# quocdat32461997/ggpm

Hardware: AMD Instinct MI355X
Metric: HierMPNEncoder fwd+bwd target row (SURVEY 8(d): encoder + KL heads + optimizer, tree fixed-point hint on; full depth loops in full_depth_loops, the full VAE fwd+bwd row in vae_step) of BASELINE's molecules/sec VAE fwd+bwd (hidden=300, depth=20, batch=32) (higher is better)
Workload: dtype f32

## Files before the change

### ggpm_amd/_lib.py

```python
from __future__ import annotations

import ctypes
import os
from ctypes import c_char_p, c_double, c_float, c_int, c_size_t, c_void_p, POINTER

from . import build as _build

_LIB = None

P = c_void_p
I = c_int
SIGNATURES = {
    "ggpm_version": (I, []),
    "ggpm_error_string": (c_char_p, [I]),
    "ggpm_padded_hidden": (I, [I]),
    "ggpm_padded_to_csr": (I, [P, I, I, P, P, P]),
    "ggpm_csr_transpose": (I, [P, P, I, I, P, P, P, P]),
    "ggpm_extract_column": (I, [P, I, I, I, P, P]),
    "ggpm_gemm_workspace_bytes": (c_size_t, [I, I, I]),
    "ggpm_gemm": (I, [I, I, I, I, I, P, I, P, I, P, I, I, P, I, I, I, P, c_size_t, P]),
    "ggpm_gemm_grouped": (I, [I, I, I, I, I, I, P, P]),
    "ggpm_gemm_grouped_splitk_workspace_bytes": (c_size_t, [I, I, I, I]),
    "ggpm_gemm_grouped_splitk": (I, [I, I, I, I, I, I, P, P, c_size_t, P]),
    "ggpm_gemm_ksegments": (I, [I, I, I, I, P, P, P, P, P, P, I, I, P, I, I, I, P]),
    "ggpm_gemm_tn_bf16": (I, [I, I, I, P, I, P, I, P, I, P, c_size_t, P]),
    "ggpm_gemm_tn_bf16_applies": (I, [I, I, I]),
    "ggpm_colsum": (I, [P, I, I, I, P, P, P]),
    "ggpm_act_backward": (I, [P, P, I, I, I, I, I, P, P]),
    "ggpm_segment_sum": (I, [P, I, P, P, I, I, P, I, I, I, P]),
    "ggpm_gather_rows": (I, [P, I, P, I, I, P, I, I, I, P]),
    "ggpm_scatter_rows": (I, [P, I, P, I, I, P, I, I, P]),
    "ggpm_adam_step": (I, [P, P, P, P, c_size_t, c_float, c_float, c_float, c_float, c_float, I, P]),
    "ggpm_flat_sqnorm_workspace_bytes": (c_size_t, [c_size_t]),
    "ggpm_flat_sqnorm_partials": (I, [P, c_size_t, P, c_size_t, P]),
    "ggpm_flat_norm_finish": (I, [P, I, c_float, P, P]),
    "ggpm_adam_step_groups": (I, [P, P, P, P, c_size_t, P, I, P, I, P, I, c_float, P, I, P]),
    "ggpm_onehot": (I, [P, I, I, P, I, I, I, P]),
    "ggpm_embed_graph": (I, [P, I, P, I, I, I, I, P, I, P, I, P]),
    "ggpm_level_bf16_storage": (I, [I, I]),
    "ggpm_gru_backward_stashes": (I, [P, I, I, I, POINTER(c_void_p), POINTER(c_void_p)]),
    "ggpm_lstm_backward_stashes": (I, [P, I, I, I, POINTER(c_void_p), POINTER(c_void_p), POINTER(c_void_p)]),
    "ggpm_sum_slots": (I, [P, I, c_size_t, P, P]),
    "ggpm_gru_pack_floats": (c_size_t, [I]),
    "ggpm_gru_forward": (I, [I, I, I, P, P, P, P, I, P, I, P, P, I, P, P, P, P, P, P, P, P, P, P, I, P, P]),
    "ggpm_gru_backward_workspace_bytes": (c_size_t, [I, I, I]),
    "ggpm_gru_backward": (I, [I, I, I, P, P, I, P, I, P, I, P, P, P, P, P, P, P, P, P, P, P, P, P, P, P,
                              P, I, P, I, P, P, I, P, c_size_t, I, P, P]),
    "ggpm_gru_weight_grads": (I, [I, I, I, P, P, P, P, c_size_t, P, I, P, I, P, P, I, P, P]),
    "ggpm_gru_sparse_forward": (I, [I, I, I, P, P, P, P, P, P, I, P, I, P, P, I, P, P, P, P, P, P, P, P, P, P, I, P, P]),
    "ggpm_gru_sparse_backward": (I, [I, I, I, P, P, P, I, P, I, P, I, P, P, P, P, P, P, P, P, P, P, P, P, P, P, P, P,
                                     P, I, P, I, P, P, I, P, c_size_t, P, P]),
    "ggpm_weight_grads_stacked_workspace_bytes": (c_size_t, [I, I]),
    "ggpm_gru_weight_grads_stacked": (I, [I, I, I, P, P, P, P, P, P, P, I, P, I, P, P, I, P, c_size_t, P]),
    "ggpm_lstm_weight_grads_stacked": (I, [I, I, I, P, P, P, P, P, P, P, I, P, I, P, I, P, I, P, c_size_t, P]),
    "ggpm_decode_steps_forward": (I, [P, P, P, P, P, P, P, P, P, c_size_t, P, P, P]),
    "ggpm_decode_steps_backward": (I, [P, P, P, P, P, P, P, P, c_size_t, P, P, P, P, c_size_t, P, P, P, c_size_t, P, P]),
    "ggpm_decode_steps_forward_async": (I, [P, P, P, P, P, P, P, P, P, c_size_t, P, P, P]),
    "ggpm_decode_steps_backward_async": (I, [P, P, P, P, P, P, P, P, c_size_t, P, P, P, P, c_size_t, P, P, P, c_size_t, P, P]),
    "ggpm_decode_join": (I, []),
    "ggpm_decode_steps_infer": (I, [P, P, P, P, P, P, P, P, P, P, P, P]),
    "ggpm_decode_steps_infer_async": (I, [P, P, P, P, P, P, P, P, P, P, P, P]),
    "ggpm_lstm_pack_floats": (c_size_t, [I]),
    "ggpm_lstm_forward": (I, [I, I, I, P, P, P, P, P, I, P, I, P, I, P, I, P, P, P, P, P, P, P, P, P, P, P, I, P, P]),
    "ggpm_lstm_backward_workspace_bytes": (c_size_t, [I, I, I]),
    "ggpm_lstm_backward": (I, [I, I, I, P, P, I, P, I, P, I, P, I, P, P, P, P, P, P, P, P, P, P, P, P, P,
                               P, P, P, P, P, I, P, I, P, I, P, I, P, c_size_t, I, P, P]),
    "ggpm_lstm_weight_grads": (I, [I, I, I, P, P, P, c_size_t, P, I, P, I, P, I, P, I, P, P]),
    "ggpm_lstm_sparse_forward": (I, [I, I, I, P, P, P, P, P, P, P, P, I, P, I, P, I, P, I, P, P, P, P, P, P, P, P, P, P,
                                     P, I, P, P]),
    "ggpm_lstm_sparse_backward": (I, [I, I, I, P, P, P, I, P, I, P, I, P, I, P, P, P, P, P, P, P, P, P, P, P, P, P, P,
                                      P, P, P, P, P, P, P, I, P, I, P, I, P, I, P, c_size_t, P, P]),
    "ggpm_rsample_forward": (I, [P, P, P, I, I, P, P, P]),
    "ggpm_rsample_backward": (I, [P, P, P, P, P, I, I, P, P, P]),
    "ggpm_softmax_ce": (I, [P, I, I, I, P, I, P, P, P, P, I, P, P, P]),
    "ggpm_bce_logits": (I, [P, P, I, P, P, P, P]),
    "ggpm_scale_rows": (I, [P, I, I, I, P, P]),
    "ggpm_head_accuracies": (I, [P, P, P, P, I, P, I, P, I, P, I, I, I, I, P, P]),
    "ggpm_motif_assm_forward": (I, [P, I, P, I, I, I, I, P, I, P, P, P, P, I, P, P, P, P, P, P]),
    "ggpm_motif_assm_backward": (I, [P, P, I, P, I, I, I, I, I, P, I, P, P, P, I, P, P, P, P, P, P, P, P, P, P]),
    "ggpm_motif_decode_tree_step": (I, [I, I, I, I, POINTER(c_void_p), P, P, P, P, I, I, P, P, P, I, I, P, I, P, I, P, I,
                                        P, I, P]),
    "ggpm_motif_decode_mlp": (I, [P, I, P, P, I, I, I, I, P, P, P, P, I, I, P, I, P, I, P]),
    "ggpm_hier_topk": (I, [P, I, I, P, I, I, P, I, I, I, P, P]),
    "ggpm_motif_decode_assm_score": (I, [P, I, I, I, P, P, I, P, I, P, P, P, P, I, P, P]),
    "ggpm_hier_decode_atom_step": (I, [P, P, P, P, P, P, I, P]),
    "ggpm_hier_decode_tree_step": (I, [P, P, P, P, I, P, I, P, I, I, P, I, P, I, P]),
    "ggpm_hier_decode_assm_score": (I, [P, P, P, P, P, P, I, I, I, I, P, I, P, P, P, I, P, I, I, P, P]),
    "ggpm_sample_topo": (I, [P, P, P, I, I, ctypes.c_uint, ctypes.c_uint, P, P]),
    "ggpm_sample_beam_order": (I, [P, P, P, I, I, I, ctypes.c_uint, ctypes.c_uint, P, P]),
    "ggpm_sample_normal": (I, [P, I, I, I, P, ctypes.c_uint, ctypes.c_uint, P]),
    "ggpm_sample_latent_normal": (I, [P, I, I, I, P, ctypes.c_uint, ctypes.c_uint, P]),
    "ggpm_mol_loss_parts": (I, [P, I, P, P]),
    "ggpm_latent_terms": (I, [P, P, P, I, I, I, P, P, P, P]),
    "ggpm_iwae_finish": (I, [P, P, P, I, I, P, P, P]),
    "ggpm_dropout": (I, [P, I, I, I, ctypes.c_float, ctypes.c_uint, ctypes.c_uint, I, P]),
    "ggpm_property_heads_workspace_bytes": (c_size_t, [I, I, P, P]),
# ... 66 lines not shown
```

### ggpm_amd/csrc/common.h

```cpp
#pragma once
#include <hip/hip_runtime.h>
#include <stdint.h>
#include <stdlib.h>
#include <atomic>
#include <mutex>
#include "../../include/ggpm_hip.h"

typedef float f32x4 __attribute__((ext_vector_type(4)));
typedef float f32x16 __attribute__((ext_vector_type(16)));

#define GGPM_WAVE 64

#define GGPM_CHECK_LAUNCH()                                   \
    do {                                                      \
        if (hipGetLastError() != hipSuccess) return GGPM_ERR_LAUNCH; \
    } while (0)

#define GGPM_CLEAR_STALE_ERROR() (void)hipGetLastError()

#ifdef GGPM_DEV_SWITCHES
inline const char* ggpm_dev_env(const char* name) { return getenv(name); }
#else
inline const char* ggpm_dev_env(const char*) { return nullptr; }
#endif
// ... 48 lines not shown
__device__ __forceinline__ float4 operator*(float4 a, float4 b) {
    return make_float4(a.x * b.x, a.y * b.y, a.z * b.z, a.w * b.w);
}
__device__ __forceinline__ float4 ggpm_sigmoid4(float4 a) {
    return make_float4(ggpm_sigmoid(a.x), ggpm_sigmoid(a.y), ggpm_sigmoid(a.z), ggpm_sigmoid(a.w));
}
__device__ __forceinline__ float4 ggpm_zero4() { return make_float4(0.f, 0.f, 0.f, 0.f); }
__device__ __forceinline__ float ggpm_fsigmoid_fast(float x) { return __frcp_rn(1.0f + __expf(-x)); }
__device__ __forceinline__ float ggpm_fsigmoid_acc(float x) {
    const float L_hi = 1.44269502162933349609375f, L_lo = 1.925963033500011e-08f, LN2 = 0.693147182464599609375f;
    const float nx = -__builtin_amdgcn_fmed3f(x, -88.f, 88.f);
    const float t = nx * L_hi;
    float lo = __builtin_fmaf(nx, L_hi, -t);
    lo = __builtin_fmaf(nx, L_lo, lo);
    float e = __builtin_amdgcn_exp2f(t);
    e = __builtin_fmaf(e, lo * LN2, e);
    const float d = 1.0f + e;
    const float r = __builtin_amdgcn_rcpf(d);
    return __builtin_fmaf(__builtin_fmaf(-d, r, 1.0f), r, r);
}
#ifdef GGPM_ABL_EXACT_GATHER_SIGMOID
template <bool BF16> __device__ __forceinline__ float ggpm_fsigmoid(float x) { return ggpm_sigmoid(x); }
#elif defined(GGPM_ABL_FAST_GATHER_SIGMOID)
template <bool BF16> __device__ __forceinline__ float ggpm_fsigmoid(float x) { return ggpm_fsigmoid_fast(x); }
#elif defined(GGPM_ABL_FAST_SIGMOID_BF16)
template <bool BF16> __device__ __forceinline__ float ggpm_fsigmoid(float x) { return BF16 ? ggpm_fsigmoid_fast(x) : ggpm_fsigmoid_acc(x); }
#else
template <bool BF16> __device__ __forceinline__ float ggpm_fsigmoid(float x) { return ggpm_fsigmoid_acc(x); }
#endif
template <bool BF16> __device__ __forceinline__ float4 ggpm_fsigmoid4(float4 a) {
    return make_float4(ggpm_fsigmoid<BF16>(a.x), ggpm_fsigmoid<BF16>(a.y), ggpm_fsigmoid<BF16>(a.z), ggpm_fsigmoid<BF16>(a.w));
}

__device__ __forceinline__ void ggpm_lds_barrier() {
    asm volatile("s_waitcnt lgkmcnt(0)\n\ts_barrier" ::: "memory");
}

bool ggpm_gemm_prefers_grouped(int M, int N, int K, int count);
int ggpm_gemm_tall_grouped(int M, int N, int count, const ggpm_gemm_problem* p, const int* K, float* ws, size_t ws_bytes,
                           ggpm_stream_t stream, int bf16 = 0);
#define GGPM_GEMM_MAX_GROUP 4
typedef ggpm_gemm_problem GgpmGemmProblem;

inline const ggpm_level_opts& ggpm_opts_or_default(const ggpm_level_opts* opts) {
    static const ggpm_level_opts none = {};
    return opts ? *opts : none;
}
int ggpm_gru_bias_u_grad(int E1, int H, int depth, int lo, float* work, float* dbu, float* csws, const ggpm_level_opts* opts,
                         ggpm_stream_t stream);
int ggpm_gru_sparse_weight_grads(int E1, int H, int depth, const float* Hs, const float* Ss, const float* Gs, float* work,
                                 size_t work_bytes, float* dWz_h, int ld_dwz, float* dUr, int ld_dur, float* dbu, float* dWh_h,
                                 int ld_dwh, const ggpm_level_opts* opts, ggpm_stream_t stream);
int ggpm_lstm_sparse_weight_grads(int E1, int H, int depth, const float* Hs, const float* Ss, float* work, size_t work_bytes,
                                  float* dWi_h, int ld_dwi, float* dWo_h, int ld_dwo, float* dWu_h, int ld_dwu, float* dWf_h,
                                  int ld_dwf, const ggpm_level_opts* opts, ggpm_stream_t stream);
hipEvent_t ggpm_wgrad_event(int i);

bool ggpm_bf16_storage_applies(int E1, int H);
int ggpm_sum_slots_any(const float* src, int slots, size_t slot_floats, float* out, bool src_bf16, ggpm_stream_t stream);
int ggpm_sum_slots_pair_grouped(int count, const float* const* src, const int* slots, size_t slot_floats, float* const* hi,
                                float* const* lo, ggpm_stream_t stream);
struct ggpm_pair_problem { const float *hi, *lo, *B; float* C; int ldc; };
int ggpm_gemm_tn_pair_grouped(int M, int N, int rows, int ld, int count, const ggpm_pair_problem* p, ggpm_stream_t stream);
int ggpm_colsum_any(const float* A, int lda, int rows, int cols, float* out, float* scratch, bool a_bf16, ggpm_stream_t stream);

void ggpm_timing_tag(int tag);
// ... 3 lines not shown
```

### ggpm_amd/csrc/encoder.hip

```cpp
#include "common.h"
#include <condition_variable>
#include <cstring>
#include <cstdlib>
#include <deque>
#include <functional>
#include <mutex>
#include <thread>

hipEvent_t ggpm_wgrad_event(int i);

namespace {

struct Arena {
    char* base;
    size_t off;
    bool overflow;
    size_t cap;
    template <typename T>
    T* take(size_t n) {
        const size_t bytes = (n * sizeof(T) + 255) & ~(size_t)255;
        T* p = base ? reinterpret_cast<T*>(base + off) : nullptr;
        off += bytes;
        if (base && off > cap) overflow = true;
        return p;
// ... 279 lines not shown
inline int backward_lo(const Dims& d, int level, int depth, int E1) {
    static const bool off = ggpm_dev_env("GGPM_TREE_FIXED_POINT") && atoi(ggpm_dev_env("GGPM_TREE_FIXED_POINT")) == 0;
    if (off || level == 2 || bf16_stored(d, E1) || d.tree_chain <= 0) return 1;
    const int lo = depth - d.tree_chain + 1;
    return lo < 1 ? 1 : lo;
}

inline int fixed_slot(const Dims& d, int level, int depth, int E1) {
    const int run = run_steps(d, level, depth, E1);
    if (run >= depth || d.gate_dtype == 1) return 0;
    const int blo = backward_lo(d, level, depth, E1);
    return (blo >= run && blo >= 3) ? run : 0;
}

int replicate_tail(const Dims& d, int E1, int depth, int run, int level, const LevelSaved& L, ggpm_stream_t s) {
    if (run >= depth || fixed_slot(d, level, depth, E1)) return GGPM_OK;
    const size_t slot = (size_t)E1 * d.Hp, ds = (size_t)depth * slot;
    const int blo = backward_lo(d, level, depth, E1);
    ReplicateArgs r = {};
    int n = 0;
    auto add = [&](float* base, int src, int lo, int hi) {
        r.base[n] = base; r.src[n] = src; r.lo[n] = lo > src ? lo : src + 1; r.hi[n] = hi; ++n;
    };
    add(L.Hs, run, blo, depth);
    if (L.Cs) add(L.Cs, run, blo, depth);
    add(L.Qs, run, blo, depth - 1);
    for (int k = 0; k < 5; ++k) add(L.St + k * ds, run - 1, blo - 1, depth - 1);
    r.slot4 = slot / 4;
    dim3 grid((unsigned)ggpm_ceil_div((int)r.slot4, 256 * 4), n);
    replicate_slots_k<<<grid, 256, 0, (hipStream_t)s>>>(r);
    return GGPM_OK;
}

int level_forward(const Dims& d, int E1, int N1, int I, int depth, const float* x, int ldx, float* const* P, int level,
                  const Csr& pred, const Csr& agr, LevelSaved& L, ggpm_stream_t s) {
    const int H = d.H, Hp = d.Hp;
    const size_t slot = (size_t)E1 * Hp;
    const int run = run_steps(d, level, depth, E1);
    struct Tag { Tag(int level) { ggpm_timing_tag(3 - level); } ~Tag() { ggpm_timing_tag(0); } } tag(level);
    ggpm_level_opts o = level_opts(d);
    o.run_depth = run;
    const bool infer = L.hout != nullptr;
    o.h_out = L.hout;
    const int fs = infer ? 0 : fixed_slot(d, level, depth, E1);
    o.fixed_slot = fs;
    const float* result = infer ? L.hout : L.Hs + (size_t)(fs ? fs : depth) * slot;
    if (d.lstm) {
        const float* W[4] = {P[lq(level, Q_WI)], P[lq(level, Q_WOG)], P[lq(level, Q_WU)], P[lq(level, Q_WF)]};
        const float* b[4] = {P[lq(level, Q_BI)], P[lq(level, Q_BOG)], P[lq(level, Q_BU)], P[lq(level, Q_BF)]};
        GgpmGemmProblem gp[4];
        for (int k = 0; k < 4; ++k) gp[k] = {x, ldx, W[k], I + H, L.X + k * slot, Hp, Hp, b[k], 0, GGPM_ACT_NONE, 0};
        CK(ggpm_gemm_grouped(0, 1, E1, H, I, 4, gp, s));
        const size_t dsl = (size_t)depth * slot;
        CK(ggpm_lstm_forward(E1, H, depth, L.X, L.X + slot, L.X + 2 * slot, L.X + 3 * slot, W[0] + I, I + H, W[1] + I, I + H,
                             W[2] + I, I + H, W[3] + I, I + H, pred.rowptr, pred.col, L.Hs, L.Cs, L.Qs,
                             infer ? nullptr : L.St, infer ? nullptr : L.St + dsl, infer ? nullptr : L.St + 2 * dsl,
                             infer ? nullptr : L.St + 3 * dsl, infer ? nullptr : L.St + 4 * dsl, L.wpack, infer ? 0 : 1, &o, s));
        if (!infer) CK(replicate_tail(d, E1, depth, run, level, L, s));
        CK(ggpm_segment_sum(result, Hp, agr.rowptr, agr.col, N1, H, L.nei, Hp, 0, Hp, s));
        return GGPM_OK;
    }
    const float *Wz = P[lp(level, L_WZ)], *Wr = P[lp(level, L_WR)], *Wh = P[lp(level, L_WH)];
    const GgpmGemmProblem gp[3] = {{x, ldx, Wz, I + H, L.X, Hp, Hp, P[lp(level, L_BZ)], 0, GGPM_ACT_NONE, 0},
                                   {x, ldx, Wr, I, L.X + slot, Hp, Hp, nullptr, 0, GGPM_ACT_NONE, 0},
                                   {x, ldx, Wh, I + H, L.X + 2 * slot, Hp, Hp, P[lp(level, L_BH)], 0, GGPM_ACT_NONE, 0}};
    CK(ggpm_gemm_grouped(0, 1, E1, H, I, 3, gp, s));
    const size_t ds = (size_t)depth * slot;
    CK(ggpm_gru_forward(E1, H, depth, L.X, L.X + slot, L.X + 2 * slot, Wz + I, I + H, P[lp(level, L_UR)], H,
                            P[lp(level, L_BU)], Wh + I, I + H, pred.rowptr, pred.col,
                            L.Hs, L.Qs, infer ? nullptr : L.St, infer ? nullptr : L.St + ds, infer ? nullptr : L.St + 2 * ds,
                            infer ? nullptr : L.St + 3 * ds, infer ? nullptr : L.St + 4 * ds, L.wpack, infer ? 0 : 1, &o, s));
    if (!infer) CK(replicate_tail(d, E1, depth, run, level, L, s));
    CK(ggpm_segment_sum(result, Hp, agr.rowptr, agr.col, N1, H, L.nei, Hp, 0, Hp, s));
    return GGPM_OK;
}

int transpose(const Csr& c, const int32_t* col, ggpm_stream_t s) {
    return ggpm_csr_transpose(c.rowptr, col ? col : c.col, c.rows, c.ncols, c.rowptrT, c.colT, c.cursor, s);
}

}

extern "C" size_t ggpm_encoder_saved_bytes(const ggpm_enc_dims* dims) {
    if (!dims) return 0;
    const Dims d = make_dims(dims);
    Arena A = {nullptr, 0, false, 0};
    Saved s;
    layout_saved(A, d, s);
    return A.off;
}

extern "C" size_t ggpm_encoder_infer_bytes(const ggpm_enc_dims* dims) {
    if (!dims) return 0;
    const Dims d = make_dims(dims);
    Arena A = {nullptr, 0, false, 0};
    Saved s;
    layout_infer(A, d, s);
    return A.off;
}

static int encoder_forward_impl(const ggpm_enc_dims* dims, float* const* params, const int64_t* tfnode,
                                const int64_t* tfmess, const int64_t* tagraph, const int64_t* tbgraph,
                                const int64_t* tcgraph, const int64_t* gfnode, const int64_t* gfmess,
                                const int64_t* gagraph, const int64_t* gbgraph, const int32_t* roots, void* saved,
                                size_t saved_bytes, float* hroot, float* hnode, float* hinter, float* hatom,
                                ggpm_stream_t stream, ggpm_stream_t side_stream, bool infer) {
    GGPM_CLEAR_STALE_ERROR();
    if (!dims || !params || !tfnode || !tfmess || !tagraph || !tbgraph || !tcgraph || !gfnode || !gfmess || !gagraph ||
        !gbgraph || !roots || !saved || !hroot || !hnode || !hinter || !hatom)
        return GGPM_ERR_ARG;
    const Dims d = make_dims(dims);
    Arena A = {reinterpret_cast<char*>(saved), 0, false, saved_bytes};
    Saved S;
    if (infer) layout_infer(A, d, S);
    else layout_saved(A, d, S);
    if (A.overflow) return GGPM_ERR_WORKSPACE;
    hipStream_t s = (hipStream_t)stream;
    float* const* P = params;
    const int H = d.H, Hp = d.Hp, He = d.He;

    ggpm_stream_t ts = side_stream ? side_stream : stream;
    SideWorker* wk = side_stream ? SideWorker::get() : nullptr;
    DrainGuard guard = {wk};
    hipEvent_t ev_in = nullptr;
    if (side_stream) {
        ev_in = ggpm_wgrad_event(60);
        if (!ev_in) return GGPM_ERR_LAUNCH;
        (void)hipEventRecord(ev_in, s);
    }
    CK(ggpm_padded_to_csr(gbgraph, d.E1g, d.Kgb, S.gpred.rowptr, S.gpred.col, stream));
    CK(ggpm_padded_to_csr(gagraph, d.N1g, d.Kga, S.gagr.rowptr, S.gagr.col, stream));
    hipEvent_t ev_atom = nullptr, ev_tree = nullptr;
    if (side_stream) {
        ev_atom = ggpm_wgrad_event(54);
        ev_tree = ggpm_wgrad_event(53);
        if (!ev_atom || !ev_tree) return GGPM_ERR_LAUNCH;
        (void)hipEventRecord(ev_atom, s);
    }
    auto tree_layout = [=]() -> int {
        if (side_stream) (void)hipStreamWaitEvent((hipStream_t)side_stream, ev_in, 0);
        CK(ggpm_padded_to_csr(tbgraph, d.E1t, d.Ktb, S.tpred.rowptr, S.tpred.col, ts));
        CK(ggpm_padded_to_csr(tagraph, d.N1t, d.Kta, S.tagr.rowptr, S.tagr.col, ts));
        CK(ggpm_padded_to_csr(tcgraph, d.N1t, d.Ktc, S.tcgr.rowptr, S.tcgr.col, ts));
        CK(ggpm_extract_column(tfmess, d.E1t, 4, 0, S.src, ts));
        CK(ggpm_extract_column(tfmess, d.E1t, 4, 2, S.attr0, ts));
        CK(ggpm_extract_column(tfnode, d.N1t, 2, 0, S.motif_id, ts));
        CK(ggpm_extract_column(tfnode, d.N1t, 2, 1, S.attach_id, ts));
        if (!infer) {
            const int nio = (d.E1t > d.N1t ? d.E1t : d.N1t) + 1;
            const int n = nio > d.B + 1 ? nio : d.B + 1;
            iota_k<<<ggpm_ceil_div(n, 256), 256, 0, (hipStream_t)ts>>>(S.iota, n);
        }
        CK(ggpm_gather_rows(P[P_EI], He, S.attach_id, d.N1t, He, S.finput_i, d.Hep, 0, d.Hep, ts));
        CK(drop(d, S.finput_i, d.N1t, He, d.Hep, DS_EI, ts));
        CK(ggpm_gather_rows(P[P_EC], He, S.motif_id, d.N1t, He, S.finput_t, d.Hep, 0, d.Hep, ts));
        CK(drop(d, S.finput_t, d.N1t, He, d.Hep, DS_EC, ts));
        CK(ggpm_onehot(S.attr0, d.E1t, 20, S.hmess_i, d.ld_t, H, d.ld_t, ts));
        CK(ggpm_onehot(S.attr0, d.E1t, 20, S.hmess_t, d.ld_t, H, d.ld_t, ts));
        if (side_stream) (void)hipEventRecord(ev_tree, (hipStream_t)side_stream);
        if (infer) return GGPM_OK;
        if (side_stream) (void)hipStreamWaitEvent((hipStream_t)side_stream, ev_atom, 0);
        CK(transpose(S.gpred, nullptr, ts));
        CK(transpose(S.gagr, nullptr, ts));
        CK(transpose(S.tpred, nullptr, ts));
        CK(transpose(S.tagr, nullptr, ts));
        CK(transpose(S.tcgr, nullptr, ts));
        CK(transpose(S.tsrc, S.src, ts));
        CK(transpose(S.root, roots, ts));
        CK(transpose(S.motif, S.motif_id, ts));
        CK(transpose(S.attach, S.attach_id, ts));
        return GGPM_OK;
    };
    if (wk) {
        int dev = 0;
        (void)hipGetDevice(&dev);
        wk->use_device(dev);
        wk->post(tree_layout);
    } else {
        CK(tree_layout());
    }

    CK(ggpm_embed_graph(gfnode, d.N1g, gfmess, d.E1g, d.atom, 4, 20, S.hnode_a, d.ld_n, S.hmess_a, d.ld_m, stream));
    CK(level_forward(d, d.E1g, d.N1g, d.Ig, d.depthG, S.hmess_a, d.ld_m, P, 2, S.gpred, S.gagr, S.lv[2], stream));
    CK(linear2(d.N1g, H, S.hnode_a, d.ld_n, d.atom, S.lv[2].nei, Hp, H, P[lwo(d.lstm, 2)], P[lbo(d.lstm, 2)], GGPM_ACT_RELU, 1,
               hatom, Hp, stream));
    CK(drop(d, hatom, d.N1g, H, Hp, DS_WO_ATOM, stream));

    if (wk) CK(wk->drain());
    if (side_stream) (void)hipStreamWaitEvent(s, ev_tree, 0);
    CK(ggpm_segment_sum(hatom, Hp, S.tcgr.rowptr, S.tcgr.col, d.N1t, H, S.pooled, Hp, 0, Hp, stream));
    CK(linear2(d.N1t, H, S.finput_i, d.Hep, He, S.pooled, Hp, H, P[P_WI], P[P_BI], GGPM_ACT_RELU, 0, S.hnode_i, Hp,
               stream));
    CK(drop(d, S.hnode_i, d.N1t, H, Hp, DS_WI, stream));
    CK(ggpm_gather_rows(S.hnode_i, Hp, S.src, d.E1t, H, S.hmess_i, d.ld_t, 0, 0, stream));
    CK(level_forward(d, d.E1t, d.N1t, d.It, d.depthT, S.hmess_i, d.ld_t, P, 1, S.tpred, S.tagr, S.lv[1], stream));
    CK(linear2(d.N1t, H, S.hnode_i, Hp, H, S.lv[1].nei, Hp, H, P[lwo(d.lstm, 1)], P[lbo(d.lstm, 1)], GGPM_ACT_RELU, 1, hinter, Hp,
               stream));
    CK(drop(d, hinter, d.N1t, H, Hp, DS_WO_INTER, stream));

    CK(linear2(d.N1t, H, S.finput_t, d.Hep, He, hinter, Hp, H, P[P_WC], P[P_BC], GGPM_ACT_RELU, 0, S.hnode_t, Hp, stream));
    CK(drop(d, S.hnode_t, d.N1t, H, Hp, DS_WC, stream));
    CK(ggpm_gather_rows(S.hnode_t, Hp, S.src, d.E1t, H, S.hmess_t, d.ld_t, 0, 0, stream));
    CK(level_forward(d, d.E1t, d.N1t, d.It, d.depthT, S.hmess_t, d.ld_t, P, 0, S.tpred, S.tagr, S.lv[0], stream));
    CK(linear2(d.N1t, H, S.hnode_t, Hp, H, S.lv[0].nei, Hp, H, P[lwo(d.lstm, 0)], P[lbo(d.lstm, 0)], GGPM_ACT_RELU, 1, hnode, Hp,
               stream));
    CK(drop(d, hnode, d.N1t, H, Hp, DS_WO_TREE, stream));

    CK(ggpm_gather_rows(S.hnode_t, Hp, roots, d.B, H, S.f, Hp, 0, Hp, stream));
    CK(ggpm_gather_rows(S.lv[0].nei, Hp, roots, d.B, H, S.n, Hp, 0, Hp, stream));
    CK(linear2(d.B, H, S.f, Hp, H, S.n, Hp, H, P[P_WROOT], P[P_BROOT], GGPM_ACT_TANH, 0, hroot, Hp, stream));
    GGPM_CHECK_LAUNCH();
    return GGPM_OK;
}

extern "C" int ggpm_encoder_forward(const ggpm_enc_dims* dims, float* const* params, const int64_t* tfnode,
                                    const int64_t* tfmess, const int64_t* tagraph, const int64_t* tbgraph,
                                    const int64_t* tcgraph, const int64_t* gfnode, const int64_t* gfmess,
                                    const int64_t* gagraph, const int64_t* gbgraph, const int32_t* roots, void* saved,
                                    size_t saved_bytes, float* hroot, float* hnode, float* hinter, float* hatom,
                                    ggpm_stream_t stream, ggpm_stream_t side_stream) {
    return encoder_forward_impl(dims, params, tfnode, tfmess, tagraph, tbgraph, tcgraph, gfnode, gfmess, gagraph, gbgraph,
                                roots, saved, saved_bytes, hroot, hnode, hinter, hatom, stream, side_stream, false);
}

extern "C" int ggpm_encoder_infer(const ggpm_enc_dims* dims, float* const* params, const int64_t* tfnode,
                                  const int64_t* tfmess, const int64_t* tagraph, const int64_t* tbgraph,
                                  const int64_t* tcgraph, const int64_t* gfnode, const int64_t* gfmess,
                                  const int64_t* gagraph, const int64_t* gbgraph, const int32_t* roots, void* arena,
                                  size_t arena_bytes, float* hroot, float* hnode, float* hinter, float* hatom,
                                  ggpm_stream_t stream, ggpm_stream_t side_stream) {
    return encoder_forward_impl(dims, params, tfnode, tfmess, tagraph, tbgraph, tcgraph, gfnode, gfmess, gagraph, gbgraph,
                                roots, arena, arena_bytes, hroot, hnode, hinter, hatom, stream, side_stream, true);
}

namespace {

struct BwdWork {
    float *dpre_root, *df, *dn, *d_hnode_t, *d_nei_t, *dpre, *d_h, *dX, *dx_mess, *d_finput, *d_hinter, *d_hnode_i,
        *d_nei_i, *d_pooled, *d_hatom, *d_nei_g, *level_work, *skws, *csws;
    size_t level_work_bytes, skws_bytes;
    float *xws[3], *xcs[3];
    size_t xws_bytes;
};

void layout_work(Arena& A, const Dims& d, BwdWork& w) {
    const int Hp = d.Hp;
    const int Nmax = d.N1g > d.N1t ? d.N1g : d.N1t, Emax = d.E1g > d.E1t ? d.E1g : d.E1t;
    w.dpre_root = A.take<float>((size_t)d.B * Hp); w.df = A.take<float>((size_t)d.B * Hp);
    w.dn = A.take<float>((size_t)d.B * Hp);
    w.d_hnode_t = A.take<float>((size_t)d.N1t * Hp); w.d_nei_t = A.take<float>((size_t)d.N1t * Hp);
    w.dpre = A.take<float>((size_t)5 * Nmax * Hp);
    w.d_h = A.take<float>((size_t)Emax * Hp);
    w.dX = A.take<float>((size_t)3 * 4 * Emax * Hp);
    w.dx_mess = A.take<float>((size_t)d.E1t * d.ld_t);
    w.d_finput = A.take<float>((size_t)2 * d.N1t * d.Hep);
    w.d_hinter = A.take<float>((size_t)d.N1t * Hp);
    w.d_hnode_i = A.take<float>((size_t)d.N1t * Hp); w.d_nei_i = A.take<float>((size_t)d.N1t * Hp);
    w.d_pooled = A.take<float>((size_t)d.N1t * Hp);
    w.d_hatom = A.take<float>((size_t)d.N1g * Hp); w.d_nei_g = A.take<float>((size_t)d.N1g * Hp);
    size_t lw = d.lstm ? ggpm_lstm_backward_workspace_bytes(d.E1g, d.H, d.depthG)
                       : ggpm_gru_backward_workspace_bytes(d.E1g, d.H, d.depthG);
    const size_t lwt = d.lstm ? ggpm_lstm_backward_workspace_bytes(d.E1t, d.H, d.depthT)
                              : ggpm_gru_backward_workspace_bytes(d.E1t, d.H, d.depthT);
    w.level_work_bytes = lw > lwt ? lw : lwt;
    w.level_work = A.take<float>(3 * (w.level_work_bytes / 4 + 64));
    size_t sk = 0;
    const int Imax = d.It > d.Ig ? d.It : d.Ig;
    const size_t cand[] = {ggpm_gemm_workspace_bytes(d.H, Imax, Emax), ggpm_gemm_workspace_bytes(d.H, d.Hp, Nmax),
                           ggpm_gemm_workspace_bytes(d.H, d.Hp, d.B)};
    for (size_t c : cand) sk = c > sk ? c : sk;
    w.skws_bytes = sk + 1024;
    w.skws = A.take<float>(w.skws_bytes / 4);
    w.csws = A.take<float>((size_t)256 * (Hp > d.ld_t ? Hp : d.ld_t));
    const int gates = d.lstm ? 4 : 3;
    const size_t xa = ggpm_gemm_grouped_splitk_workspace_bytes(d.H, d.It, d.E1t, gates);
    const size_t xb = ggpm_gemm_grouped_splitk_workspace_bytes(d.H, d.Ig, d.E1g, gates);
    w.xws_bytes = (xa > xb ? xa : xb) + 256;
    for (int l = 0; l < 3; ++l) {
        w.xws[l] = A.take<float>(w.xws_bytes / 4);
        w.xcs[l] = A.take<float>((size_t)256 * Hp);
    }
}

struct Streams {
    ggpm_stream_t main, side;
    int n_ev;
    SideWorker* wk;
    int side_after_main() {
        if (!side) return GGPM_OK;
        hipEvent_t ev = ggpm_wgrad_event(n_ev++ & 31);
        if (!ev) return GGPM_ERR_LAUNCH;
        (void)hipEventRecord(ev, (hipStream_t)main);
// ... 14 lines not shown
};

int linear2_dx(int M, int H, int K1, const float* dpre, int ldp, const float* W, float* d1, int ld1, int acc1, float* d2,
               int ld2, int acc2, ggpm_stream_t s) {
    const int ldw = K1 + H;
    if (K1 == H) {
        const GgpmGemmProblem gp[2] = {{dpre, ldp, W, ldw, d1, ld1, ld1, nullptr, acc1, GGPM_ACT_NONE, 0},
                                       {dpre, ldp, W + K1, ldw, d2, ld2, ld2, nullptr, acc2, GGPM_ACT_NONE, 0}};
        return ggpm_gemm_grouped(0, 0, M, H, H, 2, gp, s);
    }
    CK(ggpm_gemm(0, 0, M, K1, H, dpre, ldp, W, ldw, d1, ld1, ld1, nullptr, acc1, GGPM_ACT_NONE, 0, nullptr, 0, s));
    CK(ggpm_gemm(0, 0, M, H, H, dpre, ldp, W + K1, ldw, d2, ld2, ld2, nullptr, acc2, GGPM_ACT_NONE, 0, nullptr, 0, s));
    return GGPM_OK;
}

int linear2_wgrad(int M, int N, const float* dpre, int ldp, const float* x1, int ld1, int K1, const float* x2, int ld2,
                  int K2, float* dW, float* db, BwdWork& w, Streams& st) {
    CK(st.side_after_main());
    const int ldw = K1 + K2;
    const ggpm_stream_t sw = st.w();
    float* const skws = w.skws;
    float* const csws = w.csws;
    const size_t skb = w.skws_bytes;
    return st.on_side([=]() -> int {
        CK(ggpm_gemm(1, 0, N, K1, M, dpre, ldp, x1, ld1, dW, ldw, K1, nullptr, 0, GGPM_ACT_NONE, 0, skws, skb, sw));
        CK(ggpm_gemm(1, 0, N, K2, M, dpre, ldp, x2, ld2, dW + K1, ldw, K2, nullptr, 0, GGPM_ACT_NONE, 0, skws, skb, sw));
        if (db) CK(ggpm_colsum(dpre, ldp, M, N, db, csws, sw));
        return GGPM_OK;
    });
}

int level_backward(const Dims& d, int E1, int I, int depth, const float* x, int ldx, float* const* P, float* const* G,
                   int level, const Csr& pred, const LevelSaved& L, const float* dHD, float* dX, float* level_work,
                   float* dx, int lddx, BwdWork& w, Streams& st) {
    const int H = d.H, Hp = d.Hp;
    const size_t slot = (size_t)E1 * Hp, ds = (size_t)depth * slot;
    const int blo = backward_lo(d, level, depth, E1);
    struct Tag { Tag(int level) { ggpm_timing_tag(3 - level); } ~Tag() { ggpm_timing_tag(0); } } tag(level);
    static const bool xsum_env = !(ggpm_dev_env("GGPM_SKIP_XSUM") && atoi(ggpm_dev_env("GGPM_SKIP_XSUM")) == 0);
    const bool skip_xsum = xsum_env && dx == nullptr && depth > 1;
    ggpm_level_opts o = level_opts(d);
    o.lo = blo;
    o.fixed_slot = fixed_slot(d, level, depth, E1);
    o.skip_x_sums = skip_xsum;
    if (d.lstm) {
        const float* W[4] = {P[lq(level, Q_WI)], P[lq(level, Q_WOG)], P[lq(level, Q_WU)], P[lq(level, Q_WF)]};
        float* dW[4] = {G[lq(level, Q_WI)], G[lq(level, Q_WOG)], G[lq(level, Q_WU)], G[lq(level, Q_WF)]};
        float* db[4] = {G[lq(level, Q_BI)], G[lq(level, Q_BOG)], G[lq(level, Q_BU)], G[lq(level, Q_BF)]};
        CK(ggpm_lstm_backward(E1, H, depth, L.X + 3 * slot, W[0] + I, I + H, W[1] + I, I + H, W[2] + I, I + H, W[3] + I, I + H,
                              pred.rowptr, pred.col, pred.rowptrT, pred.colT, L.Hs, L.Cs, L.Qs, L.St, L.St + ds,
                              L.St + 2 * ds, L.St + 3 * ds, L.St + 4 * ds, dHD, dX, dX + slot, dX + 2 * slot, dX + 3 * slot,
                              dW[0] + I, I + H, dW[1] + I, I + H, dW[2] + I, I + H, dW[3] + I, I + H, level_work,
                              w.level_work_bytes, 0, &o, st.main));
        if (dx) {
            const float* A[4] = {dX, dX + slot, dX + 2 * slot, dX + 3 * slot};
            const int lda[4] = {Hp, Hp, Hp, Hp}, ldb[4] = {I + H, I + H, I + H, I + H}, K[4] = {H, H, H, H};
            CK(ggpm_gemm_ksegments(0, E1, I, 4, A, lda, W, ldb, K, dx, lddx, lddx, nullptr, 0, GGPM_ACT_NONE, 0, st.main));
        }
        CK(st.side_after_main());
        const ggpm_stream_t sw = st.w();
        const BwdWork wc = w;
        float* const dW0 = dW[0]; float* const dW1 = dW[1]; float* const dW2 = dW[2]; float* const dW3 = dW[3];
        float* const db0 = db[0]; float* const db1 = db[1]; float* const db2 = db[2]; float* const db3 = db[3];
        const float* Hs = L.Hs; const float* St = L.St;
        auto x_part = [=](ggpm_stream_t sx) -> int {
            float* const dWk[4] = {dW0, dW1, dW2, dW3};
            float* const dbk[4] = {db0, db1, db2, db3};
            if (skip_xsum) {
                float *DI = nullptr, *DO = nullptr, *DU = nullptr;
                CK(ggpm_lstm_backward_stashes(level_work, E1, H, depth, &DI, &DO, &DU));
                const int lo_ = blo < 1 ? 1 : blo;
                float* const src[3] = {DI, DO, DU};
                const bool b16 = bf16_stored(d, E1);
                for (int k = 0; k < 3; ++k)
                    CK(ggpm_sum_slots_any(src[k] + (b16 ? 0 : (size_t)(lo_ - 1) * slot), depth - lo_ + 1, slot, dX + (size_t)k * slot,
                                          b16, sx));
            }
// ... 94 lines not shown
                                     const float* hnode, const float* hinter, const float* hatom, const float* d_hroot,
                                     const float* d_hnode, const float* d_hinter, const float* d_hatom, void* work,
                                     size_t work_bytes, int phase, ggpm_stream_t stream, ggpm_stream_t side_stream) {
    GGPM_CLEAR_STALE_ERROR();
    if (!dims || !params || !grads || !roots || !saved || !work || !hroot || !hnode || !hinter || !hatom || phase < 0 ||
        phase > 2)
        return GGPM_ERR_ARG;
    const Dims d = make_dims(dims);
    Arena A = {reinterpret_cast<char*>(saved), 0, false, saved_bytes};
    Saved S;
    layout_saved(A, d, S);
    Arena B = {reinterpret_cast<char*>(work), 0, false, work_bytes};
    BwdWork w;
    layout_work(B, d, w);
    if (A.overflow || B.overflow) return GGPM_ERR_WORKSPACE;
    hipStream_t s = (hipStream_t)stream;
    float* const* P = params;
    float* const* G = grads;
    const int H = d.H, Hp = d.Hp, He = d.He;
    Streams st = {stream, side_stream, 0, side_stream ? SideWorker::get() : nullptr};
    DrainGuard guard = {st.wk};
    if (st.wk) {
        int dev = 0;
        (void)hipGetDevice(&dev);
        st.wk->use_device(dev);
    }
    const int Nmax = d.N1g > d.N1t ? d.N1g : d.N1t, Emax = d.E1g > d.E1t ? d.E1g : d.E1t;
    float* dpre[5];
    for (int i = 0; i < 5; ++i) dpre[i] = w.dpre + (size_t)i * Nmax * Hp;
    float* dXl[3];
    for (int i = 0; i < 3; ++i) dXl[i] = w.dX + (size_t)i * 4 * Emax * Hp;
    float* lwork[3];
    for (int i = 0; i < 3; ++i) lwork[i] = w.level_work + (size_t)i * (w.level_work_bytes / 4 + 64);
    const size_t nt = (size_t)d.N1t * Hp * sizeof(float), ng = (size_t)d.N1g * Hp * sizeof(float);

    if (side_stream && phase != 2) {
        hipEvent_t ev = ggpm_wgrad_event(61);
        if (!ev) return GGPM_ERR_LAUNCH;
        (void)hipEventRecord(ev, (hipStream_t)side_stream);
        (void)hipStreamWaitEvent(s, ev, 0);
    }
    if (phase != 2) {
    if (d_hroot) {
        CK(ggpm_act_backward(d_hroot, hroot, d.B, H, Hp, GGPM_ACT_TANH, 0, w.dpre_root, stream));
        CK(linear2_dx(d.B, H, H, w.dpre_root, Hp, P[P_WROOT], w.df, Hp, 0, w.dn, Hp, 0, stream));
        CK(ggpm_segment_sum(w.df, Hp, S.root.rowptrT, S.root.colT, d.N1t, H, w.d_hnode_t, Hp, 0, Hp, stream));
        CK(ggpm_segment_sum(w.dn, Hp, S.root.rowptrT, S.root.colT, d.N1t, H, w.d_nei_t, Hp, 0, Hp, stream));
        CK(linear2_wgrad(d.B, H, w.dpre_root, Hp, S.f, Hp, H, S.n, Hp, H, G[P_WROOT], G[P_BROOT], w, st));
    } else {
        (void)hipMemsetAsync(w.d_hnode_t, 0, nt, s);
        (void)hipMemsetAsync(w.d_nei_t, 0, nt, s);
        float* const gw = G[P_WROOT]; float* const gb = G[P_BROOT];
        const ggpm_stream_t sw = st.w();
        CK(st.on_side([=]() -> int {
            (void)hipMemsetAsync(gw, 0, (size_t)H * 2 * H * sizeof(float), (hipStream_t)sw);
            (void)hipMemsetAsync(gb, 0, (size_t)H * sizeof(float), (hipStream_t)sw);
            return GGPM_OK;
        }));
    }

    if (d_hnode) {
        CK(ggpm_act_backward(d_hnode, hnode, d.N1t, H, Hp, GGPM_ACT_RELU, 1, dpre[0], stream));
        CK(drop(d, dpre[0], d.N1t, H, Hp, DS_WO_TREE, stream));
        CK(linear2_dx(d.N1t, H, H, dpre[0], Hp, P[lwo(d.lstm, 0)], w.d_hnode_t, Hp, 1, w.d_nei_t, Hp, 1, stream));
        CK(linear2_wgrad(d.N1t, H, dpre[0], Hp, S.hnode_t, Hp, H, S.lv[0].nei, Hp, H, G[lwo(d.lstm, 0)], G[lbo(d.lstm, 0)], w, st));
    } else {
        float* const gw = G[lwo(d.lstm, 0)]; float* const gb = G[lbo(d.lstm, 0)];
        const ggpm_stream_t sw = st.w();
        CK(st.on_side([=]() -> int {
            (void)hipMemsetAsync(gw, 0, (size_t)H * 2 * H * sizeof(float), (hipStream_t)sw);
            (void)hipMemsetAsync(gb, 0, (size_t)H * sizeof(float), (hipStream_t)sw);
            return GGPM_OK;
        }));
    }
    CK(ggpm_segment_sum(w.d_nei_t, Hp, S.tagr.rowptrT, S.tagr.colT, d.E1t, H, w.d_h, Hp, 0, Hp, stream));
    CK(level_backward(d, d.E1t, d.It, d.depthT, S.hmess_t, d.ld_t, P, G, 0, S.tpred, S.lv[0], w.d_h, dXl[0], lwork[0],
                      w.dx_mess, d.ld_t, w, st));
    CK(ggpm_segment_sum(w.dx_mess, d.ld_t, S.tsrc.rowptrT, S.tsrc.colT, d.N1t, H, w.d_hnode_t, Hp, 1, 0, stream));
    CK(ggpm_act_backward(w.d_hnode_t, S.hnode_t, d.N1t, H, Hp, GGPM_ACT_RELU, 0, dpre[1], stream));
    CK(drop(d, dpre[1], d.N1t, H, Hp, DS_WC, stream));
    if (d_hinter) (void)hipMemcpyAsync(w.d_hinter, d_hinter, nt, hipMemcpyDeviceToDevice, s);
    CK(linear2_dx(d.N1t, H, He, dpre[1], Hp, P[P_WC], w.d_finput, d.Hep, 0, w.d_hinter, Hp, d_hinter ? 1 : 0, stream));
    CK(drop(d, w.d_finput, d.N1t, He, d.Hep, DS_EC, stream));
    CK(linear2_wgrad(d.N1t, H, dpre[1], Hp, S.finput_t, d.Hep, He, hinter, Hp, H, G[P_WC], G[P_BC], w, st));
    {
        const float* src = w.d_finput; const int32_t* rp = S.motif.rowptrT; const int32_t* cl = S.motif.colT;
        float* const g = G[P_EC]; const ggpm_stream_t sw = st.w(); const int Hep = d.Hep, rows = d.n_motif;
        CK(st.on_side([=]() -> int { return ggpm_segment_sum(src, Hep, rp, cl, rows, He, g, He, 0, He, sw); }));
    }

    CK(ggpm_act_backward(w.d_hinter, hinter, d.N1t, H, Hp, GGPM_ACT_RELU, 1, dpre[2], stream));
    CK(drop(d, dpre[2], d.N1t, H, Hp, DS_WO_INTER, stream));
    CK(linear2_dx(d.N1t, H, H, dpre[2], Hp, P[lwo(d.lstm, 1)], w.d_hnode_i, Hp, 0, w.d_nei_i, Hp, 0, stream));
    CK(linear2_wgrad(d.N1t, H, dpre[2], Hp, S.hnode_i, Hp, H, S.lv[1].nei, Hp, H, G[lwo(d.lstm, 1)], G[lbo(d.lstm, 1)], w, st));
    CK(ggpm_segment_sum(w.d_nei_i, Hp, S.tagr.rowptrT, S.tagr.colT, d.E1t, H, w.d_h, Hp, 0, Hp, stream));
    CK(level_backward(d, d.E1t, d.It, d.depthT, S.hmess_i, d.ld_t, P, G, 1, S.tpred, S.lv[1], w.d_h, dXl[1], lwork[1],
                      w.dx_mess, d.ld_t, w, st));
    CK(ggpm_segment_sum(w.dx_mess, d.ld_t, S.tsrc.rowptrT, S.tsrc.colT, d.N1t, H, w.d_hnode_i, Hp, 1, 0, stream));
    CK(ggpm_act_backward(w.d_hnode_i, S.hnode_i, d.N1t, H, Hp, GGPM_ACT_RELU, 0, dpre[3], stream));
    CK(drop(d, dpre[3], d.N1t, H, Hp, DS_WI, stream));
    float* d_finput_i = w.d_finput + (size_t)d.N1t * d.Hep;
    CK(linear2_dx(d.N1t, H, He, dpre[3], Hp, P[P_WI], d_finput_i, d.Hep, 0, w.d_pooled, Hp, 0, stream));
    CK(drop(d, d_finput_i, d.N1t, He, d.Hep, DS_EI, stream));
    CK(linear2_wgrad(d.N1t, H, dpre[3], Hp, S.finput_i, d.Hep, He, S.pooled, Hp, H, G[P_WI], G[P_BI], w, st));
    {
        const int32_t* rp = S.attach.rowptrT; const int32_t* cl = S.attach.colT;
        float* const g = G[P_EI]; const ggpm_stream_t sw = st.w(); const int Hep = d.Hep, rows = d.n_attach;
        CK(st.on_side([=]() -> int { return ggpm_segment_sum(d_finput_i, Hep, rp, cl, rows, He, g, He, 0, He, sw); }));
    }
    if (d_hatom) (void)hipMemcpyAsync(w.d_hatom, d_hatom, ng, hipMemcpyDeviceToDevice, s);
    CK(ggpm_segment_sum(w.d_pooled, Hp, S.tcgr.rowptrT, S.tcgr.colT, d.N1g, H, w.d_hatom, Hp, d_hatom ? 1 : 0,
                        d_hatom ? 0 : Hp, stream));

    }
    if (phase == 1) {
        CK(st.drain());
        GGPM_CHECK_LAUNCH();
        return GGPM_OK;
    }

    CK(ggpm_act_backward(w.d_hatom, hatom, d.N1g, H, Hp, GGPM_ACT_RELU, 1, dpre[4], stream));
    CK(drop(d, dpre[4], d.N1g, H, Hp, DS_WO_ATOM, stream));
    CK(ggpm_gemm(0, 0, d.N1g, H, H, dpre[4], Hp, P[lwo(d.lstm, 2)] + d.atom, d.atom + H, w.d_nei_g, Hp, Hp, nullptr, 0,
                 GGPM_ACT_NONE, 0, nullptr, 0, stream));
    CK(linear2_wgrad(d.N1g, H, dpre[4], Hp, S.hnode_a, d.ld_n, d.atom, S.lv[2].nei, Hp, H, G[lwo(d.lstm, 2)], G[lbo(d.lstm, 2)], w,
                     st));
    CK(ggpm_segment_sum(w.d_nei_g, Hp, S.gagr.rowptrT, S.gagr.colT, d.E1g, H, w.d_h, Hp, 0, Hp, stream));
    CK(level_backward(d, d.E1g, d.Ig, d.depthG, S.hmess_a, d.ld_m, P, G, 2, S.gpred, S.lv[2], w.d_h, dXl[2], lwork[2],
                      nullptr, 0, w, st));

    CK(st.drain());
    if (side_stream) {
        hipEvent_t ev = ggpm_wgrad_event(62);
        if (!ev) return GGPM_ERR_LAUNCH;
        (void)hipEventRecord(ev, (hipStream_t)side_stream);
        (void)hipStreamWaitEvent(s, ev, 0);
    }
    GGPM_CHECK_LAUNCH();
    return GGPM_OK;
}
```

### ggpm_amd/csrc/gather.hip

```cpp
#include "common.h"
#include <cmath>

namespace {

template <bool VEC>
__global__ void __launch_bounds__(256) segment_sum_k(const float* __restrict__ src, int ld_src,
                                                     const int32_t* __restrict__ rowptr,
                                                     const int32_t* __restrict__ col, int rows, int width,
                                                     float* __restrict__ out, int ld_out, int accumulate, int zero_to) {
    const int lane = threadIdx.x & 63;
    const int r = blockIdx.x * 4 + (threadIdx.x >> 6);
    if (r >= rows) return;
    const int lo = rowptr[r], hi = rowptr[r + 1];
    float* dst = out + (size_t)r * ld_out;
    for (int c = width + lane; c < zero_to; c += 64) dst[c] = 0.f;
    if (VEC) {
        for (int c = lane * 4; c < width; c += 256) {
            float4 acc = accumulate ? ggpm_ld4(dst + c) : ggpm_zero4();
            for (int j = lo; j < hi; ++j) acc = acc + ggpm_ld4(src + (size_t)col[j] * ld_src + c);
            ggpm_st4(dst + c, acc);
        }
    } else {
        for (int c = lane; c < width; c += 64) {
            float acc = accumulate ? dst[c] : 0.f;
            for (int j = lo; j < hi; ++j) acc += src[(size_t)col[j] * ld_src + c];
            dst[c] = acc;
        }
    }
}

__global__ void __launch_bounds__(256) gather_rows_k(const float* __restrict__ table, int ld_table,
                                                     const int32_t* __restrict__ idx, int rows, int width,
                                                     float* __restrict__ out, int ld_out, int col_off, int zero_to) {
    const int lane = threadIdx.x & 63;
    const int r = blockIdx.x * 4 + (threadIdx.x >> 6);
    if (r >= rows) return;
    const int id = idx[r];
    float* dst = out + (size_t)r * ld_out + col_off;
    for (int c = width + lane; c < zero_to - col_off; c += 64) dst[c] = 0.f;
    if (id < 0) {
        for (int c = lane; c < width; c += 64) dst[c] = 0.f;
    } else {
        const float* s = table + (size_t)id * ld_table;
        for (int c = lane; c < width; c += 64) dst[c] = s[c];
    }
}

__global__ void __launch_bounds__(256) scatter_rows_k(const float* __restrict__ src, int ld_src,
                                                      const int32_t* __restrict__ idx, int rows, int width,
                                                      float* __restrict__ dst, int ld_dst, int accumulate) {
    const int lane = threadIdx.x & 63;
    const int r = blockIdx.x * 4 + (threadIdx.x >> 6);
    if (r >= rows) return;
    const int id = idx[r];
    if (id < 0) return;
    const float* s = src + (size_t)r * ld_src;
    float* d = dst + (size_t)id * ld_dst;
    if (accumulate) for (int c = lane; c < width; c += 64) d[c] += s[c];
    else for (int c = lane; c < width; c += 64) d[c] = s[c];
}

__global__ void onehot_k(const int32_t* __restrict__ idx, int rows, int classes, float* __restrict__ out,
                         int ld_out, int col_off, int zero_to) {
    const int c = blockIdx.x * blockDim.x + threadIdx.x;
    const int r = blockIdx.y;
    if (col_off + c >= (zero_to > col_off + classes ? zero_to : col_off + classes)) return;
    out[(size_t)r * ld_out + col_off + c] = (c < classes && idx[r] == c) ? 1.f : 0.f;
}

__global__ void embed_graph_k(const int64_t* __restrict__ fnode, int N1, const int64_t* __restrict__ fmess,
                              int E1, int atom_size, int bond_types, int max_pos, float* __restrict__ hnode,
                              int ld_n, float* __restrict__ hmess, int ld_m) {
    const int r = blockIdx.x;
    const int c = threadIdx.x;
    if (r < N1) {
        if (c < ld_n) hnode[(size_t)r * ld_n + c] = (c < atom_size && fnode[r] == c) ? 1.f : 0.f;
    } else {
        const int e = r - N1;
        if (e < E1 && c < ld_m) {
            const int64_t* f = fmess + (size_t)e * 4;
            const int64_t a = fnode[f[0]];
            float v = 0.f;
            if (c < atom_size) v = (a == c) ? 1.f : 0.f;
            else if (c < atom_size + bond_types) v = (f[2] == c - atom_size) ? 1.f : 0.f;
            else if (c < atom_size + bond_types + max_pos) v = (f[3] == c - atom_size - bond_types) ? 1.f : 0.f;
            hmess[(size_t)e * ld_m + c] = v;
        }
    }
}

}

extern "C" int ggpm_segment_sum(const float* src, int ld_src, const int32_t* rowptr, const int32_t* col,
                                int rows, int width, float* out, int ld_out, int accumulate, int zero_to,
                                ggpm_stream_t stream) {
    GGPM_CLEAR_STALE_ERROR();
    if (!src || !rowptr || !col || !out || rows <= 0 || width <= 0) return GGPM_ERR_ARG;
    hipStream_t s = (hipStream_t)stream;
    const bool vec = (width % 4 == 0) && (ld_src % 4 == 0) && (ld_out % 4 == 0) &&
                     (((uintptr_t)src & 15) == 0) && (((uintptr_t)out & 15) == 0);
    const int grid = ggpm_ceil_div(rows, 4);
    if (vec) segment_sum_k<true><<<grid, 256, 0, s>>>(src, ld_src, rowptr, col, rows, width, out, ld_out, accumulate,
                                                           zero_to);
    else segment_sum_k<false><<<grid, 256, 0, s>>>(src, ld_src, rowptr, col, rows, width, out, ld_out, accumulate, zero_to);
    GGPM_CHECK_LAUNCH();
    return GGPM_OK;
}

extern "C" int ggpm_gather_rows(const float* table, int ld_table, const int32_t* idx, int rows, int width,
                                float* out, int ld_out, int col_off, int zero_to, ggpm_stream_t stream) {
    GGPM_CLEAR_STALE_ERROR();
    if (!table || !idx || !out || rows <= 0 || width <= 0) return GGPM_ERR_ARG;
    gather_rows_k<<<ggpm_ceil_div(rows, 4), 256, 0, (hipStream_t)stream>>>(table, ld_table, idx, rows, width, out,
                                                                          ld_out, col_off, zero_to);
    GGPM_CHECK_LAUNCH();
    return GGPM_OK;
}

extern "C" int ggpm_scatter_rows(const float* src, int ld_src, const int32_t* idx, int rows, int width, float* dst,
                                 int ld_dst, int accumulate, ggpm_stream_t stream) {
    GGPM_CLEAR_STALE_ERROR();
    if (!src || !idx || !dst || rows <= 0 || width <= 0) return GGPM_ERR_ARG;
    scatter_rows_k<<<ggpm_ceil_div(rows, 4), 256, 0, (hipStream_t)stream>>>(src, ld_src, idx, rows, width, dst, ld_dst,
                                                                           accumulate);
    GGPM_CHECK_LAUNCH();
    return GGPM_OK;
}

extern "C" int ggpm_onehot(const int32_t* idx, int rows, int classes, float* out, int ld_out, int col_off, int zero_to,
                           ggpm_stream_t stream) {
    GGPM_CLEAR_STALE_ERROR();
    if (!idx || !out || rows <= 0 || classes <= 0) return GGPM_ERR_ARG;
    const int span = (zero_to > col_off + classes ? zero_to - col_off : classes);
    dim3 grid(ggpm_ceil_div(span, 64), rows);
    onehot_k<<<grid, 64, 0, (hipStream_t)stream>>>(idx, rows, classes, out, ld_out, col_off, zero_to);
    GGPM_CHECK_LAUNCH();
    return GGPM_OK;
}

extern "C" int ggpm_embed_graph(const int64_t* fnode, int N1, const int64_t* fmess, int E1, int atom_size,
                                int bond_types, int max_pos, float* hnode, int ld_n, float* hmess, int ld_m,
                                ggpm_stream_t stream) {
    GGPM_CLEAR_STALE_ERROR();
    if (!fnode || !fmess || !hnode || !hmess || N1 <= 0 || E1 <= 0) return GGPM_ERR_ARG;
    if (ld_n > 256 || ld_m > 256 || ld_n < atom_size || ld_m < atom_size + bond_types + max_pos)
        return GGPM_ERR_UNSUPPORTED;
    embed_graph_k<<<N1 + E1, 256, 0, (hipStream_t)stream>>>(fnode, N1, fmess, E1, atom_size, bond_types, max_pos,
                                                           hnode, ld_n, hmess, ld_m);
    GGPM_CHECK_LAUNCH();
    return GGPM_OK;
}


namespace {
__device__ __forceinline__ unsigned int fmix32(unsigned int h) {
    h ^= h >> 16; h *= 0x85EBCA6Bu; h ^= h >> 13; h *= 0xC2B2AE35u; h ^= h >> 16;
    return h;
}

__global__ void dropout_k(float* __restrict__ x, int rows, int cols, int ld, unsigned int thresh, float scale,
                          unsigned int seed_lo, unsigned int seed_hi, unsigned int site) {
    const int c = blockIdx.x * blockDim.x + threadIdx.x;
    const int r = blockIdx.y;
    if (c >= cols) return;
    const unsigned int idx = (unsigned int)r * (unsigned int)cols + (unsigned int)c;
    unsigned int h = fmix32(idx * 0x9E3779B1u + seed_lo);
    h = fmix32(h ^ (seed_hi + site * 0x7F4A7C15u));
    float* p = x + (size_t)r * ld + c;
    *p = ((h >> 8) >= thresh) ? *p * scale : 0.f;
}
}

namespace {
__global__ void __launch_bounds__(256) adam_flat_k(float* __restrict__ p, const float* __restrict__ g,
                                                   float* __restrict__ m, float* __restrict__ v, size_t n, float b1,
                                                   float b2, float eps, float wd, float step_size, float inv_bc2_sqrt) {
    const size_t n4 = n >> 2;
    for (size_t i = (size_t)blockIdx.x * blockDim.x + threadIdx.x; i < n4; i += (size_t)gridDim.x * blockDim.x) {
        float4 pp = ggpm_ld4(p + 4 * i), gg = ggpm_ld4(g + 4 * i), mm = ggpm_ld4(m + 4 * i), vv = ggpm_ld4(v + 4 * i);
        float* P = &pp.x; float* G = &gg.x; float* M = &mm.x; float* V = &vv.x;
#pragma unroll
// ... 207 lines not shown
```

### ggpm_amd/csrc/gemm.hip

```cpp
#include <stdio.h>
#include <stdlib.h>
#include "common.h"

namespace {

constexpr int BM = 64, BN = 64, BK = 32, LDT = 68;

struct GemmArgs {
    int M, N, K;
    const float* A; int lda;
    const float* B; int ldb;
    float* C; int ldc; int n_pad;
    const float* bias;
    int accumulate, act, zero_row0;
    int vecA, vecB;
    int k_chunk;
    float* ws;
    unsigned long long* dbg;
    int nseg;
    const float* segA[GGPM_GEMM_MAX_GROUP];
    const float* segB[GGPM_GEMM_MAX_GROUP];
    int seg_lda[GGPM_GEMM_MAX_GROUP], seg_ldb[GGPM_GEMM_MAX_GROUP], segK[GGPM_GEMM_MAX_GROUP];
};

struct GemmGroupArgs {
    GemmArgs p[GGPM_GEMM_MAX_GROUP];
};

__device__ __forceinline__ float apply_act(float v, int act) {
    switch (act) {
        case GGPM_ACT_RELU: return v > 0.f ? v : 0.f;
        case GGPM_ACT_TANH: return tanhf(v);
        case GGPM_ACT_SIGMOID: return ggpm_sigmoid(v);
        default: return v;
    }
}

template <bool CONTIG_K>
__device__ __forceinline__ void fetch_tile(const float* __restrict__ P, int ld, int r0, int R, int k0, int kend,
                                           bool vec, float4 (&v)[2]) {
#pragma unroll
    for (int i = 0; i < 2; ++i) {
        const int f = threadIdx.x + 256 * i;
        float4 x = ggpm_zero4();
        if (CONTIG_K) {
            const int gr = r0 + (f >> 3), gk = k0 + (f & 7) * 4;
            if (gr < R && gk < kend) {
                const float* src = P + (size_t)gr * ld + gk;
                if (vec && gk + 3 < kend) x = ggpm_ld4(src);
                else {
                    x.x = src[0];
                    if (gk + 1 < kend) x.y = src[1];
                    if (gk + 2 < kend) x.z = src[2];
                    if (gk + 3 < kend) x.w = src[3];
                }
            }
        } else {
            const int gk = k0 + (f >> 4), gr = r0 + (f & 15) * 4;
            if (gk < kend && gr < R) {
                const float* src = P + (size_t)gk * ld + gr;
                if (vec && gr + 3 < R) x = ggpm_ld4(src);
                else {
                    x.x = src[0];
                    if (gr + 1 < R) x.y = src[1];
                    if (gr + 2 < R) x.z = src[2];
                    if (gr + 3 < R) x.w = src[3];
                }
            }
// ... 36 lines not shown
        fetch_tile<!TA>(g.A, g.lda, m0, g.M, kbeg, kend, g.vecA != 0, ra);
        fetch_tile<TB>(g.B, g.ldb, n0, g.N, kbeg, kend, g.vecB != 0, rb);
        for (int k0 = kbeg; k0 < kend; k0 += BK) {
            stash_tile<!TA>(ra, As);
            stash_tile<TB>(rb, Bs);
            __syncthreads();
            if (k0 + BK < kend) {
                fetch_tile<!TA>(g.A, g.lda, m0, g.M, k0 + BK, kend, g.vecA != 0, ra);
                fetch_tile<TB>(g.B, g.ldb, n0, g.N, k0 + BK, kend, g.vecB != 0, rb);
            }
#pragma unroll
            for (int kk = 0; kk < BK; kk += 2) {
                float a = As[kk + (lane >> 5)][wm * 32 + (lane & 31)];
                float b = Bs[kk + (lane >> 5)][wn * 32 + (lane & 31)];
                acc = __builtin_amdgcn_mfma_f32_32x32x2f32(a, b, acc, 0, 0, 0);
            }
            __syncthreads();
        }
    }

    const int n = n0 + wn * 32 + (lane & 31);
#pragma unroll
    for (int r = 0; r < 16; ++r) {
        const int m = m0 + wm * 32 + (r & 3) + 8 * (r >> 2) + 4 * (lane >> 5);
        if (m >= g.M) continue;
        if (g.ws) {
            if (n < g.N) g.ws[((size_t)blockIdx.z * g.M + m) * g.N + n] = acc[r];
            continue;
        }
        if (n < g.N) {
            float v = acc[r];
            if (g.bias) v += g.bias[n];
            float* dst = g.C + (size_t)m * g.ldc + n;
            if (g.accumulate) v += *dst;
            v = apply_act(v, g.act);
            if (g.zero_row0 && m == 0) v = 0.f;
            *dst = v;
        } else if (n < g.n_pad) {
            g.C[(size_t)m * g.ldc + n] = 0.f;
        }
    }
}

constexpr int BK2 = 64;

template <bool CONTIG_K>
struct OperandStage {
    __amdgpu_buffer_rsrc_t rs;
    unsigned voff[4], vstep;
    int loff[4];
    int kq[4];

    __device__ __forceinline__ void init(const float* P, int ld, int r0, int R, int kbeg, int kend, int total_rows) {
        const size_t last = CONTIG_K ? (size_t)(total_rows - 1) * ld + kend : (size_t)(max(kend, 1) - 1) * ld + R;
        const size_t bytes = kend > 0 ? last * 4 : 0;
        rs = __builtin_amdgcn_make_buffer_rsrc(const_cast<float*>(P), 0, (unsigned)bytes, 0x00020000);
#pragma unroll
        for (int i = 0; i < 4; ++i) {
            const int f = threadIdx.x + 256 * i;
            if (CONTIG_K) {
                const int r = f >> 4, k4 = (f & 15) * 4;
                kq[i] = k4;
                loff[i] = k4 * LDT + r;
                voff[i] = r0 + r < R ? (unsigned)(((size_t)(r0 + r) * ld + kbeg + k4) * 4) : 0xffffff00u;
            } else {
                const int k = f >> 4, c = (f & 15) * 4;
                kq[i] = 0;
// ... 73 lines not shown
            if (sg) ggpm_lds_barrier();
#pragma unroll
            for (int i = 0; i < 4; ++i) { sa.load(ra0[i], i); sb.load(rb0[i], i); }
#pragma unroll
            for (int i = 0; i < 4; ++i) {
                sa.store(Ls[0][0], ra0[i], i, kend - kbeg);
                sb.store(Ls[0][1], rb0[i], i, kend - kbeg);
            }
#pragma unroll
            for (int i = 0; i < 4; ++i) { sa.load(ra1[i], i); sb.load(rb1[i], i); }
            ggpm_lds_barrier();
            frag(0, 0, 0);
            for (int k0 = kbeg; k0 < kend; k0 += 2 * BK2) {
                step(ra1, rb1, ra0, rb0, 0, kend - k0 - BK2);
                step(ra0, rb0, ra1, rb1, 1, kend - k0 - 2 * BK2);
            }
        }
        asm volatile("s_nop 15\n\ts_nop 15" ::: "memory");
    }

    const int n = n0 + wn * 32 + (lane & 31);
#pragma unroll
    for (int r = 0; r < 16; ++r) {
        const int m = m0 + wm * 32 + (r & 3) + 8 * (r >> 2) + 4 * (lane >> 5);
        if (m >= g.M) continue;
        if (g.ws) {
            if (n < g.N) g.ws[((size_t)bz * g.M + m) * g.N + n] = acc[r];
            continue;
        }
        if (n < g.N) {
            float v = acc[r];
            if (g.bias) v += g.bias[n];
            float* dst = g.C + (size_t)m * g.ldc + n;
            if (g.accumulate) v += *dst;
            v = apply_act(v, g.act);
            if (g.zero_row0 && m == 0) v = 0.f;
            *dst = v;
        } else if (n < g.n_pad) {
            g.C[(size_t)m * g.ldc + n] = 0.f;
        }
    }
}

__device__ __forceinline__ void xcd_tile(int& bx, int& by, int& bz) {
    const unsigned T = gridDim.x * gridDim.y * gridDim.z;
    const unsigned L = blockIdx.x + gridDim.x * (blockIdx.y + gridDim.y * blockIdx.z);
    const unsigned xq = T >> 3, xr = T & 7, xcd = L & 7;
    const unsigned logical = xcd * xq + min(xcd, xr) + (L >> 3);
    bx = logical % gridDim.x;
    by = (logical / gridDim.x) % gridDim.y;
    bz = logical / (gridDim.x * gridDim.y);
}

template <bool TA, bool TB>
__global__ void __launch_bounds__(256) gemm_kernel_v2(GemmArgs g) {
    __shared__ __attribute__((aligned(16))) float Ls[2][2][BK2 * LDT];
    int bx, by, bz;
    xcd_tile(bx, by, bz);
    gemm_v2_tile<TA, TB>(g, bx, by, bz, Ls);
}

template <bool TA, bool TB>
__global__ void __launch_bounds__(256) gemm_group_v2(GemmGroupArgs gg) {
    __shared__ __attribute__((aligned(16))) float Ls[2][2][BK2 * LDT];
    int bx, by, bz;
    xcd_tile(bx, by, bz);
    gemm_v2_tile<TA, TB>(gg.p[bz], bx, by, 0, Ls);
// ... 141 lines not shown
#pragma unroll
        for (int i = 0; i < 2; ++i) { sa.load(ra1[i], i); sb.load(rb1[i], i); }
        next_load();
        ggpm_lds_barrier();
        frag(0, 0, 0);
        for (int s2 = 0; s2 < total_steps; s2 += 2) {
            step(ra1, rb1, ra0, rb0, 0);
            step(ra0, rb0, ra1, rb1, 1);
        }
        asm volatile("s_nop 15\n\ts_nop 15" ::: "memory");
    }

    float* part = &Ls[0][0][0];
    __syncthreads();
#pragma unroll
    for (int r = 0; r < 16; ++r) part[(wave * 16 + r) * 64 + lane] = acc[r];
    __syncthreads();
#pragma unroll
    for (int j = 0; j < 4; ++j) {
        const int idx = threadIdx.x + 256 * j, r = idx >> 6, l = idx & 63;
        const int m = m0 + (r & 3) + 8 * (r >> 2) + 4 * (l >> 5), n = n0 + (l & 31);
        if (m >= g.M) continue;
        if (g.ws) {
            if (n < g.N)
                g.ws[((size_t)chunk * g.M + m) * g.N + n] = (part[(0 * 16 + r) * 64 + l] + part[(1 * 16 + r) * 64 + l]) +
                                                             (part[(2 * 16 + r) * 64 + l] + part[(3 * 16 + r) * 64 + l]);
            continue;
        }
        if (n < g.N) {
            float v = (part[(0 * 16 + r) * 64 + l] + part[(1 * 16 + r) * 64 + l]) +
                      (part[(2 * 16 + r) * 64 + l] + part[(3 * 16 + r) * 64 + l]);
            if (g.bias) v += g.bias[n];
            float* dst = g.C + (size_t)m * g.ldc + n;
            if (g.accumulate) v += *dst;
            v = apply_act(v, g.act);
            if (g.zero_row0 && m == 0) v = 0.f;
            *dst = v;
        } else if (n < g.n_pad) {
            g.C[(size_t)m * g.ldc + n] = 0.f;
        }
    }
}

template <bool TA, bool TB>
__global__ void __launch_bounds__(256) gemm_small_v3(GemmGroupArgs gg, int splits) {
    __shared__ __attribute__((aligned(16))) float Ls[2][2][SK * SLD];
    int bx, by, bz;
    xcd_tile(bx, by, bz);
    gemm_v3_tile<TA, TB>(gg.p[bz / splits], bx, by, bz % splits, Ls);
}

__global__ void splitk_reduce_group(GemmGroupArgs gg, int splits) {
    const GemmArgs& g = gg.p[blockIdx.z];
    const int n = blockIdx.x * blockDim.x + threadIdx.x;
    const int m = blockIdx.y;
    if (n >= g.n_pad) return;
    float* dst = g.C + (size_t)m * g.ldc + n;
    if (n >= g.N) { *dst = 0.f; return; }
    float v = 0.f;
    for (int z = 0; z < splits; ++z) v += g.ws[((size_t)z * g.M + m) * g.N + n];
    if (g.bias) v += g.bias[n];
    if (g.accumulate) v += *dst;
    v = apply_act(v, g.act);
    if (g.zero_row0 && m == 0) v = 0.f;
    *dst = v;
}

// ... 475 lines not shown

__global__ void __launch_bounds__(256) colsum_stage2(const float* __restrict__ ws, int N, int chunks,
                                                     float* __restrict__ out) {
    __shared__ float red[4][64];
    const int n = blockIdx.x * 64 + (threadIdx.x & 63);
    const int rl = threadIdx.x >> 6;
    float v = 0.f;
    if (n < N)
        for (int c = rl; c < chunks; c += 4) v += ws[(size_t)c * N + n];
    red[rl][threadIdx.x & 63] = v;
    __syncthreads();
    if (rl == 0 && n < N) out[n] = (red[0][threadIdx.x] + red[1][threadIdx.x]) + (red[2][threadIdx.x] + red[3][threadIdx.x]);
}

constexpr int CS_ONE_MAX = 2048;
__global__ void __launch_bounds__(1024) colsum_one(const float* __restrict__ A, int lda, int M, int N,
                                                   float* __restrict__ out) {
    __shared__ float red[16][64];
    const int c = threadIdx.x & 63, n = blockIdx.x * 64 + c;
    const int rl = threadIdx.x >> 6;
    float v = 0.f;
    if (n < N)
        for (int m = rl; m < M; m += 16) v += A[(size_t)m * lda + n];
    red[rl][c] = v;
    __syncthreads();
    if (rl == 0 && n < N) {
        float t = 0.f;
#pragma unroll
        for (int i = 0; i < 16; ++i) t += red[i][c];
        out[n] = t;
    }
}

__global__ void act_backward_k(const float* __restrict__ dy, const float* __restrict__ y, int rows, int cols,
                               int ld, int act, int zero_row0, float* __restrict__ dpre) {
    const int c = blockIdx.x * blockDim.x + threadIdx.x;
    const int r = blockIdx.y;
    if (c >= cols) return;
    const size_t i = (size_t)r * ld + c;
    float g = dy[i], o = y[i];
    switch (act) {
        case GGPM_ACT_RELU: g = o > 0.f ? g : 0.f; break;
        case GGPM_ACT_TANH: g = g * (1.f - o * o); break;
        case GGPM_ACT_SIGMOID: g = g * o * (1.f - o); break;
        default: break;
    }
    if (zero_row0 && r == 0) g = 0.f;
    dpre[i] = g;
}

}

namespace {
inline bool small_launch(int M, int N, int count) {
    static const int use_v3 = [] { const char* e = ggpm_dev_env("GGPM_GEMM_V3"); return e ? atoi(e) : 1; }();
    static const int max_tiles = [] { const char* e = ggpm_dev_env("GGPM_GEMM_V3_TILES"); return e ? atoi(e) : 300; }();
    return use_v3 && (size_t)ggpm_ceil_div(M, BM) * ggpm_ceil_div(N, BN) * count <= (size_t)max_tiles;
}
inline void launch_small(int trans_a, int trans_b, const GemmGroupArgs& gg, int count, int M, int n_pad_max, hipStream_t s,
                         int splits = 1) {
    dim3 grid(ggpm_ceil_div(n_pad_max, SN), ggpm_ceil_div(M, SM), count * splits);
    if (!trans_a && !trans_b) gemm_small_v3<false, false><<<grid, 256, 0, s>>>(gg, splits);
    else if (!trans_a && trans_b) gemm_small_v3<false, true><<<grid, 256, 0, s>>>(gg, splits);
    else if (trans_a && !trans_b) gemm_small_v3<true, false><<<grid, 256, 0, s>>>(gg, splits);
    else gemm_small_v3<true, true><<<grid, 256, 0, s>>>(gg, splits);
}
inline int small_splits(int M, int N, int K, int count, int* k_chunk) {
    const int tiles = ggpm_ceil_div(M, SM) * ggpm_ceil_div(N, SN) * count;
    int want = 1024 / tiles, maxs = K / (4 * SK);
    int sp = want < maxs ? want : maxs;
    if (sp < 2) { *k_chunk = ggpm_round_up(K, BK); return 1; }
    *k_chunk = ggpm_round_up(ggpm_ceil_div(K, sp), SK);
    return ggpm_ceil_div(K, *k_chunk);
}
}

extern "C" size_t ggpm_gemm_workspace_bytes(int M, int N, int K) {
    const int s = choose_splits(M, N, K);
    size_t bytes = s > 1 ? (size_t)s * M * N * sizeof(float) : 0;
    if (tall_shape(M, N, K)) {
        const int ts = max(tall_splits(M, N, K), tall_splits(M, N, K, GGPM_TALL_BF16_WGS));
        if (ts > 1) bytes = max(bytes, ts * tall_slab_bytes(M, N));
    }
    return bytes;
}

extern "C" int ggpm_gemm(int trans_a, int trans_b, int M, int N, int K, const float* A, int lda,
                         const float* B, int ldb, float* C, int ldc, int n_pad, const float* bias,
                         int accumulate, int act, int zero_row0, float* splitk_ws, size_t splitk_ws_bytes,
                         ggpm_stream_t stream) {
    GGPM_CLEAR_STALE_ERROR();
    if (!A || !B || !C || M <= 0 || N <= 0 || K <= 0 || n_pad < N || n_pad > ldc) return GGPM_ERR_ARG;
    hipStream_t s = (hipStream_t)stream;
    GemmArgs g{};
    g.M = M; g.N = N; g.K = K; g.A = A; g.lda = lda; g.B = B; g.ldb = ldb; g.C = C; g.ldc = ldc;
    g.n_pad = n_pad; g.bias = bias; g.accumulate = accumulate; g.act = act; g.zero_row0 = zero_row0;
    g.vecA = ((lda & 3) == 0) && (((uintptr_t)A & 15) == 0);
    g.vecB = ((ldb & 3) == 0) && (((uintptr_t)B & 15) == 0);
    static const int use_tall = [] { const char* e = ggpm_dev_env("GGPM_GEMM_TALL"); return e ? atoi(e) : 1; }();
    if (use_tall && trans_a && !trans_b && g.vecA && g.vecB && lda >= ggpm_round_up(M, 4) && ldb >= ggpm_round_up(N, 4) &&
        tall_shape(M, N, K) && n_pad <= ggpm_round_up(N, TN) && (size_t)K * lda * 4 < 0xffffff00ull && (size_t)K * ldb * 4 < 0xffffff00ull) {
        const size_t slab = tall_slab_bytes(M, N);
        if (tall_split_mode() && splitk_ws && splitk_ws_bytes >= slab) {
            int sp = tall_splits(M, N, K, tall_split_wgs());
            if ((size_t)sp * slab > splitk_ws_bytes) sp = (int)(splitk_ws_bytes / slab);
            if (sp < 1) sp = 1;
            g.k_chunk = ggpm_round_up(ggpm_ceil_div(K, sp), BTK);
            sp = ggpm_ceil_div(K, g.k_chunk);
            g.ws = splitk_ws;
            const int tiles_n = ggpm_ceil_div(N, TN), tiles_m = ggpm_ceil_div(M, TM);
            GemmGroupArgs gg;
            for (int i = 0; i < GGPM_GEMM_MAX_GROUP; ++i) gg.p[i] = g;
            launch_tall_split(gg, dim3(tiles_n, tiles_m, sp), sp, s);
            tall_reduce<<<tiles_n * tiles_m * 100, 256, 0, s>>>(gg, sp, tiles_n, tiles_n * tiles_m);
            GGPM_CHECK_LAUNCH();
            return GGPM_OK;
        }
        int splits = splitk_ws ? tall_splits(M, N, K) : 1;
        if (splits > 1 && (size_t)splits * slab > splitk_ws_bytes) splits = (int)(splitk_ws_bytes / slab);
        if (splits < 1) splits = 1;
        g.k_chunk = ggpm_round_up(ggpm_ceil_div(K, splits), TK);
        splits = ggpm_ceil_div(K, g.k_chunk);
        g.ws = splits > 1 ? splitk_ws : nullptr;
        const int tiles_n = ggpm_ceil_div(N, TN), tiles_m = ggpm_ceil_div(M, TM);
        dim3 grid(tiles_n, tiles_m, splits);
        static unsigned long long* dbg = [] {
            unsigned long long* p = nullptr;
            if (ggpm_dev_env("GGPM_GEMM_DEBUG")) (void)hipMalloc(&p, 64);
            return p;
// ... 24 lines not shown
        g.k_chunk = ggpm_round_up(ggpm_ceil_div(K, splits), BK);
        splits = ggpm_ceil_div(K, g.k_chunk);
    }
    if (splits <= 1) { splits = 1; g.k_chunk = ggpm_round_up(K, BK); g.ws = nullptr; } else { g.ws = splitk_ws; }
    dim3 grid(ggpm_ceil_div(splits > 1 ? N : n_pad, BN), ggpm_ceil_div(M, BM), splits);
    static const int use_v2 = [] { const char* e = ggpm_dev_env("GGPM_GEMM_V2"); return e ? atoi(e) : 1; }();
    const size_t rows_a = trans_a ? K : M, rows_b = trans_b ? N : K;
    if (use_v2 && splits == 1 && small_launch(M, N, 1) && g.vecA && g.vecB && rows_a * lda * 4 < 0xffffff00ull &&
        rows_b * ldb * 4 < 0xffffff00ull) {
        GemmGroupArgs gg;
        for (int i = 0; i < GGPM_GEMM_MAX_GROUP; ++i) gg.p[i] = g;
        launch_small(trans_a, trans_b, gg, 1, M, n_pad, s);
        GGPM_CHECK_LAUNCH();
        return GGPM_OK;
    }
    const bool resident = (size_t)grid.x * grid.y * grid.z <= 512 || use_v2 == 2;
    if (use_v2 && resident && g.vecA && g.vecB && rows_a * lda * 4 < 0xffffff00ull && rows_b * ldb * 4 < 0xffffff00ull) {
        if (!trans_a && !trans_b) gemm_kernel_v2<false, false><<<grid, 256, 0, s>>>(g);
        else if (!trans_a && trans_b) gemm_kernel_v2<false, true><<<grid, 256, 0, s>>>(g);
        else if (trans_a && !trans_b) gemm_kernel_v2<true, false><<<grid, 256, 0, s>>>(g);
        else gemm_kernel_v2<true, true><<<grid, 256, 0, s>>>(g);
    } else if (!trans_a && !trans_b) gemm_kernel<false, false><<<grid, 256, 0, s>>>(g);
    else if (!trans_a && trans_b) gemm_kernel<false, true><<<grid, 256, 0, s>>>(g);
    else if (trans_a && !trans_b) gemm_kernel<true, false><<<grid, 256, 0, s>>>(g);
    else gemm_kernel<true, true><<<grid, 256, 0, s>>>(g);
    if (splits > 1) {
        dim3 rg(ggpm_ceil_div(n_pad, 256), M);
        splitk_reduce<<<rg, 256, 0, s>>>(g, splits);
    }
    GGPM_CHECK_LAUNCH();
    return GGPM_OK;
}

namespace {
inline bool v2_operands_ok(const float* A, int lda, size_t rows_a, const float* B, int ldb, size_t rows_b) {
    static const int use_v2 = [] { const char* e = ggpm_dev_env("GGPM_GEMM_V2"); return e ? atoi(e) : 1; }();
    return use_v2 && (lda & 3) == 0 && (ldb & 3) == 0 && ((uintptr_t)A & 15) == 0 && ((uintptr_t)B & 15) == 0 &&
           rows_a * lda * 4 < 0xffffff00ull && rows_b * ldb * 4 < 0xffffff00ull;
}
inline void fill_args(GemmArgs& g, int M, int N, int K, const GgpmGemmProblem& p) {
    g = GemmArgs{};
    g.M = M; g.N = N; g.K = K; g.A = p.A; g.lda = p.lda; g.B = p.B; g.ldb = p.ldb; g.C = p.C; g.ldc = p.ldc;
    g.n_pad = p.n_pad; g.bias = p.bias; g.accumulate = p.accumulate; g.act = p.act; g.zero_row0 = p.zero_row0;
    g.vecA = g.vecB = 1;
    g.k_chunk = ggpm_round_up(K, BK);
}
}

int ggpm_gemm_tall_grouped(int M, int N, int count, const GgpmGemmProblem* p, const int* K, float* ws, size_t ws_bytes,
                           ggpm_stream_t stream, int bf16) {
    GGPM_CLEAR_STALE_ERROR();
    if (count <= 0 || count > GGPM_GEMM_MAX_GROUP || !p || !K || M <= 0 || N <= 0) return GGPM_ERR_ARG;
    static const int use_tall = [] { const char* e = ggpm_dev_env("GGPM_GEMM_TALL"); return e ? atoi(e) : 1; }();
    const size_t slab = tall_slab_bytes(M, N);
    const bool in16 = bf16 == 2;
    const size_t es = in16 ? 2 : 4;
    bool ok = use_tall && (count > 1 || bf16) && ws != nullptr;
    const bool split = !bf16 && tall_split_mode() != 0;
    int splits = 1 << 30;
    for (int i = 0; i < count && ok; ++i) {
        ok = (p[i].lda & 3) == 0 && (p[i].ldb & 3) == 0 && ((uintptr_t)p[i].A & 15) == 0 && ((uintptr_t)p[i].B & 15) == 0 &&
             p[i].lda >= ggpm_round_up(M, 4) && p[i].ldb >= ggpm_round_up(N, 4) && tall_shape(M, N, K[i]) &&
             p[i].n_pad <= ggpm_round_up(N, TN) && p[i].n_pad >= N && p[i].n_pad <= p[i].ldc &&
             (size_t)K[i] * p[i].lda * es < 0xffffff00ull && (size_t)K[i] * p[i].ldb * es < 0xffffff00ull;
        splits = min(splits, tall_splits(M, N, K[i], bf16 ? GGPM_TALL_BF16_WGS / count : (split ? tall_split_wgs() / count : 0)));
    }
// ... 89 lines not shown
    bool ok = count > 1;
    int n_pad_max = 0;
    for (int i = 0; i < count; ++i) {
        if (!p[i].A || !p[i].B || !p[i].C || p[i].n_pad < N || p[i].n_pad > p[i].ldc) return GGPM_ERR_ARG;
        ok = ok && v2_operands_ok(p[i].A, p[i].lda, trans_a ? K : M, p[i].B, p[i].ldb, trans_b ? N : K);
        n_pad_max = max(n_pad_max, p[i].n_pad);
    }
    if (!ok) {
        for (int i = 0; i < count; ++i) {
            const int rc = ggpm_gemm(trans_a, trans_b, M, N, K, p[i].A, p[i].lda, p[i].B, p[i].ldb, p[i].C, p[i].ldc,
                                     p[i].n_pad, p[i].bias, p[i].accumulate, p[i].act, p[i].zero_row0, nullptr, 0, stream);
            if (rc) return rc;
        }
        return GGPM_OK;
    }
    GemmGroupArgs gg;
    for (int i = 0; i < count; ++i) fill_args(gg.p[i], M, N, K, p[i]);
    for (int i = count; i < GGPM_GEMM_MAX_GROUP; ++i) gg.p[i] = gg.p[0];
    hipStream_t s = (hipStream_t)stream;
    if (small_launch(M, N, count)) {
        launch_small(trans_a, trans_b, gg, count, M, n_pad_max, s);
        GGPM_CHECK_LAUNCH();
        return GGPM_OK;
    }
    dim3 grid(ggpm_ceil_div(n_pad_max, BN), ggpm_ceil_div(M, BM), count);
    if (!trans_a && !trans_b) gemm_group_v2<false, false><<<grid, 256, 0, s>>>(gg);
    else if (!trans_a && trans_b) gemm_group_v2<false, true><<<grid, 256, 0, s>>>(gg);
    else if (trans_a && !trans_b) gemm_group_v2<true, false><<<grid, 256, 0, s>>>(gg);
    else gemm_group_v2<true, true><<<grid, 256, 0, s>>>(gg);
    GGPM_CHECK_LAUNCH();
    return GGPM_OK;
}

extern "C" size_t ggpm_gemm_grouped_splitk_workspace_bytes(int M, int N, int K, int count) {
    if (M <= 0 || N <= 0 || K <= 0 || count <= 0 || count > GGPM_GEMM_MAX_GROUP || !small_launch(M, N, count)) return 0;
    int kc;
    const int sp = small_splits(M, N, K, count, &kc);
    return sp > 1 ? (size_t)sp * count * M * N * sizeof(float) : 0;
}

extern "C" int ggpm_gemm_grouped_splitk(int trans_a, int trans_b, int M, int N, int K, int count, const ggpm_gemm_problem* p,
                                        float* ws, size_t ws_bytes, ggpm_stream_t stream) {
    GGPM_CLEAR_STALE_ERROR();
    if (count <= 0 || count > GGPM_GEMM_MAX_GROUP || !p || M <= 0 || N <= 0 || K <= 0) return GGPM_ERR_ARG;
    const size_t need = ggpm_gemm_grouped_splitk_workspace_bytes(M, N, K, count);
    bool ok = need > 0 && ws && ws_bytes >= need;
    int n_pad_max = 0;
    for (int i = 0; i < count && ok; ++i) {
        if (!p[i].A || !p[i].B || !p[i].C || p[i].n_pad < N || p[i].n_pad > p[i].ldc) return GGPM_ERR_ARG;
        ok = v2_operands_ok(p[i].A, p[i].lda, trans_a ? K : M, p[i].B, p[i].ldb, trans_b ? N : K);
        n_pad_max = max(n_pad_max, p[i].n_pad);
    }
    if (!ok) return ggpm_gemm_grouped(trans_a, trans_b, M, N, K, count, p, stream);
    int kc;
    const int sp = small_splits(M, N, K, count, &kc);
    GemmGroupArgs gg;
    for (int i = 0; i < count; ++i) {
        fill_args(gg.p[i], M, N, K, p[i]);
        gg.p[i].k_chunk = kc;
        gg.p[i].ws = ws + (size_t)i * sp * M * N;
    }
    for (int i = count; i < GGPM_GEMM_MAX_GROUP; ++i) gg.p[i] = gg.p[0];
    hipStream_t s = (hipStream_t)stream;
    launch_small(trans_a, trans_b, gg, count, M, N, s, sp);
    splitk_reduce_group<<<dim3(ggpm_ceil_div(n_pad_max, 256), M, count), 256, 0, s>>>(gg, sp);
    GGPM_CHECK_LAUNCH();
// ... 43 lines not shown
    return GGPM_OK;
}

extern "C" int ggpm_colsum(const float* A, int lda, int M, int N, float* out, float* ws, ggpm_stream_t stream) {
    return ggpm_colsum_any(A, lda, M, N, out, ws, false, stream);
}

int ggpm_colsum_any(const float* A, int lda, int M, int N, float* out, float* ws, bool a_bf16, ggpm_stream_t stream) {
    GGPM_CLEAR_STALE_ERROR();
    if (!A || !out || !ws || M <= 0 || N <= 0) return GGPM_ERR_ARG;
    hipStream_t s = (hipStream_t)stream;
    if (a_bf16) {
        int chunks = ggpm_ceil_div(M, 128);
        if (chunks > CS_ROWS) chunks = CS_ROWS;
        colsum_stage1<true><<<dim3(ggpm_ceil_div(N, 64), chunks), 256, 0, s>>>(A, lda, M, N, ws);
        colsum_stage2<<<ggpm_ceil_div(N, 64), 256, 0, s>>>(ws, N, chunks, out);
        GGPM_CHECK_LAUNCH();
        return GGPM_OK;
    }
    if (M <= CS_ONE_MAX) {
        colsum_one<<<ggpm_ceil_div(N, 64), 1024, 0, s>>>(A, lda, M, N, out);
        GGPM_CHECK_LAUNCH();
        return GGPM_OK;
    }
    int chunks = ggpm_ceil_div(M, 128);
    if (chunks > CS_ROWS) chunks = CS_ROWS;
    dim3 g1(ggpm_ceil_div(N, 64), chunks);
    colsum_stage1<false><<<g1, 256, 0, s>>>(A, lda, M, N, ws);
    colsum_stage2<<<ggpm_ceil_div(N, 64), 256, 0, s>>>(ws, N, chunks, out);
    GGPM_CHECK_LAUNCH();
    return GGPM_OK;
}

extern "C" int ggpm_act_backward(const float* dy, const float* y, int rows, int cols, int ld, int act,
                                 int zero_row0, float* dpre, ggpm_stream_t stream) {
    GGPM_CLEAR_STALE_ERROR();
    if (!dy || !y || !dpre || rows <= 0 || cols <= 0) return GGPM_ERR_ARG;
    dim3 grid(ggpm_ceil_div(cols, 256), rows);
    act_backward_k<<<grid, 256, 0, (hipStream_t)stream>>>(dy, y, rows, cols, ld, act, zero_row0, dpre);
    GGPM_CHECK_LAUNCH();
    return GGPM_OK;
}

extern "C" int ggpm_linear_wgrads_batch(int count, const ggpm_wgrad_item* items, float* ws, size_t ws_bytes, float* csws,
                                        ggpm_stream_t stream) {
    if (count < 0 || (count > 0 && !items)) return GGPM_ERR_ARG;
    for (int i = 0; i < count; ++i) {
        const ggpm_wgrad_item& it = items[i];
        if (!it.dpre || !it.x || !it.dW || it.M <= 0 || it.N <= 0 || it.K <= 0) return GGPM_ERR_ARG;
        const size_t need = ggpm_gemm_workspace_bytes(it.N, it.K, it.M);
        const bool split = ws && need && need <= ws_bytes;
        int rc = ggpm_gemm(1, 0, it.N, it.K, it.M, it.dpre, it.ld_dpre, it.x, it.ld_x, it.dW, it.ld_dw, it.K, nullptr, 0, GGPM_ACT_NONE, 0,
                           split ? ws : nullptr, split ? ws_bytes : 0, stream);
        if (rc) return rc;
        if (it.db) {
            if (!csws) return GGPM_ERR_ARG;
            rc = ggpm_colsum(it.dpre, it.ld_dpre, it.M, it.N, it.db, csws, stream);
            if (rc) return rc;
        }
    }
    return GGPM_OK;
}
```

### ggpm_amd/csrc/graph.hip

```cpp
#include "common.h"

namespace {

constexpr int SCAN_THREADS = 1024;

__global__ void count_nonzero_rows(const int64_t* __restrict__ padded, int rows, int width,
                                   int32_t* __restrict__ counts) {
    int r = blockIdx.x * blockDim.x + threadIdx.x;
    if (r >= rows) return;
    const int64_t* p = padded + (size_t)r * width;
    int c = 0;
    for (int k = 0; k < width; ++k) c += (p[k] != 0);
    counts[r] = c;
}

__global__ void __launch_bounds__(SCAN_THREADS) exclusive_scan_1block(const int32_t* counts, int n,
                                                                      int32_t* out) {
    __shared__ int32_t partial[SCAN_THREADS];
    const int t = threadIdx.x;
    const int ipt = (n + SCAN_THREADS - 1) / SCAN_THREADS;
    const int lo = min(t * ipt, n), hi = min(lo + ipt, n);
    int32_t sum = 0;
    for (int i = lo; i < hi; ++i) sum += counts[i];
    partial[t] = sum;
// ... 68 lines not shown

__global__ void extract_column_k(const int64_t* __restrict__ mat, int rows, int width, int column,
                                 int32_t* __restrict__ out) {
    int r = blockIdx.x * blockDim.x + threadIdx.x;
    if (r < rows) out[r] = (int32_t)mat[(size_t)r * width + column];
}

constexpr int SMALL_ROWS = 16384;

__device__ __forceinline__ void block_exclusive_scan_inplace(int32_t* data, int n, int32_t* partial) {
    const int t = threadIdx.x;
    const int ipt = (n + SCAN_THREADS - 1) / SCAN_THREADS;
    const int lo = min(t * ipt, n), hi = min(lo + ipt, n);
    int32_t sum = 0;
    for (int i = lo; i < hi; ++i) sum += data[i];
    partial[t] = sum;
    __syncthreads();
    for (int off = 1; off < SCAN_THREADS; off <<= 1) {
        int32_t v = (t >= off) ? partial[t - off] : 0;
        __syncthreads();
        partial[t] += v;
        __syncthreads();
    }
    int32_t run = partial[t] - sum;
    for (int i = lo; i < hi; ++i) {
        int32_t c = data[i];
        data[i] = run;
        run += c;
    }
    if (t == SCAN_THREADS - 1) data[n] = partial[t];
    __syncthreads();
}

__global__ void __launch_bounds__(SCAN_THREADS) padded_to_csr_small(const int64_t* __restrict__ padded, int rows,
                                                                     int width, int32_t* __restrict__ rowptr,
                                                                     int32_t* __restrict__ col) {
    __shared__ int32_t partial[SCAN_THREADS];
    for (int r = threadIdx.x; r < rows; r += SCAN_THREADS) {
        const int64_t* p = padded + (size_t)r * width;
        int c = 0;
        for (int k = 0; k < width; ++k) c += (p[k] != 0);
        rowptr[r] = c;
    }
    __syncthreads();
    block_exclusive_scan_inplace(rowptr, rows, partial);
    for (int r = threadIdx.x; r < rows; r += SCAN_THREADS) {
        const int64_t* p = padded + (size_t)r * width;
        int o = rowptr[r];
        for (int k = 0; k < width; ++k) {
            const int64_t v = p[k];
            if (v != 0) col[o++] = (int32_t)v;
        }
    }
}

constexpr int SORT_SERIAL = 24, SORT_WAVE_CAP = 512, SORT_WAVES = SCAN_THREADS / 64, SORT_LIST = 512;
constexpr int SORT_BLOCK_CAP = SORT_WAVES * SORT_WAVE_CAP;
constexpr int SORT_PER_THREAD = 16;

__device__ __forceinline__ void insertion_sort_global(int32_t* colT, int lo, int hi) {
    for (int i = lo + 1; i < hi; ++i) {
        const int32_t v = colT[i];
        int j = i - 1;
        while (j >= lo && colT[j] > v) { colT[j + 1] = colT[j]; --j; }
        colT[j + 1] = v;
    }
}

__global__ void __launch_bounds__(SCAN_THREADS) csr_transpose_small(const int32_t* __restrict__ rowptr,
                                                                     const int32_t* __restrict__ col, int rows,
// ... 55 lines not shown
        for (int q = 0; q < SORT_PER_THREAD; ++q) {
            const int i = threadIdx.x + q * SCAN_THREADS;
            v[q] = i < n ? colT[lo + i] : 0;
            rank[q] = 0;
        }
        for (int c0 = 0; c0 < n; c0 += SORT_BLOCK_CAP) {
            const int cn = min(SORT_BLOCK_CAP, n - c0);
            for (int j = threadIdx.x; j < cn; j += SCAN_THREADS) stage[j] = colT[lo + c0 + j];
            __syncthreads();
            for (int j = 0; j < cn; ++j) {
                const int32_t x = stage[j];
                const int gj = c0 + j;
#pragma unroll
                for (int q = 0; q < SORT_PER_THREAD; ++q)
                    rank[q] += (x < v[q]) || (x == v[q] && gj < threadIdx.x + q * SCAN_THREADS);
            }
            __syncthreads();
        }
#pragma unroll
        for (int q = 0; q < SORT_PER_THREAD; ++q)
            if (threadIdx.x + q * SCAN_THREADS < n) colT[lo + rank[q]] = v[q];
        __syncthreads();
    }
}

}

extern "C" int ggpm_padded_to_csr(const int64_t* padded, int rows, int width, int32_t* rowptr, int32_t* col,
                                  ggpm_stream_t stream) {
    GGPM_CLEAR_STALE_ERROR();
    if (!padded || !rowptr || !col || rows <= 0 || width <= 0) return GGPM_ERR_ARG;
    hipStream_t s = (hipStream_t)stream;
    if (rows <= SMALL_ROWS) {
        padded_to_csr_small<<<1, SCAN_THREADS, 0, s>>>(padded, rows, width, rowptr, col);
        GGPM_CHECK_LAUNCH();
        return GGPM_OK;
    }
    const int T = 256, B = ggpm_ceil_div(rows, T);
    count_nonzero_rows<<<B, T, 0, s>>>(padded, rows, width, rowptr);
    exclusive_scan_1block<<<1, SCAN_THREADS, 0, s>>>(rowptr, rows, rowptr);
    fill_csr_from_padded<<<B, T, 0, s>>>(padded, rows, width, rowptr, col);
    GGPM_CHECK_LAUNCH();
    return GGPM_OK;
}

extern "C" int ggpm_csr_transpose(const int32_t* rowptr, const int32_t* col, int rows, int ncols,
                                  int32_t* rowptrT, int32_t* colT, int32_t* cursor, ggpm_stream_t stream) {
    GGPM_CLEAR_STALE_ERROR();
    if (!rowptr || !col || !rowptrT || !colT || !cursor || rows <= 0 || ncols <= 0) return GGPM_ERR_ARG;
    hipStream_t s = (hipStream_t)stream;
    if (rows <= SMALL_ROWS && ncols <= SMALL_ROWS) {
        csr_transpose_small<<<1, SCAN_THREADS, 0, s>>>(rowptr, col, rows, ncols, rowptrT, colT, cursor);
        GGPM_CHECK_LAUNCH();
        return GGPM_OK;
    }
    const int T = 256;
    zero_i32<<<ggpm_ceil_div(ncols + 1, T), T, 0, s>>>(rowptrT, ncols + 1);
    zero_i32<<<ggpm_ceil_div(ncols, T), T, 0, s>>>(cursor, ncols);
    count_columns<<<ggpm_ceil_div(rows, T), T, 0, s>>>(rowptr, col, rows, ncols, rowptrT);
    exclusive_scan_1block<<<1, SCAN_THREADS, 0, s>>>(rowptrT, ncols, rowptrT);
    fill_transpose<<<ggpm_ceil_div(rows, T), T, 0, s>>>(rowptr, col, rows, ncols, rowptrT, cursor, colT);
    sort_lists<<<ggpm_ceil_div(ncols, T), T, 0, s>>>(rowptrT, colT, ncols);
    GGPM_CHECK_LAUNCH();
    return GGPM_OK;
}

extern "C" int ggpm_extract_column(const int64_t* mat, int rows, int width, int column, int32_t* out,
                                   ggpm_stream_t stream) {
    GGPM_CLEAR_STALE_ERROR();
    if (!mat || !out || rows <= 0 || column < 0 || column >= width) return GGPM_ERR_ARG;
    extract_column_k<<<ggpm_ceil_div(rows, 256), 256, 0, (hipStream_t)stream>>>(mat, rows, width, column, out);
    GGPM_CHECK_LAUNCH();
    return GGPM_OK;
}
```

### ggpm_amd/csrc/mpn_gru.hip

```cpp
#include "tile_mma.h"
#include <cstdlib>
#include <cstdio>

__global__ void ggpm_pack_weight_kernel(GgpmPackArgs a) {
    const int Hp = a.Hp, H = a.H, KC = Hp / 16;
    const int lane = threadIdx.x;
    const int kc = blockIdx.x, t = blockIdx.y, m = blockIdx.z;
    const float* __restrict__ W = a.W[m];
    const int ldw = a.ldw[m];
    const int out = 16 * t + (lane & 15);
    if (a.bf16 == 2) {
        const int KC32 = ggpm_kc32_dev(Hp);
        float x[8];
#pragma unroll
        for (int i = 0; i < 8; ++i) {
            const int k = 32 * kc + 8 * (lane >> 4) + i;
            x[i] = (out < H && k < H) ? (a.transpose ? W[(size_t)k * ldw + out] : W[(size_t)out * ldw + k]) : 0.f;
        }
        uint2 lo[3], hi[3];
        ggpm_split3(make_float4(x[0], x[1], x[2], x[3]), lo[0], lo[1], lo[2]);
        ggpm_split3(make_float4(x[4], x[5], x[6], x[7]), hi[0], hi[1], hi[2]);
        __bf16* dst = reinterpret_cast<__bf16*>(a.dst) + (size_t)m * 2 * ggpm_packed_matrix_floats(Hp, 2);
#pragma unroll
        for (int pl = 0; pl < 3; ++pl)
// ... 789 lines not shown
        (void)hipMemcpy(h, a.dbg, sizeof(h), hipMemcpyDeviceToHost);
        fprintf(stderr, "[adebug bwd E1=%d grid=%dx%d fuse=%d] gather %.2f barrier %.2f gemm %.2f epilogue %.2f us\n", a.E1,
                grid_a.x, grid_a.y, a.fuse_b, (h[1] - h[0]) * 0.01, (h[2] - h[1]) * 0.01, (h[3] - h[2]) * 0.01,
                (h[4] - h[3]) * 0.01);
    }
    if (with_b) {
        ggpm_timing_begin(5, s, 2 * flops1);
        if (a.st16) { if (rt2) go(gru_bwd_b<1, 2, true>, lds); else go(gru_bwd_b<1, 1, true>, lds); }
        else if (rt2) { if (a.bf16 == 1) go(gru_bwd_b<1, 2>, lds); else go(gru_bwd_b<0, 2>, lds); }
        else { if (a.bf16 == 2) go(gru_bwd_b<2, 1>, lds); else if (a.bf16 == 1) go(gru_bwd_b<1, 1>, lds); else go(gru_bwd_b<0, 1>, lds); }
        ggpm_timing_end(5, s);
    }
}

}

extern "C" size_t ggpm_gru_pack_floats(int H) {
    const int Hp = ggpm_padded_hidden(H);
    return 3 * ggpm_packed_matrix_slot(Hp) + (size_t)Hp;
}

static int gru_shape_ok(int Hp) {
    return (size_t)2 * 16 * (Hp + 4) * sizeof(float) <= 160 * 1024;
}

namespace {
__global__ void sparse_init_state(const float* __restrict__ h_in, const unsigned char* __restrict__ frozen,
                                  float* __restrict__ H0, int Hp) {
    const int c = blockIdx.x * blockDim.x + threadIdx.x;
    const int r = blockIdx.y;
    if (c >= Hp) return;
    H0[(size_t)r * Hp + c] = frozen[r] ? h_in[(size_t)r * Hp + c] : 0.f;
}
}

static int gru_forward_impl(int E1, int H, int depth, const float* Xz, const float* Xr, const float* Xh,
                            const float* Wz_h, int ld_wz, const float* Ur, int ld_ur, const float* bu,
                            const float* Wh_h, int ld_wh, const int32_t* pred_rowptr, const int32_t* pred_col,
                            float* Hs, float* Qs, float* Ss, float* Gs, float* Zs, float* Ms, float* Rs,
                            float* wpack, int save_for_backward, const float* h_in, const unsigned char* frozen,
                            const ggpm_level_opts& o, ggpm_stream_t stream) {
    GGPM_CLEAR_STALE_ERROR();
    if (E1 <= 0 || H <= 0 || depth <= 0 || !Xz || !Xr || !Xh || !Wz_h || !Ur || !bu || !Wh_h || !pred_rowptr ||
        !pred_col || !Hs || !Qs || !wpack)
        return GGPM_ERR_ARG;
    if (save_for_backward && (!Ss || !Gs || !Zs || !Ms || !Rs)) return GGPM_ERR_ARG;
    const int Hp = ggpm_padded_hidden(H);
    if (!gru_shape_ok(Hp)) return GGPM_ERR_UNSUPPORTED;
    hipStream_t s = (hipStream_t)stream;
    const size_t HH = (size_t)Hp * Hp, slot = (size_t)E1 * Hp;
    const bool rt2 = use_rt2(o, E1, Hp, frozen != nullptr);
    const int bf16 = gate_mode(o, Hp, rt2, single_group(E1, Hp), frozen != nullptr);
    const size_t mstep = ggpm_packed_matrix_floats(Hp, bf16);
    float* pWz = wpack; float* pWh = wpack + mstep; float* pUr = wpack + 2 * mstep;
    float* pbu = wpack + 3 * ggpm_packed_matrix_slot(Hp);
    {
        GgpmPackArgs pk = {};
        pk.W[0] = Wz_h; pk.ldw[0] = ld_wz; pk.W[1] = Wh_h; pk.ldw[1] = ld_wh; pk.W[2] = Ur; pk.ldw[2] = ld_ur;
        pk.H = H; pk.Hp = Hp; pk.transpose = 0; pk.dst = wpack; pk.bias = bu; pk.bias_out = pbu; pk.bf16 = bf16;
        if (!o.weights_packed) ggpm_launch_pack(pk, 3, s);
    }
    dim3 ig(ggpm_ceil_div(Hp, 256), E1);
    const int tg0 = pick_tg(E1, Hp / 16);
    const bool gathered = o.gather_h && o.gather_idx && frozen;
    if (frozen) {
        if (h_in != Hs && !gathered) sparse_init_state<<<ig, 256, 0, s>>>(h_in, frozen, Hs, Hp);
// ... 457 lines not shown
```

### ggpm_amd/csrc/mpn_lstm.hip

```cpp
#include "tile_mma.h"
#include <cstdlib>

namespace {

constexpr int ROWS = 16;

struct LstmFwdArgs {
    int E1, Hp, tg;
    const float *Xi, *Xo, *Xu, *Xf;
    const float *Hprev, *Cprev, *Qprev;
    float *Hnew, *Cnew, *Qnew;
    float *S, *I, *O, *U, *F;
    const float *Wi, *Wo, *Wu, *Wf;
    const int32_t *rowptr, *col;
    const unsigned char* frozen;
    int fuse_b;
    int h0_zero;
    int bf16;
    int st16;
    float* Hout;
    const float *src_h, *src_c;
    const int32_t* src_idx;
};

// ... 673 lines not shown
    else if (a.bf16 == 1) { set_lds(lstm_bwd_a<1, 1>, la); lstm_bwd_a<1, 1><<<grid_a, GGPM_NWA * 64, la, s>>>(a); }
    else { set_lds(lstm_bwd_a<0, 1>, la); lstm_bwd_a<0, 1><<<grid_a, GGPM_NWA * 64, la, s>>>(a); }
    ggpm_timing_end(3, s);
    if (with_b) {
        ggpm_timing_begin(7, s, 3 * flops1);
        if (a.st16) { set_lds(lstm_bwd_b<1, 1, true>, l3); lstm_bwd_b<1, 1, true><<<grid_a, GGPM_NWA * 64, l3, s>>>(a); }
        else if (rt2) { set_lds(lstm_bwd_b<0, 2>, l3); lstm_bwd_b<0, 2><<<grid_a, GGPM_NWA * 64, l3, s>>>(a); }
        else if (a.bf16 == 2) { set_lds(lstm_bwd_b<2, 1>, l3); lstm_bwd_b<2, 1><<<grid_a, GGPM_NWA * 64, l3, s>>>(a); }
        else if (a.bf16 == 1) { set_lds(lstm_bwd_b<1, 1>, l3); lstm_bwd_b<1, 1><<<grid_a, GGPM_NWA * 64, l3, s>>>(a); }
        else { set_lds(lstm_bwd_b<0, 1>, l3); lstm_bwd_b<0, 1><<<grid_a, GGPM_NWA * 64, l3, s>>>(a); }
        ggpm_timing_end(7, s);
    }
}

}

extern "C" size_t ggpm_lstm_pack_floats(int H) {
    return 4 * ggpm_packed_matrix_slot(ggpm_padded_hidden(H));
}

static int lstm_shape_ok(int Hp) { return lds_tiles(3, Hp) <= 160 * 1024; }

namespace {
__global__ void lstm_sparse_init_state(const float* __restrict__ h_in, const float* __restrict__ c_in,
                                       const unsigned char* __restrict__ frozen, float* __restrict__ H0,
                                       float* __restrict__ C0, int Hp) {
    const int c = blockIdx.x * blockDim.x + threadIdx.x;
    const int r = blockIdx.y;
    if (c >= Hp) return;
    const size_t o = (size_t)r * Hp + c;
    H0[o] = frozen[r] ? h_in[o] : 0.f;
    C0[o] = frozen[r] ? c_in[o] : 0.f;
}
}

static int lstm_forward_impl(int E1, int H, int depth, const float* Xi, const float* Xo, const float* Xu,
                             const float* Xf, const float* Wi_h, int ld_wi, const float* Wo_h, int ld_wo,
                             const float* Wu_h, int ld_wu, const float* Wf_h, int ld_wf,
                             const int32_t* pred_rowptr, const int32_t* pred_col, float* Hs, float* Cs, float* Qs,
                             float* Ss, float* Is, float* Os, float* Us, float* Fs, float* wpack,
                             int save_for_backward, const float* h_in, const float* c_in,
                             const unsigned char* frozen, const ggpm_level_opts& o, ggpm_stream_t stream) {
    GGPM_CLEAR_STALE_ERROR();
    if (E1 <= 0 || H <= 0 || depth <= 0 || !Xi || !Xo || !Xu || !Xf || !Wi_h || !Wo_h || !Wu_h || !Wf_h ||
        !pred_rowptr || !pred_col || !Hs || !Cs || !Qs || !wpack)
        return GGPM_ERR_ARG;
    if (save_for_backward && (!Ss || !Is || !Os || !Us || !Fs)) return GGPM_ERR_ARG;
    const int Hp = ggpm_padded_hidden(H);
    if (!lstm_shape_ok(Hp) || (size_t)E1 * Hp >= ((size_t)1 << 30)) return GGPM_ERR_UNSUPPORTED;
    hipStream_t s = (hipStream_t)stream;
    const size_t HH = (size_t)Hp * Hp, slot = (size_t)E1 * Hp;
    const bool rt2 = use_rt2(o, Hp, frozen != nullptr);
    const int bf16 = gate_mode(o, Hp, rt2, pick_tg(E1, Hp / 16) >= Hp / 16, frozen != nullptr);
    const size_t mstep = ggpm_packed_matrix_floats(Hp, bf16);
    float* pWi = wpack; float* pWo = wpack + mstep; float* pWu = wpack + 2 * mstep; float* pWf = wpack + 3 * mstep;
    {
        GgpmPackArgs pk = {};
        pk.W[0] = Wi_h; pk.ldw[0] = ld_wi; pk.W[1] = Wo_h; pk.ldw[1] = ld_wo; pk.W[2] = Wu_h; pk.ldw[2] = ld_wu;
        pk.W[3] = Wf_h; pk.ldw[3] = ld_wf;
        pk.H = H; pk.Hp = Hp; pk.transpose = 0; pk.dst = wpack; pk.bias = nullptr; pk.bias_out = nullptr; pk.bf16 = bf16;
        if (!o.weights_packed) ggpm_launch_pack(pk, 4, s);
    }
    const int tg = pick_tg(E1, Hp / 16);
    const bool gathered = o.gather_h && o.gather_idx && frozen && o.gather_c;
    if (frozen) {
        dim3 ig(ggpm_ceil_div(Hp, 256), E1);
// ... 361 lines not shown
```

### include/ggpm_hip.h

```cpp
#ifndef GGPM_HIP_H
#define GGPM_HIP_H

#include <stddef.h>
#include <stdint.h>

#ifdef __cplusplus
extern "C" {
#endif

typedef void* ggpm_stream_t;

enum {
    GGPM_OK = 0,
    GGPM_ERR_ARG = 1,
    GGPM_ERR_LAUNCH = 2,
    GGPM_ERR_UNSUPPORTED = 3,
    GGPM_ERR_WORKSPACE = 4
};

enum { GGPM_ACT_NONE = 0, GGPM_ACT_RELU = 1, GGPM_ACT_TANH = 2, GGPM_ACT_SIGMOID = 3 };

int ggpm_version(void);
const char* ggpm_error_string(int code);
int ggpm_padded_hidden(int H);

int ggpm_padded_to_csr(const int64_t* padded, int rows, int width, int32_t* rowptr, int32_t* col,
                       ggpm_stream_t stream);
int ggpm_csr_transpose(const int32_t* rowptr, const int32_t* col, int rows, int ncols,
                       int32_t* rowptrT, int32_t* colT, int32_t* cursor, ggpm_stream_t stream);
int ggpm_extract_column(const int64_t* mat, int rows, int width, int column, int32_t* out,
                        ggpm_stream_t stream);

size_t ggpm_gemm_workspace_bytes(int M, int N, int K);
int ggpm_gemm(int trans_a, int trans_b, int M, int N, int K, const float* A, int lda, const float* B,
              int ldb, float* C, int ldc, int n_pad, const float* bias, int accumulate, int act,
              int zero_row0, float* splitk_ws, size_t splitk_ws_bytes, ggpm_stream_t stream);
typedef struct ggpm_gemm_problem {
    const float* A; int lda;
    const float* B; int ldb;
    float* C; int ldc; int n_pad;
    const float* bias;
    int accumulate, act, zero_row0;
} ggpm_gemm_problem;
int ggpm_gemm_grouped(int trans_a, int trans_b, int M, int N, int K, int count, const ggpm_gemm_problem* problems,
                      ggpm_stream_t stream);
size_t ggpm_gemm_grouped_splitk_workspace_bytes(int M, int N, int K, int count);
int ggpm_gemm_grouped_splitk(int trans_a, int trans_b, int M, int N, int K, int count, const ggpm_gemm_problem* problems,
                             float* ws, size_t ws_bytes, ggpm_stream_t stream);
int ggpm_gemm_ksegments(int trans_b, int M, int N, int nseg, const float* const* A, const int* lda,
                        const float* const* B, const int* ldb, const int* K, float* C, int ldc, int n_pad,
                        const float* bias, int accumulate, int act, int zero_row0, ggpm_stream_t stream);
int ggpm_gemm_tn_bf16(int M, int N, int K, const float* A, int lda, const float* B, int ldb, float* C, int ldc, float* ws,
                      size_t ws_bytes, ggpm_stream_t stream);
int ggpm_gemm_tn_bf16_applies(int M, int N, int K);
typedef struct ggpm_wgrad_item {
    const float* dpre; int ld_dpre;
    const float* x; int ld_x;
    float* dW; int ld_dw;
    float* db;
    int M, N, K;
} ggpm_wgrad_item;
int ggpm_linear_wgrads_batch(int count, const ggpm_wgrad_item* items, float* ws, size_t ws_bytes, float* csws,
                             ggpm_stream_t stream);
int ggpm_colsum(const float* A, int lda, int M, int N, float* out, float* ws, ggpm_stream_t stream);
int ggpm_act_backward(const float* dy, const float* y, int rows, int cols, int ld, int act,
                      int zero_row0, float* dpre, ggpm_stream_t stream);

int ggpm_segment_sum(const float* src, int ld_src, const int32_t* rowptr, const int32_t* col, int rows,
                     int width, float* out, int ld_out, int accumulate, int zero_to, ggpm_stream_t stream);
int ggpm_gather_rows(const float* table, int ld_table, const int32_t* idx, int rows, int width,
                     float* out, int ld_out, int col_off, int zero_to, ggpm_stream_t stream);
int ggpm_scatter_rows(const float* src, int ld_src, const int32_t* idx, int rows, int width, float* dst, int ld_dst,
                      int accumulate, ggpm_stream_t stream);
int ggpm_dropout(float* x, int rows, int cols, int ld, float p, unsigned int seed_lo, unsigned int seed_hi, int site,
                 ggpm_stream_t stream);
#define GGPM_PROP_MAX_LINEAR 5
#define GGPM_SITE_PROP_HOMO 16
#define GGPM_SITE_PROP_LUMO 20
typedef struct ggpm_prop_head {
    int n_linear;
    int width[GGPM_PROP_MAX_LINEAR + 1];
    const float* W[GGPM_PROP_MAX_LINEAR];
    const float* b[GGPM_PROP_MAX_LINEAR];
} ggpm_prop_head;
typedef struct ggpm_prop_head_grads {
    float* dW[GGPM_PROP_MAX_LINEAR];
    float* db[GGPM_PROP_MAX_LINEAR];
    int accumulate;
} ggpm_prop_head_grads;
size_t ggpm_property_heads_workspace_bytes(int B, int half, const ggpm_prop_head* homo, const ggpm_prop_head* lumo);
int ggpm_property_heads_forward(int B, const float* z, int ld, int half, const ggpm_prop_head* homo,
                                const ggpm_prop_head* lumo, const float* t_homo, const float* t_lumo, float p,
                                unsigned int seed_lo, unsigned int seed_hi, float* pred, float* loss, void* ws,
                                size_t ws_bytes, ggpm_stream_t stream);
int ggpm_property_heads_backward(int B, const float* z, int ld, int half, const ggpm_prop_head* homo,
                                 const ggpm_prop_head* lumo, const float* t_homo, const float* t_lumo, float p,
                                 const float* pred, const float* dloss, void* ws, size_t ws_bytes, float* dz, int ld_dz,
                                 int accumulate_dz, const ggpm_prop_head_grads* g_homo, const ggpm_prop_head_grads* g_lumo,
                                 ggpm_stream_t stream);
enum { GGPM_PROP_SEARCH_FIXED = 0, GGPM_PROP_SEARCH_SOFT = 1, GGPM_PROP_SEARCH_PATIENCE = 2 };
enum { GGPM_PROP_DONE = 0, GGPM_PROP_CAPPED = 1 };
int ggpm_property_latent_search(int mode, int B, const float* z, int ld, int half, const ggpm_prop_head* homo,
                                const ggpm_prop_head* lumo, const float* t_homo, const float* t_lumo, float lr, int steps,
                                float delta, float patience, float threshold, int max_steps, float* z_out, float* pred_out,
                                int32_t* steps_taken, int32_t* status, ggpm_stream_t stream);
int ggpm_adam_step(float* p, const float* g, float* m, float* v, size_t n, float lr, float beta1, float beta2, float eps,
                   float weight_decay, int step, ggpm_stream_t stream);
#define GGPM_NORM_MAX_PARTIALS 256
size_t ggpm_flat_sqnorm_workspace_bytes(size_t n);
int ggpm_flat_sqnorm_partials(const float* x, size_t n, double* partials, size_t partials_bytes, ggpm_stream_t stream);
int ggpm_flat_norm_finish(const double* partials, int n_partials, float max_norm, float* out, ggpm_stream_t stream);
#define GGPM_ADAM_MAX_GROUPS 8
typedef struct ggpm_adam_group { float lr, beta1, beta2, eps, weight_decay; } ggpm_adam_group;
int ggpm_adam_step_groups(float* p, float* g, float* m, float* v, size_t n, const uint8_t* tile_group, int n_groups,
                          const ggpm_adam_group* groups, int step, const double* partials, int n_partials, float max_norm,
                          float* clip_out, int write_clipped, ggpm_stream_t stream);
int ggpm_onehot(const int32_t* idx, int rows, int classes, float* out, int ld_out, int col_off, int zero_to,
                ggpm_stream_t stream);
int ggpm_embed_graph(const int64_t* fnode, int N1, const int64_t* fmess, int E1, int atom_size,
                     int bond_types, int max_pos, float* hnode, int ld_n, float* hmess, int ld_m,
                     ggpm_stream_t stream);

int ggpm_gru_backward_stashes(float* work, int E1, int H, int depth, float** DMP, float** DZP);
int ggpm_lstm_backward_stashes(float* work, int E1, int H, int depth, float** DI, float** DO, float** DU);
int ggpm_sum_slots(const float* src, int slots, size_t slot_floats, float* out, ggpm_stream_t stream);
int ggpm_level_bf16_storage(int E1, int H);
typedef struct ggpm_level_opts {
    int gate_dtype;
    int prefer_narrow;
    int weights_packed;
    float* defer_stash[4];
    const float* gather_h;
    const float* gather_c;
    const int32_t* gather_idx;
    float* scatter_h;
    float* scatter_c;
    const int32_t* scatter_idx;
    int skip_x_sums;
    int run_depth;
    int lo;
    int skip_bias_u;
    int skip_sparse_wgrads;
    float* h_out;
    float* c_out;
    int fixed_slot;
} ggpm_level_opts;

size_t ggpm_gru_pack_floats(int H);
int ggpm_gru_forward(int E1, int H, int depth, const float* Xz, const float* Xr, const float* Xh,
                     const float* Wz_h, int ld_wz, const float* Ur, int ld_ur, const float* bu,
                     const float* Wh_h, int ld_wh, const int32_t* pred_rowptr, const int32_t* pred_col,
                     float* Hs, float* Qs, float* Ss, float* Gs, float* Zs, float* Ms, float* Rs,
                     float* wpack, int save_for_backward, const ggpm_level_opts* opts, ggpm_stream_t stream);
size_t ggpm_gru_backward_workspace_bytes(int E1, int H, int depth);
int ggpm_gru_backward(int E1, int H, int depth, const float* Xr, const float* Wz_h, int ld_wz,
                      const float* Ur, int ld_ur, const float* Wh_h, int ld_wh,
                      const int32_t* pred_rowptr, const int32_t* pred_col, const int32_t* succ_rowptr,
                      const int32_t* succ_col, const float* Hs, const float* Qs, const float* Ss,
                      const float* Gs, const float* Zs, const float* Ms, const float* Rs, const float* dHD, float* dXz,
                      float* dXr, float* dXh, float* dWz_h, int ld_dwz, float* dUr, int ld_dur,
                      float* dbu, float* dWh_h, int ld_dwh, float* work, size_t work_bytes,
                      int weight_grads, const ggpm_level_opts* opts, ggpm_stream_t stream);
int ggpm_gru_weight_grads(int E1, int H, int depth, const float* Hs, const float* Ss, const float* Gs, float* work,
                          size_t work_bytes, float* dWz_h, int ld_dwz, float* dUr, int ld_dur, float* dbu,
                          float* dWh_h, int ld_dwh, const ggpm_level_opts* opts, ggpm_stream_t stream);

int ggpm_gru_sparse_forward(int E1, int H, int depth, const float* h_in, const unsigned char* frozen, const float* Xz,
                            const float* Xr, const float* Xh, const float* Wz_h, int ld_wz, const float* Ur, int ld_ur,
                            const float* bu, const float* Wh_h, int ld_wh, const int32_t* pred_rowptr,
                            const int32_t* pred_col, float* Hs, float* Qs, float* Ss, float* Gs, float* Zs, float* Ms,
                            float* Rs, float* wpack, int save_for_backward, const ggpm_level_opts* opts, ggpm_stream_t stream);
int ggpm_gru_sparse_backward(int E1, int H, int depth, const unsigned char* frozen, const float* Xr, const float* Wz_h,
                             int ld_wz, const float* Ur, int ld_ur, const float* Wh_h, int ld_wh,
                             const int32_t* pred_rowptr, const int32_t* pred_col, const int32_t* succ_rowptr,
                             const int32_t* succ_col, const float* Hs, const float* Qs, const float* Ss, const float* Gs,
                             const float* Zs, const float* Ms, const float* Rs, const float* dHD, float* dHin,
                             float* dXz, float* dXr, float* dXh, float* dWz_h, int ld_dwz, float* dUr, int ld_dur,
                             float* dbu, float* dWh_h, int ld_dwh, float* work, size_t work_bytes,
                             const ggpm_level_opts* opts, ggpm_stream_t stream);

size_t ggpm_lstm_pack_floats(int H);
int ggpm_lstm_forward(int E1, int H, int depth, const float* Xi, const float* Xo, const float* Xu,
                      const float* Xf, const float* Wi_h, int ld_wi, const float* Wo_h, int ld_wo,
                      const float* Wu_h, int ld_wu, const float* Wf_h, int ld_wf,
                      const int32_t* pred_rowptr, const int32_t* pred_col, float* Hs, float* Cs,
                      float* Qs, float* Ss, float* Is, float* Os, float* Us, float* Fs, float* wpack,
                      int save_for_backward, const ggpm_level_opts* opts, ggpm_stream_t stream);
size_t ggpm_lstm_backward_workspace_bytes(int E1, int H, int depth);
int ggpm_lstm_backward(int E1, int H, int depth, const float* Xf, const float* Wi_h, int ld_wi,
                       const float* Wo_h, int ld_wo, const float* Wu_h, int ld_wu, const float* Wf_h,
                       int ld_wf, const int32_t* pred_rowptr, const int32_t* pred_col,
                       const int32_t* succ_rowptr, const int32_t* succ_col, const float* Hs,
                       const float* Cs, const float* Qs, const float* Ss, const float* Is,
                       const float* Os, const float* Us, const float* Fs, const float* dHD, float* dXi,
                       float* dXo, float* dXu, float* dXf, float* dWi_h, int ld_dwi, float* dWo_h, int ld_dwo,
                       float* dWu_h, int ld_dwu, float* dWf_h, int ld_dwf, float* work,
                       size_t work_bytes, int weight_grads, const ggpm_level_opts* opts, ggpm_stream_t stream);
int ggpm_lstm_weight_grads(int E1, int H, int depth, const float* Hs, const float* Ss, float* work, size_t work_bytes,
                           float* dWi_h, int ld_dwi, float* dWo_h, int ld_dwo, float* dWu_h, int ld_dwu,
                           float* dWf_h, int ld_dwf, const ggpm_level_opts* opts, ggpm_stream_t stream);

int ggpm_lstm_sparse_forward(int E1, int H, int depth, const float* h_in, const float* c_in, const unsigned char* frozen,
                             const float* Xi, const float* Xo, const float* Xu, const float* Xf, const float* Wi_h,
                             int ld_wi, const float* Wo_h, int ld_wo, const float* Wu_h, int ld_wu, const float* Wf_h,
                             int ld_wf, const int32_t* pred_rowptr, const int32_t* pred_col, float* Hs, float* Cs,
                             float* Qs, float* Ss, float* Is, float* Os, float* Us, float* Fs, float* wpack,
                             int save_for_backward, const ggpm_level_opts* opts, ggpm_stream_t stream);
int ggpm_lstm_sparse_backward(int E1, int H, int depth, const unsigned char* frozen, const float* Xf, const float* Wi_h,
                              int ld_wi, const float* Wo_h, int ld_wo, const float* Wu_h, int ld_wu, const float* Wf_h,
                              int ld_wf, const int32_t* pred_rowptr, const int32_t* pred_col,
                              const int32_t* succ_rowptr, const int32_t* succ_col, const float* Hs, const float* Cs,
                              const float* Qs, const float* Ss, const float* Is, const float* Os, const float* Us,
                              const float* Fs, const float* dHD, const float* dCD, float* dHin, float* dCin, float* dXi,
                              float* dXo, float* dXu, float* dXf, float* dWi_h, int ld_dwi, float* dWo_h, int ld_dwo,
                              float* dWu_h, int ld_dwu, float* dWf_h, int ld_dwf, float* work, size_t work_bytes,
                              const ggpm_level_opts* opts, ggpm_stream_t stream);

size_t ggpm_weight_grads_stacked_workspace_bytes(int H, int rows);
int ggpm_gru_weight_grads_stacked(int rows, int rows_q, int H, const float* DMP, const float* Gs, const float* DZP,
                                  const float* Ss, const float* DQ, const float* Hs, float* dWz_h, int ld_dwz, float* dUr,
// ... 210 lines not shown
```

Baseline: 12180.

## Overlap weight packing on side stream and fuse encoder input, gather and activation kernels

```diff
diff --git a/ggpm_amd/_lib.py b/ggpm_amd/_lib.py
--- a/ggpm_amd/_lib.py
+++ b/ggpm_amd/_lib.py
@@ -15,6 +15,7 @@
     "ggpm_error_string": (c_char_p, [I]),
     "ggpm_padded_hidden": (I, [I]),
     "ggpm_padded_to_csr": (I, [P, I, I, P, P, P]),
+    "ggpm_padded_to_csr_pair": (I, [P, I, I, P, P, P, I, I, P, P, P]),
     "ggpm_csr_transpose": (I, [P, P, I, I, P, P, P, P]),
     "ggpm_extract_column": (I, [P, I, I, I, P, P]),
     "ggpm_gemm_workspace_bytes": (c_size_t, [I, I, I]),
@@ -23,11 +24,15 @@
     "ggpm_gemm_grouped_splitk_workspace_bytes": (c_size_t, [I, I, I, I]),
     "ggpm_gemm_grouped_splitk": (I, [I, I, I, I, I, I, P, P, c_size_t, P]),
     "ggpm_gemm_ksegments": (I, [I, I, I, I, P, P, P, P, P, P, I, I, P, I, I, I, P]),
+    "ggpm_gemm_row_table": (I, [I, I, I, I, P, I, P, I, P, I, I, P, I, I, P, P, I, I, P]),
+    "ggpm_gemm_k_quarters": (I, [I, I, I, I, P]),
     "ggpm_gemm_tn_bf16": (I, [I, I, I, P, I, P, I, P, I, P, c_size_t, P]),
     "ggpm_gemm_tn_bf16_applies": (I, [I, I, I]),
     "ggpm_colsum": (I, [P, I, I, I, P, P, P]),
     "ggpm_act_backward": (I, [P, P, I, I, I, I, I, P, P]),
+    "ggpm_act_backward_add": (I, [P, P, P, I, I, I, I, I, P, P]),
     "ggpm_segment_sum": (I, [P, I, P, P, I, I, P, I, I, I, P]),
+    "ggpm_segment_sum_masked": (I, [P, I, P, P, I, I, P, I, P, I, I, I, P, I, I, P]),
     "ggpm_gather_rows": (I, [P, I, P, I, I, P, I, I, I, P]),
     "ggpm_scatter_rows": (I, [P, I, P, I, I, P, I, I, P]),
     "ggpm_adam_step": (I, [P, P, P, P, c_size_t, c_float, c_float, c_float, c_float, c_float, I, P]),
@@ -37,12 +42,15 @@
     "ggpm_adam_step_groups": (I, [P, P, P, P, c_size_t, P, I, P, I, P, I, c_float, P, I, P]),
     "ggpm_onehot": (I, [P, I, I, P, I, I, I, P]),
     "ggpm_embed_graph": (I, [P, I, P, I, I, I, I, P, I, P, I, P]),
+    "ggpm_gate_inputs_threehot": (I, [P, I, P, I, I, I, I, I, I, P, P]),
     "ggpm_level_bf16_storage": (I, [I, I]),
     "ggpm_gru_backward_stashes": (I, [P, I, I, I, POINTER(c_void_p), POINTER(c_void_p)]),
     "ggpm_lstm_backward_stashes": (I, [P, I, I, I, POINTER(c_void_p), POINTER(c_void_p), POINTER(c_void_p)]),
     "ggpm_sum_slots": (I, [P, I, c_size_t, P, P]),
     "ggpm_gru_pack_floats": (c_size_t, [I]),
     "ggpm_gru_forward": (I, [I, I, I, P, P, P, P, I, P, I, P, P, I, P, P, P, P, P, P, P, P, P, P, I, P, P]),
+    "ggpm_gru_pack_forward": (I, [I, I, P, I, P, I, P, P, I, P, P, P]),
+    "ggpm_gru_pack_backward": (I, [I, I, P, I, P, I, P, I, P, P, P]),
     "ggpm_gru_backward_workspace_bytes": (c_size_t, [I, I, I]),
     "ggpm_gru_backward": (I, [I, I, I, P, P, I, P, I, P, I, P, P, P, P, P, P, P, P, P, P, P, P, P, P, P,
                               P, I, P, I, P, P, I, P, c_size_t, I, P, P]),
@@ -62,6 +70,8 @@
     "ggpm_decode_steps_infer_async": (I, [P, P, P, P, P, P, P, P, P, P, P, P]),
     "ggpm_lstm_pack_floats": (c_size_t, [I]),
     "ggpm_lstm_forward": (I, [I, I, I, P, P, P, P, P, I, P, I, P, I, P, I, P, P, P, P, P, P, P, P, P, P, P, I, P, P]),
+    "ggpm_lstm_pack_forward": (I, [I, I, P, I, P, I, P, I, P, I, P, P, P]),
+    "ggpm_lstm_pack_backward": (I, [I, I, P, I, P, I, P, I, P, I, P, P, P]),
     "ggpm_lstm_backward_workspace_bytes": (c_size_t, [I, I, I]),
     "ggpm_lstm_backward": (I, [I, I, I, P, P, I, P, I, P, I, P, I, P, P, P, P, P, P, P, P, P, P, P, P, P,
                                P, P, P, P, P, I, P, I, P, I, P, I, P, c_size_t, I, P, P]),
diff --git a/ggpm_amd/csrc/common.h b/ggpm_amd/csrc/common.h
--- a/ggpm_amd/csrc/common.h
+++ b/ggpm_amd/csrc/common.h
@@ -104,6 +104,15 @@
     return make_float4(ggpm_fsigmoid<BF16>(a.x), ggpm_fsigmoid<BF16>(a.y), ggpm_fsigmoid<BF16>(a.z), ggpm_fsigmoid<BF16>(a.w));
 }
 
+__device__ __forceinline__ float ggpm_act_grad(float g, float o, int act) {
+    switch (act) {
+        case GGPM_ACT_RELU: return o > 0.f ? g : 0.f;
+        case GGPM_ACT_TANH: return g * (1.f - o * o);
+        case GGPM_ACT_SIGMOID: return g * o * (1.f - o);
+        default: return g;
+    }
+}
+
 __device__ __forceinline__ void ggpm_lds_barrier() {
     asm volatile("s_waitcnt lgkmcnt(0)\n\ts_barrier" ::: "memory");
 }
diff --git a/ggpm_amd/csrc/encoder.hip b/ggpm_amd/csrc/encoder.hip
--- a/ggpm_amd/csrc/encoder.hip
+++ b/ggpm_amd/csrc/encoder.hip
@@ -335,8 +335,24 @@
     return GGPM_OK;
 }
 
+int gate_problems(const Dims& d, int E1, int I, const float* x, int ldx, float* const* P, int level, const LevelSaved& L,
+                  GgpmGemmProblem (&gp)[4]) {
+    const int H = d.H, Hp = d.Hp;
+    const size_t slot = (size_t)E1 * Hp;
+    if (d.lstm) {
+        const float* W[4] = {P[lq(level, Q_WI)], P[lq(level, Q_WOG)], P[lq(level, Q_WU)], P[lq(level, Q_WF)]};
+        const float* b[4] = {P[lq(level, Q_BI)], P[lq(level, Q_BOG)], P[lq(level, Q_BU)], P[lq(level, Q_BF)]};
+        for (int k = 0; k < 4; ++k) gp[k] = {x, ldx, W[k], I + H, L.X + k * slot, Hp, Hp, b[k], 0, GGPM_ACT_NONE, 0};
+        return 4;
+    }
+    gp[0] = {x, ldx, P[lp(level, L_WZ)], I + H, L.X, Hp, Hp, P[lp(level, L_BZ)], 0, GGPM_ACT_NONE, 0};
+    gp[1] = {x, ldx, P[lp(level, L_WR)], I, L.X + slot, Hp, Hp, nullptr, 0, GGPM_ACT_NONE, 0};
+    gp[2] = {x, ldx, P[lp(level, L_WH)], I + H, L.X + 2 * slot, Hp, Hp, P[lp(level, L_BH)], 0, GGPM_ACT_NONE, 0};
+    return 3;
+}
+
 int level_forward(const Dims& d, int E1, int N1, int I, int depth, const float* x, int ldx, float* const* P, int level,
-                  const Csr& pred, const Csr& agr, LevelSaved& L, ggpm_stream_t s) {
+                  const Csr& pred, const Csr& agr, LevelSaved& L, ggpm_stream_t s, bool x_ready = false, bool packed = false) {
     const int H = d.H, Hp = d.Hp;
     const size_t slot = (size_t)E1 * Hp;
     const int run = run_steps(d, level, depth, E1);
@@ -347,13 +363,15 @@
     o.h_out = L.hout;
     const int fs = infer ? 0 : fixed_slot(d, level, depth, E1);
     o.fixed_slot = fs;
+    o.weights_packed = packed ? 1 : 0;
     const float* result = infer ? L.hout : L.Hs + (size_t)(fs ? fs : depth) * slot;
+    if (!x_ready) {
+        GgpmGemmProblem gp[4];
+        const int gates = gate_problems(d, E1, I, x, ldx, P, level, L, gp);
+        CK(ggpm_gemm_grouped(0, 1, E1, H, I, gates, gp, s));
+    }
     if (d.lstm) {
         const float* W[4] = {P[lq(level, Q_WI)], P[lq(level, Q_WOG)], P[lq(level, Q_WU)], P[lq(level, Q_WF)]};
-        const float* b[4] = {P[lq(level, Q_BI)], P[lq(level, Q_BOG)], P[lq(level, Q_BU)], P[lq(level, Q_BF)]};
-        GgpmGemmProblem gp[4];
-        for (int k = 0; k < 4; ++k) gp[k] = {x, ldx, W[k], I + H, L.X + k * slot, Hp, Hp, b[k], 0, GGPM_ACT_NONE, 0};
-        CK(ggpm_gemm_grouped(0, 1, E1, H, I, 4, gp, s));
         const size_t dsl = (size_t)depth * slot;
         CK(ggpm_lstm_forward(E1, H, depth, L.X, L.X + slot, L.X + 2 * slot, L.X + 3 * slot, W[0] + I, I + H, W[1] + I, I + H,
                              W[2] + I, I + H, W[3] + I, I + H, pred.rowptr, pred.col, L.Hs, L.Cs, L.Qs,
@@ -363,11 +381,7 @@
         CK(ggpm_segment_sum(result, Hp, agr.rowptr, agr.col, N1, H, L.nei, Hp, 0, Hp, s));
         return GGPM_OK;
     }
-    const float *Wz = P[lp(level, L_WZ)], *Wr = P[lp(level, L_WR)], *Wh = P[lp(level, L_WH)];
-    const GgpmGemmProblem gp[3] = {{x, ldx, Wz, I + H, L.X, Hp, Hp, P[lp(level, L_BZ)], 0, GGPM_ACT_NONE, 0},
-                                   {x, ldx, Wr, I, L.X + slot, Hp, Hp, nullptr, 0, GGPM_ACT_NONE, 0},
-                                   {x, ldx, Wh, I + H, L.X + 2 * slot, Hp, Hp, P[lp(level, L_BH)], 0, GGPM_ACT_NONE, 0}};
-    CK(ggpm_gemm_grouped(0, 1, E1, H, I, 3, gp, s));
+    const float *Wz = P[lp(level, L_WZ)], *Wh = P[lp(level, L_WH)];
     const size_t ds = (size_t)depth * slot;
     CK(ggpm_gru_forward(E1, H, depth, L.X, L.X + slot, L.X + 2 * slot, Wz + I, I + H, P[lp(level, L_UR)], H,
                             P[lp(level, L_BU)], Wh + I, I + H, pred.rowptr, pred.col,
@@ -381,6 +395,23 @@
 int transpose(const Csr& c, const int32_t* col, ggpm_stream_t s) {
     return ggpm_csr_transpose(c.rowptr, col ? col : c.col, c.rows, c.ncols, c.rowptrT, c.colT, c.cursor, s);
 }
+
+int level_pack(const Dims& d, int E1, int I, float* const* P, int level, float* dst, bool backward, ggpm_stream_t s) {
+    const int H = d.H;
+    const ggpm_level_opts o = level_opts(d);
+    if (d.lstm) {
+        const float* W[4] = {P[lq(level, Q_WI)] + I, P[lq(level, Q_WOG)] + I, P[lq(level, Q_WU)] + I, P[lq(level, Q_WF)] + I};
+        return backward ? ggpm_lstm_pack_backward(E1, H, W[0], I + H, W[1], I + H, W[2], I + H, W[3], I + H, dst, &o, s)
+                        : ggpm_lstm_pack_forward(E1, H, W[0], I + H, W[1], I + H, W[2], I + H, W[3], I + H, dst, &o, s);
+    }
+    const float *Wz = P[lp(level, L_WZ)] + I, *Ur = P[lp(level, L_UR)], *Wh = P[lp(level, L_WH)] + I;
+    return backward ? ggpm_gru_pack_backward(E1, H, Wz, I + H, Ur, H, Wh, I + H, dst, &o, s)
+                    : ggpm_gru_pack_forward(E1, H, Wz, I + H, Ur, H, P[lp(level, L_BU)], Wh, I + H, dst, &o, s);
+}
+
+struct PackJoin {
+    hipEvent_t wait, done[3];
+};
 
 }
 
@@ -431,8 +462,24 @@
         if (!ev_in) return GGPM_ERR_LAUNCH;
         (void)hipEventRecord(ev_in, s);
     }
-    CK(ggpm_padded_to_csr(gbgraph, d.E1g, d.Kgb, S.gpred.rowptr, S.gpred.col, stream));
-    CK(ggpm_padded_to_csr(gagraph, d.N1g, d.Kga, S.gagr.rowptr, S.gagr.col, stream));
+    const bool packs_aside = side_stream != nullptr && !infer;
+    PackJoin pj = {};
+    if (packs_aside) {
+        pj.wait = ev_in;
+        for (int l = 0; l < 3; ++l)
+            if (!(pj.done[l] = ggpm_wgrad_event(55 + l))) return GGPM_ERR_LAUNCH;
+        auto packs = [=]() -> int {
+            (void)hipStreamWaitEvent((hipStream_t)side_stream, pj.wait, 0);
+            for (int l = 2; l >= 0; --l) {
+                CK(level_pack(d, l == 2 ? d.E1g : d.E1t, l == 2 ? d.Ig : d.It, P, l, S.lv[l].wpack, false, side_stream));
+                (void)hipEventRecord(pj.done[l], (hipStream_t)side_stream);
+            }
+            return GGPM_OK;
+        };
+        CK(packs());
+    }
+    CK(ggpm_padded_to_csr_pair(gbgraph, d.E1g, d.Kgb, S.gpred.rowptr, S.gpred.col, gagraph, d.N1g, d.Kga, S.gagr.rowptr,
+                               S.gagr.col, stream));
     hipEvent_t ev_atom = nullptr, ev_tree = nullptr;
     if (side_stream) {
         ev_atom = ggpm_wgrad_event(54);
@@ -440,8 +487,17 @@
         if (!ev_atom || !ev_tree) return GGPM_ERR_LAUNCH;
         (void)hipEventRecord(ev_atom, s);
     }
+    const bool wo_table = (d.atom & 3) != 0;
+    {
+        GgpmGemmProblem gp[4];
+        const int gates = gate_problems(d, d.E1g, d.Ig, S.hmess_a, d.ld_m, P, 2, S.lv[2], gp);
+        CK(ggpm_gate_inputs_threehot(gfnode, d.N1g, gfmess, d.E1g, d.atom, 4, 20, H, gates, gp, stream));
+    }
+    if (packs_aside) (void)hipStreamWaitEvent(s, pj.done[2], 0);
     auto tree_layout = [=]() -> int {
         if (side_stream) (void)hipStreamWaitEvent((hipStream_t)side_stream, ev_in, 0);
+        if (!infer || !wo_table)
+            CK(ggpm_embed_graph(gfnode, d.N1g, gfmess, d.E1g, d.atom, 4, 20, S.hnode_a, d.ld_n, S.hmess_a, d.ld_m, ts));
         CK(ggpm_padded_to_csr(tbgraph, d.E1t, d.Ktb, S.tpred.rowptr, S.tpred.col, ts));
         CK(ggpm_padded_to_csr(tagraph, d.N1t, d.Kta, S.tagr.rowptr, S.tagr.col, ts));
         CK(ggpm_padded_to_csr(tcgraph, d.N1t, d.Ktc, S.tcgr.rowptr, S.tcgr.col, ts));
@@ -483,10 +539,20 @@
         CK(tree_layout());
     }
 
-    CK(ggpm_embed_graph(gfnode, d.N1g, gfmess, d.E1g, d.atom, 4, 20, S.hnode_a, d.ld_n, S.hmess_a, d.ld_m, stream));
-    CK(level_forward(d, d.E1g, d.N1g, d.Ig, d.depthG, S.hmess_a, d.ld_m, P, 2, S.gpred, S.gagr, S.lv[2], stream));
-    CK(linear2(d.N1g, H, S.hnode_a, d.ld_n, d.atom, S.lv[2].nei, Hp, H, P[lwo(d.lstm, 2)], P[lbo(d.lstm, 2)], GGPM_ACT_RELU, 1,
-               hatom, Hp, stream));
+    CK(level_forward(d, d.E1g, d.N1g, d.Ig, d.depthG, S.hmess_a, d.ld_m, P, 2, S.gpred, S.gagr, S.lv[2], stream, true,
+                     packs_aside));
+    if (wo_table) {
+        const float* Wo = P[lwo(d.lstm, 2)];
+        CK(ggpm_gemm_row_table(1, d.N1g, H, H, S.lv[2].nei, Hp, Wo + d.atom, d.atom + H, hatom, Hp, Hp, Wo, d.atom + H, d.atom,
+                               gfnode, P[lbo(d.lstm, 2)], GGPM_ACT_RELU, 1, stream));
+    } else {
+        if (side_stream) {
+            if (wk) CK(wk->drain());
+            (void)hipStreamWaitEvent(s, ev_tree, 0);
+        }
+        CK(linear2(d.N1g, H, S.hnode_a, d.ld_n, d.atom, S.lv[2].nei, Hp, H, P[lwo(d.lstm, 2)], P[lbo(d.lstm, 2)], GGPM_ACT_RELU,
+                   1, hatom, Hp, stream));
+    }
     CK(drop(d, hatom, d.N1g, H, Hp, DS_WO_ATOM, stream));
 
     if (wk) CK(wk->drain());
@@ -496,7 +562,9 @@
                stream));
     CK(drop(d, S.hnode_i, d.N1t, H, Hp, DS_WI, stream));
     CK(ggpm_gather_rows(S.hnode_i, Hp, S.src, d.E1t, H, S.hmess_i, d.ld_t, 0, 0, stream));
-    CK(level_forward(d, d.E1t, d.N1t, d.It, d.depthT, S.hmess_i, d.ld_t, P, 1, S.tpred, S.tagr, S.lv[1], stream));
+    if (packs_aside) (void)hipStreamWaitEvent(s, pj.done[1], 0);
+    CK(level_forward(d, d.E1t, d.N1t, d.It, d.depthT, S.hmess_i, d.ld_t, P, 1, S.tpred, S.tagr, S.lv[1], stream, false,
+                     packs_aside));
     CK(linear2(d.N1t, H, S.hnode_i, Hp, H, S.lv[1].nei, Hp, H, P[lwo(d.lstm, 1)], P[lbo(d.lstm, 1)], GGPM_ACT_RELU, 1, hinter, Hp,
                stream));
     CK(drop(d, hinter, d.N1t, H, Hp, DS_WO_INTER, stream));
@@ -504,7 +572,9 @@
     CK(linear2(d.N1t, H, S.finput_t, d.Hep, He, hinter, Hp, H, P[P_WC], P[P_BC], GGPM_ACT_RELU, 0, S.hnode_t, Hp, stream));
     CK(drop(d, S.hnode_t, d.N1t, H, Hp, DS_WC, stream));
     CK(ggpm_gather_rows(S.hnode_t, Hp, S.src, d.E1t, H, S.hmess_t, d.ld_t, 0, 0, stream));
-    CK(level_forward(d, d.E1t, d.N1t, d.It, d.depthT, S.hmess_t, d.ld_t, P, 0, S.tpred, S.tagr, S.lv[0], stream));
+    if (packs_aside) (void)hipStreamWaitEvent(s, pj.done[0], 0);
+    CK(level_forward(d, d.E1t, d.N1t, d.It, d.depthT, S.hmess_t, d.ld_t, P, 0, S.tpred, S.tagr, S.lv[0], stream, false,
+                     packs_aside));
     CK(linear2(d.N1t, H, S.hnode_t, Hp, H, S.lv[0].nei, Hp, H, P[lwo(d.lstm, 0)], P[lbo(d.lstm, 0)], GGPM_ACT_RELU, 1, hnode, Hp,
                stream));
     CK(drop(d, hnode, d.N1t, H, Hp, DS_WO_TREE, stream));
@@ -540,7 +610,7 @@
 
 struct BwdWork {
     float *dpre_root, *df, *dn, *d_hnode_t, *d_nei_t, *dpre, *d_h, *dX, *dx_mess, *d_finput, *d_hinter, *d_hnode_i,
-        *d_nei_i, *d_pooled, *d_hatom, *d_nei_g, *level_work, *skws, *csws;
+        *d_nei_i, *d_pooled, *d_nei_g, *level_work, *skws, *csws;
     size_t level_work_bytes, skws_bytes;
     float *xws[3], *xcs[3];
     size_t xws_bytes;
@@ -560,7 +630,7 @@
     w.d_hinter = A.take<float>((size_t)d.N1t * Hp);
     w.d_hnode_i = A.take<float>((size_t)d.N1t * Hp); w.d_nei_i = A.take<float>((size_t)d.N1t * Hp);
     w.d_pooled = A.take<float>((size_t)d.N1t * Hp);
-    w.d_hatom = A.take<float>((size_t)d.N1g * Hp); w.d_nei_g = A.take<float>((size_t)d.N1g * Hp);
+    w.d_nei_g = A.take<float>((size_t)d.N1g * Hp);
     size_t lw = d.lstm ? ggpm_lstm_backward_workspace_bytes(d.E1g, d.H, d.depthG)
                        : ggpm_gru_backward_workspace_bytes(d.E1g, d.H, d.depthG);
     const size_t lwt = d.lstm ? ggpm_lstm_backward_workspace_bytes(d.E1t, d.H, d.depthT)
@@ -641,7 +711,7 @@
 
 int level_backward(const Dims& d, int E1, int I, int depth, const float* x, int ldx, float* const* P, float* const* G,
                    int level, const Csr& pred, const LevelSaved& L, const float* dHD, float* dX, float* level_work,
-                   float* dx, int lddx, BwdWork& w, Streams& st) {
+                   float* dx, int lddx, BwdWork& w, Streams& st, bool packed) {
     const int H = d.H, Hp = d.Hp;
     const size_t slot = (size_t)E1 * Hp, ds = (size_t)depth * slot;
     const int blo = backward_lo(d, level, depth, E1);
@@ -652,6 +722,7 @@
     o.lo = blo;
     o.fixed_slot = fixed_slot(d, level, depth, E1);
     o.skip_x_sums = skip_xsum;
+    o.weights_packed = packed ? 1 : 0;
     if (d.lstm) {
         const float* W[4] = {P[lq(level, Q_WI)], P[lq(level, Q_WOG)], P[lq(level, Q_WU)], P[lq(level, Q_WF)]};
         float* dW[4] = {G[lq(level, Q_WI)], G[lq(level, Q_WOG)], G[lq(level, Q_WU)], G[lq(level, Q_WF)]};
@@ -812,7 +883,7 @@
     for (int i = 0; i < 3; ++i) dXl[i] = w.dX + (size_t)i * 4 * Emax * Hp;
     float* lwork[3];
     for (int i = 0; i < 3; ++i) lwork[i] = w.level_work + (size_t)i * (w.level_work_bytes / 4 + 64);
-    const size_t nt = (size_t)d.N1t * Hp * sizeof(float), ng = (size_t)d.N1g * Hp * sizeof(float);
+    const size_t nt = (size_t)d.N1t * Hp * sizeof(float);
 
     if (side_stream && phase != 2) {
         hipEvent_t ev = ggpm_wgrad_event(61);
@@ -820,6 +891,22 @@
         (void)hipEventRecord(ev, (hipStream_t)side_stream);
         (void)hipStreamWaitEvent(s, ev, 0);
     }
+    const bool packs_aside = side_stream != nullptr;
+    PackJoin pj = {};
+    if (packs_aside) {
+        for (int l = 0; l < 3; ++l)
+            if (!(pj.done[l] = ggpm_wgrad_event(45 + l))) return GGPM_ERR_LAUNCH;
+    }
+    if (packs_aside && phase != 2) {
+        if (!(pj.wait = ggpm_wgrad_event(44))) return GGPM_ERR_LAUNCH;
+        (void)hipEventRecord(pj.wait, s);
+        (void)hipStreamWaitEvent((hipStream_t)side_stream, pj.wait, 0);
+        for (int l = 0; l < 3; ++l) {
+            CK(level_pack(d, l == 2 ? d.E1g : d.E1t, l == 2 ? d.Ig : d.It, P, l, lwork[l], true, side_stream));
+            (void)hipEventRecord(pj.done[l], (hipStream_t)side_stream);
+        }
+    }
+
     if (phase != 2) {
     if (d_hroot) {
         CK(ggpm_act_backward(d_hroot, hroot, d.B, H, Hp, GGPM_ACT_TANH, 0, w.dpre_root, stream));
@@ -854,13 +941,13 @@
         }));
     }
     CK(ggpm_segment_sum(w.d_nei_t, Hp, S.tagr.rowptrT, S.tagr.colT, d.E1t, H, w.d_h, Hp, 0, Hp, stream));
+    if (packs_aside) (void)hipStreamWaitEvent(s, pj.done[0], 0);
     CK(level_backward(d, d.E1t, d.It, d.depthT, S.hmess_t, d.ld_t, P, G, 0, S.tpred, S.lv[0], w.d_h, dXl[0], lwork[0],
-                      w.dx_mess, d.ld_t, w, st));
-    CK(ggpm_segment_sum(w.dx_mess, d.ld_t, S.tsrc.rowptrT, S.tsrc.colT, d.N1t, H, w.d_hnode_t, Hp, 1, 0, stream));
-    CK(ggpm_act_backward(w.d_hnode_t, S.hnode_t, d.N1t, H, Hp, GGPM_ACT_RELU, 0, dpre[1], stream));
+                      w.dx_mess, d.ld_t, w, st, packs_aside));
+    CK(ggpm_segment_sum_masked(w.dx_mess, d.ld_t, S.tsrc.rowptrT, S.tsrc.colT, d.N1t, H, w.d_hnode_t, Hp, S.hnode_t, Hp,
+                               GGPM_ACT_RELU, 0, dpre[1], Hp, 0, stream));
     CK(drop(d, dpre[1], d.N1t, H, Hp, DS_WC, stream));
-    if (d_hinter) (void)hipMemcpyAsync(w.d_hinter, d_hinter, nt, hipMemcpyDeviceToDevice, s);
-    CK(linear2_dx(d.N1t, H, He, dpre[1], Hp, P[P_WC], w.d_finput, d.Hep, 0, w.d_hinter, Hp, d_hinter ? 1 : 0, stream));
+    CK(linear2_dx(d.N1t, H, He, dpre[1], Hp, P[P_WC], w.d_finput, d.Hep, 0, w.d_hinter, Hp, 0, stream));
     CK(drop(d, w.d_finput, d.N1t, He, d.Hep, DS_EC, stream));
     CK(linear2_wgrad(d.N1t, H, dpre[1], Hp, S.finput_t, d.Hep, He, hinter, Hp, H, G[P_WC], G[P_BC], w, st));
     {
@@ -869,15 +956,16 @@
         CK(st.on_side([=]() -> int { return ggpm_segment_sum(src, Hep, rp, cl, rows, He, g, He, 0, He, sw); }));
     }
 
-    CK(ggpm_act_backward(w.d_hinter, hinter, d.N1t, H, Hp, GGPM_ACT_RELU, 1, dpre[2], stream));
+    CK(ggpm_act_backward_add(w.d_hinter, d_hinter, hinter, d.N1t, H, Hp, GGPM_ACT_RELU, 1, dpre[2], stream));
     CK(drop(d, dpre[2], d.N1t, H, Hp, DS_WO_INTER, stream));
     CK(linear2_dx(d.N1t, H, H, dpre[2], Hp, P[lwo(d.lstm, 1)], w.d_hnode_i, Hp, 0, w.d_nei_i, Hp, 0, stream));
     CK(linear2_wgrad(d.N1t, H, dpre[2], Hp, S.hnode_i, Hp, H, S.lv[1].nei, Hp, H, G[lwo(d.lstm, 1)], G[lbo(d.lstm, 1)], w, st));
     CK(ggpm_segment_sum(w.d_nei_i, Hp, S.tagr.rowptrT, S.tagr.colT, d.E1t, H, w.d_h, Hp, 0, Hp, stream));
+    if (packs_aside) (void)hipStreamWaitEvent(s, pj.done[1], 0);
     CK(level_backward(d, d.E1t, d.It, d.depthT, S.hmess_i, d.ld_t, P, G, 1, S.tpred, S.lv[1], w.d_h, dXl[1], lwork[1],
-                      w.dx_mess, d.ld_t, w, st));
-    CK(ggpm_segment_sum(w.dx_mess, d.ld_t, S.tsrc.rowptrT, S.tsrc.colT, d.N1t, H, w.d_hnode_i, Hp, 1, 0, stream));
-    CK(ggpm_act_backward(w.d_hnode_i, S.hnode_i, d.N1t, H, Hp, GGPM_ACT_RELU, 0, dpre[3], stream));
+                      w.dx_mess, d.ld_t, w, st, packs_aside));
+    CK(ggpm_segment_sum_masked(w.dx_mess, d.ld_t, S.tsrc.rowptrT, S.tsrc.colT, d.N1t, H, w.d_hnode_i, Hp, S.hnode_i, Hp,
+                               GGPM_ACT_RELU, 0, dpre[3], Hp, 0, stream));
     CK(drop(d, dpre[3], d.N1t, H, Hp, DS_WI, stream));
     float* d_finput_i = w.d_finput + (size_t)d.N1t * d.Hep;
     CK(linear2_dx(d.N1t, H, He, dpre[3], Hp, P[P_WI], d_finput_i, d.Hep, 0, w.d_pooled, Hp, 0, stream));
@@ -888,26 +976,26 @@
         float* const g = G[P_EI]; const ggpm_stream_t sw = st.w(); const int Hep = d.Hep, rows = d.n_attach;
         CK(st.on_side([=]() -> int { return ggpm_segment_sum(d_finput_i, Hep, rp, cl, rows, He, g, He, 0, He, sw); }));
     }
-    if (d_hatom) (void)hipMemcpyAsync(w.d_hatom, d_hatom, ng, hipMemcpyDeviceToDevice, s);
-    CK(ggpm_segment_sum(w.d_pooled, Hp, S.tcgr.rowptrT, S.tcgr.colT, d.N1g, H, w.d_hatom, Hp, d_hatom ? 1 : 0,
-                        d_hatom ? 0 : Hp, stream));
+    CK(ggpm_segment_sum_masked(w.d_pooled, Hp, S.tcgr.rowptrT, S.tcgr.colT, d.N1g, H, d_hatom, Hp, hatom, Hp, GGPM_ACT_RELU, 1,
+                               dpre[4], Hp, 0, stream));
 
     }
     if (phase == 1) {
+        if (packs_aside) (void)hipStreamWaitEvent(s, pj.done[2], 0);
         CK(st.drain());
         GGPM_CHECK_LAUNCH();
         return GGPM_OK;
     }
 
-    CK(ggpm_act_backward(w.d_hatom, hatom, d.N1g, H, Hp, GGPM_ACT_RELU, 1, dpre[4], stream));
     CK(drop(d, dpre[4], d.N1g, H, Hp, DS_WO_ATOM, stream));
     CK(ggpm_gemm(0, 0, d.N1g, H, H, dpre[4], Hp, P[lwo(d.lstm, 2)] + d.atom, d.atom + H, w.d_nei_g, Hp, Hp, nullptr, 0,
                  GGPM_ACT_NONE, 0, nullptr, 0, stream));
     CK(linear2_wgrad(d.N1g, H, dpre[4], Hp, S.hnode_a, d.ld_n, d.atom, S.lv[2].nei, Hp, H, G[lwo(d.lstm, 2)], G[lbo(d.lstm, 2)], w,
                      st));
     CK(ggpm_segment_sum(w.d_nei_g, Hp, S.gagr.rowptrT, S.gagr.colT, d.E1g, H, w.d_h, Hp, 0, Hp, stream));
+    if (packs_aside && phase != 2) (void)hipStreamWaitEvent(s, pj.done[2], 0);
     CK(level_backward(d, d.E1g, d.Ig, d.depthG, S.hmess_a, d.ld_m, P, G, 2, S.gpred, S.lv[2], w.d_h, dXl[2], lwork[2],
-                      nullptr, 0, w, st));
+                      nullptr, 0, w, st, packs_aside));
 
     CK(st.drain());
     if (side_stream) {
diff --git a/ggpm_amd/csrc/gather.hip b/ggpm_amd/csrc/gather.hip
--- a/ggpm_amd/csrc/gather.hip
+++ b/ggpm_amd/csrc/gather.hip
@@ -2,28 +2,45 @@
 #include <cmath>
 
 namespace {
+
+struct SegmentSumExtra {
+    const float* addend; int ld_addend;
+    const float* y; int ld_y, act, zero_row0;
+};
 
 template <bool VEC>
 __global__ void __launch_bounds__(256) segment_sum_k(const float* __restrict__ src, int ld_src,
                                                      const int32_t* __restrict__ rowptr,
                                                      const int32_t* __restrict__ col, int rows, int width,
-                                                     float* __restrict__ out, int ld_out, int accumulate, int zero_to) {
+                                                     float* __restrict__ out, int ld_out, int accumulate, int zero_to,
+                                                     SegmentSumExtra x) {
     const int lane = threadIdx.x & 63;
     const int r = blockIdx.x * 4 + (threadIdx.x >> 6);
     if (r >= rows) return;
     const int lo = rowptr[r], hi = rowptr[r + 1];
     float* dst = out + (size_t)r * ld_out;
+    const float* add = x.addend ? x.addend + (size_t)r * x.ld_addend : (accumulate ? dst : nullptr);
+    const float* y = x.y ? x.y + (size_t)r * x.ld_y : nullptr;
+    const bool zero_row = x.zero_row0 && r == 0;
     for (int c = width + lane; c < zero_to; c += 64) dst[c] = 0.f;
     if (VEC) {
         for (int c = lane * 4; c < width; c += 256) {
-            float4 acc = accumulate ? ggpm_ld4(dst + c) : ggpm_zero4();
+            float4 acc = add ? ggpm_ld4(add + c) : ggpm_zero4();
             for (int j = lo; j < hi; ++j) acc = acc + ggpm_ld4(src + (size_t)col[j] * ld_src + c);
+            if (y) {
+                const float4 o = ggpm_ld4(y + c);
+                acc = make_float4(ggpm_act_grad(acc.x, o.x, x.act), ggpm_act_grad(acc.y, o.y, x.act),
+                                  ggpm_act_grad(acc.z, o.z, x.act), ggpm_act_grad(acc.w, o.w, x.act));
+            }
+            if (zero_row) acc = ggpm_zero4();
             ggpm_st4(dst + c, acc);
         }
     } else {
         for (int c = lane; c < width; c += 64) {
-            float acc = accumulate ? dst[c] : 0.f;
+            float acc = add ? add[c] : 0.f;
             for (int j = lo; j < hi; ++j) acc += src[(size_t)col[j] * ld_src + c];
+            if (y) acc = ggpm_act_grad(acc, y[c], x.act);
+            if (zero_row) acc = 0.f;
             dst[c] = acc;
         }
     }
@@ -89,22 +106,114 @@
     }
 }
 
+constexpr int GI_ROWS = 96, GI_THREADS = 1024, GI_COL_CHUNKS = 4, GI_UNROLL = 5, GI_MAX_GATES = 4;
+struct GateInputArgs {
+    const float* W[GI_MAX_GATES]; int ldw[GI_MAX_GATES];
+    const float* bias[GI_MAX_GATES];
+    float* X[GI_MAX_GATES]; int ldx[GI_MAX_GATES];
+    int quarters;
+    const int64_t *fnode, *fmess;
+    int N1, E1, atom, bond_types, max_pos, H, Hp, Hc;
+};
+
+__global__ void __launch_bounds__(GI_THREADS) gate_inputs_threehot_k(GateInputArgs a) {
+    extern __shared__ float gi_w[];
+    __shared__ int feat[GI_ROWS][3];
+    const int g = blockIdx.z, I = a.atom + a.bond_types + a.max_pos, S = I | 1, H = a.H;
+    const int c0 = blockIdx.y * a.Hc;
+    const int hc = min(a.Hc, H - c0);
+    const int wc = min(a.Hc, a.Hp - c0);
+    const int e0 = blockIdx.x * GI_ROWS;
+    int ka = -1, kt = -1, kp = -1;
+    if (threadIdx.x < GI_ROWS && e0 + (int)threadIdx.x < a.E1) {
+        const int64_t* f = a.fmess + (size_t)(e0 + threadIdx.x) * 4;
+        const int64_t u = f[0], t = f[2], p = f[3];
+        if (u >= 0 && u < a.N1) {
+            const int64_t at = a.fnode[u];
+            if (at >= 0 && at < a.atom) ka = (int)at;
+        }
+        if (t >= 0 && t < a.bond_types) kt = a.atom + (int)t;
+        if (p >= 0 && p < a.max_pos) kp = a.atom + a.bond_types + (int)p;
+    }
+    if (threadIdx.x < GI_ROWS) { feat[threadIdx.x][0] = ka; feat[threadIdx.x][1] = kt; feat[threadIdx.x][2] = kp; }
+    const float* __restrict__ W = a.W[g] + (size_t)c0 * a.ldw[g];
+    const int ldw = a.ldw[g], n = hc * I;
+    for (int base = 0; base < n; base += GI_THREADS * GI_UNROLL) {
+        float v[GI_UNROLL];
+        int at[GI_UNROLL];
+#pragma unroll
+        for (int u = 0; u < GI_UNROLL; ++u) {
+            const int i = base + u * GI_THREADS + threadIdx.x;
+            const int c = i / I, k = i - c * I;
+            at[u] = i < n ? c * S + k : -1;
+            v[u] = i < n ? W[(size_t)c * ldw + k] : 0.f;
+        }
+#pragma unroll
+        for (int u = 0; u < GI_UNROLL; ++u)
+            if (at[u] >= 0) gi_w[at[u]] = v[u];
+    }
+    float* bias = gi_w + a.Hc * S;
+    const float* __restrict__ b = a.bias[g];
+    for (int c = threadIdx.x; c < hc; c += GI_THREADS) bias[c] = b ? b[c0 + c] : 0.f;
+    __syncthreads();
+    const bool quarters = (a.quarters >> g) & 1;
+    float* __restrict__ X = a.X[g] + c0;
+    const int ldx = a.ldx[g];
+    const int rows = min(GI_ROWS, a.E1 - e0);
+    for (int i = threadIdx.x; i < rows * wc; i += GI_THREADS) {
+        const int r = i / wc, c = i - r * wc;
+        float v = 0.f;
+        if (c < hc) {
+            const int fa = feat[r][0], ft = feat[r][1], fp = feat[r][2];
+            const int qa = quarters ? (fa & 63) >> 4 : 0, qt = quarters ? (ft & 63) >> 4 : 0, qp = quarters ? (fp & 63) >> 4 : 0;
+            const float* w = gi_w + c * S;
+            const float va = fa >= 0 ? w[fa] : 0.f, vt = ft >= 0 ? w[ft] : 0.f, vp = fp >= 0 ? w[fp] : 0.f;
+            float part[4];
+#pragma unroll
+            for (int q = 0; q < 4; ++q) {
+                float s = 0.f;
+                s += qa == q ? va : 0.f;
+                s += qt == q ? vt : 0.f;
+                s += qp == q ? vp : 0.f;
+                part[q] = s;
+            }
+            v = ((part[0] + part[1]) + (part[2] + part[3])) + bias[c];
+        }
+        X[(size_t)(e0 + r) * ldx + c] = v;
+    }
+}
+
+}
+
+static int segment_sum_launch(const float* src, int ld_src, const int32_t* rowptr, const int32_t* col, int rows, int width,
+                              float* out, int ld_out, int accumulate, int zero_to, const SegmentSumExtra& x,
+                              ggpm_stream_t stream) {
+    GGPM_CLEAR_STALE_ERROR();
+    if (!src || !rowptr || !col || !out || rows <= 0 || width <= 0) return GGPM_ERR_ARG;
+    hipStream_t s = (hipStream_t)stream;
+    bool vec = (width % 4 == 0) && (ld_src % 4 == 0) && (ld_out % 4 == 0) &&
+               (((uintptr_t)src & 15) == 0) && (((uintptr_t)out & 15) == 0);
+    if (x.addend) vec = vec && (x.ld_addend % 4 == 0) && (((uintptr_t)x.addend & 15) == 0);
+    if (x.y) vec = vec && (x.ld_y % 4 == 0) && (((uintptr_t)x.y & 15) == 0);
+    const int grid = ggpm_ceil_div(rows, 4);
+    if (vec) segment_sum_k<true><<<grid, 256, 0, s>>>(src, ld_src, rowptr, col, rows, width, out, ld_out, accumulate,
+                                                           zero_to, x);
+    else segment_sum_k<false><<<grid, 256, 0, s>>>(src, ld_src, rowptr, col, rows, width, out, ld_out, accumulate, zero_to, x);
+    GGPM_CHECK_LAUNCH();
+    return GGPM_OK;
 }
 
 extern "C" int ggpm_segment_sum(const float* src, int ld_src, const int32_t* rowptr, const int32_t* col,
                                 int rows, int width, float* out, int ld_out, int accumulate, int zero_to,
                                 ggpm_stream_t stream) {
-    GGPM_CLEAR_STALE_ERROR();
-    if (!src || !rowptr || !col || !out || rows <= 0 || width <= 0) return GGPM_ERR_ARG;
-    hipStream_t s = (hipStream_t)stream;
-    const bool vec = (width % 4 == 0) && (ld_src % 4 == 0) && (ld_out % 4 == 0) &&
-                     (((uintptr_t)src & 15) == 0) && (((uintptr_t)out & 15) == 0);
-    const int grid = ggpm_ceil_div(rows, 4);
-    if (vec) segment_sum_k<true><<<grid, 256, 0, s>>>(src, ld_src, rowptr, col, rows, width, out, ld_out, accumulate,
-                                                           zero_to);
-    else segment_sum_k<false><<<grid, 256, 0, s>>>(src, ld_src, rowptr, col, rows, width, out, ld_out, accumulate, zero_to);
-    GGPM_CHECK_LAUNCH();
-    return GGPM_OK;
+    return segment_sum_launch(src, ld_src, rowptr, col, rows, width, out, ld_out, accumulate, zero_to, SegmentSumExtra{}, stream);
+}
+
+extern "C" int ggpm_segment_sum_masked(const float* src, int ld_src, const int32_t* rowptr, const int32_t* col, int rows,
+                                       int width, const float* addend, int ld_addend, const float* y, int ld_y, int act,
+                                       int zero_row0, float* out, int ld_out, int zero_to, ggpm_stream_t stream) {
+    const SegmentSumExtra x = {addend, ld_addend, y, ld_y, act, zero_row0};
+    return segment_sum_launch(src, ld_src, rowptr, col, rows, width, out, ld_out, 0, zero_to, x, stream);
 }
 
 extern "C" int ggpm_gather_rows(const float* table, int ld_table, const int32_t* idx, int rows, int width,
@@ -147,6 +256,31 @@
         return GGPM_ERR_UNSUPPORTED;
     embed_graph_k<<<N1 + E1, 256, 0, (hipStream_t)stream>>>(fnode, N1, fmess, E1, atom_size, bond_types, max_pos,
                                                            hnode, ld_n, hmess, ld_m);
+    GGPM_CHECK_LAUNCH();
+    return GGPM_OK;
+}
+
+extern "C" int ggpm_gate_inputs_threehot(const int64_t* fnode, int N1, const int64_t* fmess, int E1, int atom_size, int bond_types,
+                                         int max_pos, int H, int count, const ggpm_gemm_problem* gates, ggpm_stream_t stream) {
+    GGPM_CLEAR_STALE_ERROR();
+    if (!fnode || !fmess || !gates || N1 <= 0 || E1 <= 0 || atom_size <= 0 || bond_types <= 0 || max_pos <= 0 || H <= 0 ||
+        count <= 0 || count > GI_MAX_GATES)
+        return GGPM_ERR_ARG;
+    const int I = atom_size + bond_types + max_pos, Hp = ggpm_padded_hidden(H);
+    const int Hc = ggpm_ceil_div(Hp, GI_COL_CHUNKS);
+    const size_t lds = ((size_t)Hc * (I | 1) + Hc) * sizeof(float);
+    if (lds > 60 * 1024) return GGPM_ERR_UNSUPPORTED;
+    GateInputArgs a = {};
+    for (int g = 0; g < count; ++g) {
+        const ggpm_gemm_problem& p = gates[g];
+        if (!p.B || !p.C || p.ldb < I || p.ldc < Hp) return GGPM_ERR_ARG;
+        a.W[g] = p.B; a.ldw[g] = p.ldb; a.bias[g] = p.bias; a.X[g] = p.C; a.ldx[g] = p.ldc;
+    }
+    a.quarters = ggpm_gemm_k_quarters(E1, H, I, count, gates);
+    a.fnode = fnode; a.fmess = fmess; a.N1 = N1; a.E1 = E1; a.atom = atom_size; a.bond_types = bond_types; a.max_pos = max_pos;
+    a.H = H; a.Hp = Hp; a.Hc = Hc;
+    const dim3 grid(ggpm_ceil_div(E1, GI_ROWS), ggpm_ceil_div(Hp, Hc), count);
+    gate_inputs_threehot_k<<<grid, GI_THREADS, lds, (hipStream_t)stream>>>(a);
     GGPM_CHECK_LAUNCH();
     return GGPM_OK;
 }
diff --git a/ggpm_amd/csrc/gemm.hip b/ggpm_amd/csrc/gemm.hip
--- a/ggpm_amd/csrc/gemm.hip
+++ b/ggpm_amd/csrc/gemm.hip
@@ -21,6 +21,9 @@
     const float* segA[GGPM_GEMM_MAX_GROUP];
     const float* segB[GGPM_GEMM_MAX_GROUP];
     int seg_lda[GGPM_GEMM_MAX_GROUP], seg_ldb[GGPM_GEMM_MAX_GROUP], segK[GGPM_GEMM_MAX_GROUP];
+    const float* tab; int ld_tab, tab_cols;
+    const int64_t* tab_idx;
+    const float* tab_bias;
 };
 
 struct GemmGroupArgs {
@@ -34,6 +37,14 @@
         case GGPM_ACT_SIGMOID: return ggpm_sigmoid(v);
         default: return v;
     }
+}
+
+__device__ __forceinline__ float table_addend(const GemmArgs& g, int m, int n) {
+    const int64_t a = g.tab_idx[m];
+    float v = 0.f;
+    if (a >= 0 && a < g.tab_cols) v += g.tab[(size_t)n * g.ld_tab + a];
+    if (g.tab_bias) v += g.tab_bias[n];
+    return v;
 }
 
 template <bool CONTIG_K>
@@ -136,7 +147,8 @@
             float v = acc[r];
             if (g.bias) v += g.bias[n];
             float* dst = g.C + (size_t)m * g.ldc + n;
-            if (g.accumulate) v += *dst;
+            if (g.tab) v += table_addend(g, m, n);
+            else if (g.accumulate) v += *dst;
             v = apply_act(v, g.act);
             if (g.zero_row0 && m == 0) v = 0.f;
             *dst = v;
@@ -276,7 +288,8 @@
             float v = acc[r];
             if (g.bias) v += g.bias[n];
             float* dst = g.C + (size_t)m * g.ldc + n;
-            if (g.accumulate) v += *dst;
+            if (g.tab) v += table_addend(g, m, n);
+            else if (g.accumulate) v += *dst;
             v = apply_act(v, g.act);
             if (g.zero_row0 && m == 0) v = 0.f;
             *dst = v;
@@ -484,7 +497,8 @@
                       (part[(2 * 16 + r) * 64 + l] + part[(3 * 16 + r) * 64 + l]);
             if (g.bias) v += g.bias[n];
             float* dst = g.C + (size_t)m * g.ldc + n;
-            if (g.accumulate) v += *dst;
+            if (g.tab) v += table_addend(g, m, n);
+            else if (g.accumulate) v += *dst;
             v = apply_act(v, g.act);
             if (g.zero_row0 && m == 0) v = 0.f;
             *dst = v;
@@ -1026,19 +1040,15 @@
     }
 }
 
-__global__ void act_backward_k(const float* __restrict__ dy, const float* __restrict__ y, int rows, int cols,
-                               int ld, int act, int zero_row0, float* __restrict__ dpre) {
+__global__ void act_backward_k(const float* __restrict__ dy, const float* __restrict__ dy2, const float* __restrict__ y,
+                               int rows, int cols, int ld, int act, int zero_row0, float* __restrict__ dpre) {
     const int c = blockIdx.x * blockDim.x + threadIdx.x;
     const int r = blockIdx.y;
     if (c >= cols) return;
     const size_t i = (size_t)r * ld + c;
     float g = dy[i], o = y[i];
-    switch (act) {
-        case GGPM_ACT_RELU: g = o > 0.f ? g : 0.f; break;
-        case GGPM_ACT_TANH: g = g * (1.f - o * o); break;
-        case GGPM_ACT_SIGMOID: g = g * o * (1.f - o); break;
-        default: break;
-    }
+    if (dy2) g += dy2[i];
+    g = ggpm_act_grad(g, o, act);
     if (zero_row0 && r == 0) g = 0.f;
     dpre[i] = g;
 }
@@ -1079,16 +1089,25 @@
     return bytes;
 }
 
-extern "C" int ggpm_gemm(int trans_a, int trans_b, int M, int N, int K, const float* A, int lda,
-                         const float* B, int ldb, float* C, int ldc, int n_pad, const float* bias,
-                         int accumulate, int act, int zero_row0, float* splitk_ws, size_t splitk_ws_bytes,
-                         ggpm_stream_t stream) {
+namespace {
+struct RowTable {
+    const float* tab; int ld_tab, tab_cols;
+    const int64_t* idx;
+    const float* bias;
+};
+}
+
+static int gemm_impl(int trans_a, int trans_b, int M, int N, int K, const float* A, int lda, const float* B, int ldb, float* C,
+                     int ldc, int n_pad, const float* bias, int accumulate, int act, int zero_row0, float* splitk_ws,
+                     size_t splitk_ws_bytes, const RowTable& rt, ggpm_stream_t stream) {
     GGPM_CLEAR_STALE_ERROR();
     if (!A || !B || !C || M <= 0 || N <= 0 || K <= 0 || n_pad < N || n_pad > ldc) return GGPM_ERR_ARG;
+    if (rt.tab && (trans_a || splitk_ws || accumulate)) return GGPM_ERR_ARG;
     hipStream_t s = (hipStream_t)stream;
     GemmArgs g{};
     g.M = M; g.N = N; g.K = K; g.A = A; g.lda = lda; g.B = B; g.ldb = ldb; g.C = C; g.ldc = ldc;
     g.n_pad = n_pad; g.bias = bias; g.accumulate = accumulate; g.act = act; g.zero_row0 = zero_row0;
+    g.tab = rt.tab; g.ld_tab = rt.ld_tab; g.tab_cols = rt.tab_cols; g.tab_idx = rt.idx; g.tab_bias = rt.bias;
     g.vecA = ((lda & 3) == 0) && (((uintptr_t)A & 15) == 0);
     g.vecB = ((ldb & 3) == 0) && (((uintptr_t)B & 15) == 0);
     static const int use_tall = [] { const char* e = ggpm_dev_env("GGPM_GEMM_TALL"); return e ? atoi(e) : 1; }();
@@ -1179,6 +1198,22 @@
     return GGPM_OK;
 }
 
+extern "C" int ggpm_gemm(int trans_a, int trans_b, int M, int N, int K, const float* A, int lda,
+                         const float* B, int ldb, float* C, int ldc, int n_pad, const float* bias,
+                         int accumulate, int act, int zero_row0, float* splitk_ws, size_t splitk_ws_bytes,
+                         ggpm_stream_t stream) {
+    return gemm_impl(trans_a, trans_b, M, N, K, A, lda, B, ldb, C, ldc, n_pad, bias, accumulate, act, zero_row0, splitk_ws,
+                     splitk_ws_bytes, RowTable{}, stream);
+}
+
+extern "C" int ggpm_gemm_row_table(int trans_b, int M, int N, int K, const float* A, int lda, const float* B, int ldb, float* C,
+                                   int ldc, int n_pad, const float* table, int ld_table, int table_cols, const int64_t* row_idx,
+                                   const float* table_bias, int act, int zero_row0, ggpm_stream_t stream) {
+    if (!table || !row_idx || table_cols <= 0 || ld_table < table_cols) return GGPM_ERR_ARG;
+    const RowTable rt = {table, ld_table, table_cols, row_idx, table_bias};
+    return gemm_impl(0, trans_b, M, N, K, A, lda, B, ldb, C, ldc, n_pad, nullptr, 0, act, zero_row0, nullptr, 0, rt, stream);
+}
+
 namespace {
 inline bool v2_operands_ok(const float* A, int lda, size_t rows_a, const float* B, int ldb, size_t rows_b) {
     static const int use_v2 = [] { const char* e = ggpm_dev_env("GGPM_GEMM_V2"); return e ? atoi(e) : 1; }();
@@ -1334,6 +1369,17 @@
     return GGPM_OK;
 }
 
+extern "C" int ggpm_gemm_k_quarters(int M, int N, int K, int count, const ggpm_gemm_problem* p) {
+    if (count <= 0 || count > GGPM_GEMM_MAX_GROUP || !p || M <= 0 || N <= 0 || K <= 0) return 0;
+    bool all = count > 1;
+    for (int i = 0; i < count; ++i) all = all && v2_operands_ok(p[i].A, p[i].lda, M, p[i].B, p[i].ldb, N);
+    if (all) return small_launch(M, N, count) ? (1 << count) - 1 : 0;
+    int mask = 0;
+    for (int i = 0; i < count; ++i)
+        if (small_launch(M, N, 1) && v2_operands_ok(p[i].A, p[i].lda, M, p[i].B, p[i].ldb, N)) mask |= 1 << i;
+    return mask;
+}
+
 extern "C" size_t ggpm_gemm_grouped_splitk_workspace_bytes(int M, int N, int K, int count) {
     if (M <= 0 || N <= 0 || K <= 0 || count <= 0 || count > GGPM_GEMM_MAX_GROUP || !small_launch(M, N, count)) return 0;
     int kc;
@@ -1443,14 +1489,19 @@
     return GGPM_OK;
 }
 
-extern "C" int ggpm_act_backward(const float* dy, const float* y, int rows, int cols, int ld, int act,
-                                 int zero_row0, float* dpre, ggpm_stream_t stream) {
+extern "C" int ggpm_act_backward_add(const float* dy, const float* dy2, const float* y, int rows, int cols, int ld, int act,
+                                     int zero_row0, float* dpre, ggpm_stream_t stream) {
     GGPM_CLEAR_STALE_ERROR();
     if (!dy || !y || !dpre || rows <= 0 || cols <= 0) return GGPM_ERR_ARG;
     dim3 grid(ggpm_ceil_div(cols, 256), rows);
-    act_backward_k<<<grid, 256, 0, (hipStream_t)stream>>>(dy, y, rows, cols, ld, act, zero_row0, dpre);
+    act_backward_k<<<grid, 256, 0, (hipStream_t)stream>>>(dy, dy2, y, rows, cols, ld, act, zero_row0, dpre);
     GGPM_CHECK_LAUNCH();
     return GGPM_OK;
+}
+
+extern "C" int ggpm_act_backward(const float* dy, const float* y, int rows, int cols, int ld, int act,
+                                 int zero_row0, float* dpre, ggpm_stream_t stream) {
+    return ggpm_act_backward_add(dy, nullptr, y, rows, cols, ld, act, zero_row0, dpre, stream);
 }
 
 extern "C" int ggpm_linear_wgrads_batch(int count, const ggpm_wgrad_item* items, float* ws, size_t ws_bytes, float* csws,
diff --git a/ggpm_amd/csrc/graph.hip b/ggpm_amd/csrc/graph.hip
--- a/ggpm_amd/csrc/graph.hip
+++ b/ggpm_amd/csrc/graph.hip
@@ -124,10 +124,17 @@
     __syncthreads();
 }
 
-__global__ void __launch_bounds__(SCAN_THREADS) padded_to_csr_small(const int64_t* __restrict__ padded, int rows,
-                                                                     int width, int32_t* __restrict__ rowptr,
-                                                                     int32_t* __restrict__ col) {
+struct PaddedToCsrArgs {
+    const int64_t* padded[2];
+    int rows[2], width[2];
+    int32_t *rowptr[2], *col[2];
+};
+__global__ void __launch_bounds__(SCAN_THREADS) padded_to_csr_small(PaddedToCsrArgs a) {
     __shared__ int32_t partial[SCAN_THREADS];
+    const int64_t* __restrict__ padded = a.padded[blockIdx.x];
+    const int rows = a.rows[blockIdx.x], width = a.width[blockIdx.x];
+    int32_t* __restrict__ rowptr = a.rowptr[blockIdx.x];
+    int32_t* __restrict__ col = a.col[blockIdx.x];
     for (int r = threadIdx.x; r < rows; r += SCAN_THREADS) {
         const int64_t* p = padded + (size_t)r * width;
         int c = 0;
@@ -249,7 +256,8 @@
     if (!padded || !rowptr || !col || rows <= 0 || width <= 0) return GGPM_ERR_ARG;
     hipStream_t s = (hipStream_t)stream;
     if (rows <= SMALL_ROWS) {
-        padded_to_csr_small<<<1, SCAN_THREADS, 0, s>>>(padded, rows, width, rowptr, col);
+        const PaddedToCsrArgs a = {{padded, padded}, {rows, rows}, {width, width}, {rowptr, rowptr}, {col, col}};
+        padded_to_csr_small<<<1, SCAN_THREADS, 0, s>>>(a);
         GGPM_CHECK_LAUNCH();
         return GGPM_OK;
     }
@@ -259,6 +267,22 @@
     fill_csr_from_padded<<<B, T, 0, s>>>(padded, rows, width, rowptr, col);
     GGPM_CHECK_LAUNCH();
     return GGPM_OK;
+}
+
+extern "C" int ggpm_padded_to_csr_pair(const int64_t* padded0, int rows0, int width0, int32_t* rowptr0, int32_t* col0,
+                                       const int64_t* padded1, int rows1, int width1, int32_t* rowptr1, int32_t* col1,
+                                       ggpm_stream_t stream) {
+    GGPM_CLEAR_STALE_ERROR();
+    if (!padded0 || !rowptr0 || !col0 || rows0 <= 0 || width0 <= 0 || !padded1 || !rowptr1 || !col1 || rows1 <= 0 || width1 <= 0)
+        return GGPM_ERR_ARG;
+    if (rows0 <= SMALL_ROWS && rows1 <= SMALL_ROWS) {
+        const PaddedToCsrArgs a = {{padded0, padded1}, {rows0, rows1}, {width0, width1}, {rowptr0, rowptr1}, {col0, col1}};
+        padded_to_csr_small<<<2, SCAN_THREADS, 0, (hipStream_t)stream>>>(a);
+        GGPM_CHECK_LAUNCH();
+        return GGPM_OK;
+    }
+    const int rc = ggpm_padded_to_csr(padded0, rows0, width0, rowptr0, col0, stream);
+    return rc ? rc : ggpm_padded_to_csr(padded1, rows1, width1, rowptr1, col1, stream);
 }
 
 extern "C" int ggpm_csr_transpose(const int32_t* rowptr, const int32_t* col, int rows, int ncols,
diff --git a/ggpm_amd/csrc/mpn_gru.hip b/ggpm_amd/csrc/mpn_gru.hip
--- a/ggpm_amd/csrc/mpn_gru.hip
+++ b/ggpm_amd/csrc/mpn_gru.hip
@@ -845,6 +845,37 @@
     if (c >= Hp) return;
     H0[(size_t)r * Hp + c] = frozen[r] ? h_in[(size_t)r * Hp + c] : 0.f;
 }
+}
+
+extern "C" int ggpm_gru_pack_forward(int E1, int H, const float* Wz_h, int ld_wz, const float* Ur, int ld_ur, const float* bu,
+                                     const float* Wh_h, int ld_wh, float* wpack, const ggpm_level_opts* opts,
+                                     ggpm_stream_t stream) {
+    GGPM_CLEAR_STALE_ERROR();
+    if (E1 <= 0 || H <= 0 || !Wz_h || !Ur || !bu || !Wh_h || !wpack) return GGPM_ERR_ARG;
+    const ggpm_level_opts& o = ggpm_opts_or_default(opts);
+    const int Hp = ggpm_padded_hidden(H);
+    GgpmPackArgs pk = {};
+    pk.W[0] = Wz_h; pk.ldw[0] = ld_wz; pk.W[1] = Wh_h; pk.ldw[1] = ld_wh; pk.W[2] = Ur; pk.ldw[2] = ld_ur;
+    pk.H = H; pk.Hp = Hp; pk.transpose = 0; pk.dst = wpack; pk.bias = bu; pk.bias_out = wpack + 3 * ggpm_packed_matrix_slot(Hp);
+    pk.bf16 = gate_mode(o, Hp, use_rt2(o, E1, Hp, false), single_group(E1, Hp), false);
+    ggpm_launch_pack(pk, 3, (hipStream_t)stream);
+    GGPM_CHECK_LAUNCH();
+    return GGPM_OK;
+}
+
+extern "C" int ggpm_gru_pack_backward(int E1, int H, const float* Wz_h, int ld_wz, const float* Ur, int ld_ur, const float* Wh_h,
+                                      int ld_wh, float* work, const ggpm_level_opts* opts, ggpm_stream_t stream) {
+    GGPM_CLEAR_STALE_ERROR();
+    if (E1 <= 0 || H <= 0 || !Wz_h || !Ur || !Wh_h || !work) return GGPM_ERR_ARG;
+    const ggpm_level_opts& o = ggpm_opts_or_default(opts);
+    const int Hp = ggpm_padded_hidden(H);
+    GgpmPackArgs pk = {};
+    pk.W[0] = Wz_h; pk.ldw[0] = ld_wz; pk.W[1] = Wh_h; pk.ldw[1] = ld_wh; pk.W[2] = Ur; pk.ldw[2] = ld_ur;
+    pk.H = H; pk.Hp = Hp; pk.transpose = 1; pk.dst = work; pk.bias = nullptr; pk.bias_out = nullptr;
+    pk.bf16 = gate_mode(o, Hp, use_rt2(o, E1, Hp, false), single_group(E1, Hp), false);
+    ggpm_launch_pack(pk, 3, (hipStream_t)stream);
+    GGPM_CHECK_LAUNCH();
+    return GGPM_OK;
 }
 
 static int gru_forward_impl(int E1, int H, int depth, const float* Xz, const float* Xr, const float* Xh,
diff --git a/ggpm_amd/csrc/mpn_lstm.hip b/ggpm_amd/csrc/mpn_lstm.hip
--- a/ggpm_amd/csrc/mpn_lstm.hip
+++ b/ggpm_amd/csrc/mpn_lstm.hip
@@ -729,6 +729,34 @@
     H0[o] = frozen[r] ? h_in[o] : 0.f;
     C0[o] = frozen[r] ? c_in[o] : 0.f;
 }
+}
+
+static int lstm_pack(int E1, int H, const float* Wi_h, int ld_wi, const float* Wo_h, int ld_wo, const float* Wu_h, int ld_wu,
+                     const float* Wf_h, int ld_wf, float* dst, int transpose, const ggpm_level_opts* opts, ggpm_stream_t stream) {
+    GGPM_CLEAR_STALE_ERROR();
+    if (E1 <= 0 || H <= 0 || !Wi_h || !Wo_h || !Wu_h || !Wf_h || !dst) return GGPM_ERR_ARG;
+    const ggpm_level_opts& o = ggpm_opts_or_default(opts);
+    const int Hp = ggpm_padded_hidden(H);
+    GgpmPackArgs pk = {};
+    pk.W[0] = Wi_h; pk.ldw[0] = ld_wi; pk.W[1] = Wo_h; pk.ldw[1] = ld_wo; pk.W[2] = Wu_h; pk.ldw[2] = ld_wu;
+    pk.W[3] = Wf_h; pk.ldw[3] = ld_wf;
+    pk.H = H; pk.Hp = Hp; pk.transpose = transpose; pk.dst = dst; pk.bias = nullptr; pk.bias_out = nullptr;
+    pk.bf16 = gate_mode(o, Hp, use_rt2(o, Hp, false), pick_tg(E1, Hp / 16) >= Hp / 16, false);
+    ggpm_launch_pack(pk, 4, (hipStream_t)stream);
+    GGPM_CHECK_LAUNCH();
+    return GGPM_OK;
+}
+
+extern "C" int ggpm_lstm_pack_forward(int E1, int H, const float* Wi_h, int ld_wi, const float* Wo_h, int ld_wo,
+                                      const float* Wu_h, int ld_wu, const float* Wf_h, int ld_wf, float* wpack,
+                                      const ggpm_level_opts* opts, ggpm_stream_t stream) {
+    return lstm_pack(E1, H, Wi_h, ld_wi, Wo_h, ld_wo, Wu_h, ld_wu, Wf_h, ld_wf, wpack, 0, opts, stream);
+}
+
+extern "C" int ggpm_lstm_pack_backward(int E1, int H, const float* Wi_h, int ld_wi, const float* Wo_h, int ld_wo,
+                                       const float* Wu_h, int ld_wu, const float* Wf_h, int ld_wf, float* work,
+                                       const ggpm_level_opts* opts, ggpm_stream_t stream) {
+    return lstm_pack(E1, H, Wi_h, ld_wi, Wo_h, ld_wo, Wu_h, ld_wu, Wf_h, ld_wf, work, 1, opts, stream);
 }
 
 static int lstm_forward_impl(int E1, int H, int depth, const float* Xi, const float* Xo, const float* Xu,
diff --git a/include/ggpm_hip.h b/include/ggpm_hip.h
--- a/include/ggpm_hip.h
+++ b/include/ggpm_hip.h
@@ -26,6 +26,9 @@
 
 int ggpm_padded_to_csr(const int64_t* padded, int rows, int width, int32_t* rowptr, int32_t* col,
                        ggpm_stream_t stream);
+int ggpm_padded_to_csr_pair(const int64_t* padded0, int rows0, int width0, int32_t* rowptr0, int32_t* col0,
+                            const int64_t* padded1, int rows1, int width1, int32_t* rowptr1, int32_t* col1,
+                            ggpm_stream_t stream);
 int ggpm_csr_transpose(const int32_t* rowptr, const int32_t* col, int rows, int ncols,
                        int32_t* rowptrT, int32_t* colT, int32_t* cursor, ggpm_stream_t stream);
 int ggpm_extract_column(const int64_t* mat, int rows, int width, int column, int32_t* out,
@@ -50,6 +53,10 @@
 int ggpm_gemm_ksegments(int trans_b, int M, int N, int nseg, const float* const* A, const int* lda,
                         const float* const* B, const int* ldb, const int* K, float* C, int ldc, int n_pad,
                         const float* bias, int accumulate, int act, int zero_row0, ggpm_stream_t stream);
+int ggpm_gemm_row_table(int trans_b, int M, int N, int K, const float* A, int lda, const float* B, int ldb, float* C, int ldc,
+                        int n_pad, const float* table, int ld_table, int table_cols, const int64_t* row_idx,
+                        const float* table_bias, int act, int zero_row0, ggpm_stream_t stream);
+int ggpm_gemm_k_quarters(int M, int N, int K, int count, const ggpm_gemm_problem* problems);
 int ggpm_gemm_tn_bf16(int M, int N, int K, const float* A, int lda, const float* B, int ldb, float* C, int ldc, float* ws,
                       size_t ws_bytes, ggpm_stream_t stream);
 int ggpm_gemm_tn_bf16_applies(int M, int N, int K);
@@ -65,9 +72,14 @@
 int ggpm_colsum(const float* A, int lda, int M, int N, float* out, float* ws, ggpm_stream_t stream);
 int ggpm_act_backward(const float* dy, const float* y, int rows, int cols, int ld, int act,
                       int zero_row0, float* dpre, ggpm_stream_t stream);
+int ggpm_act_backward_add(const float* dy, const float* dy2, const float* y, int rows, int cols, int ld, int act,
+                          int zero_row0, float* dpre, ggpm_stream_t stream);
 
 int ggpm_segment_sum(const float* src, int ld_src, const int32_t* rowptr, const int32_t* col, int rows,
                      int width, float* out, int ld_out, int accumulate, int zero_to, ggpm_stream_t stream);
+int ggpm_segment_sum_masked(const float* src, int ld_src, const int32_t* rowptr, const int32_t* col, int rows, int width,
+                            const float* addend, int ld_addend, const float* y, int ld_y, int act, int zero_row0,
+                            float* out, int ld_out, int zero_to, ggpm_stream_t stream);
 int ggpm_gather_rows(const float* table, int ld_table, const int32_t* idx, int rows, int width,
                      float* out, int ld_out, int col_off, int zero_to, ggpm_stream_t stream);
 int ggpm_scatter_rows(const float* src, int ld_src, const int32_t* idx, int rows, int width, float* dst, int ld_dst,
@@ -120,6 +132,8 @@
 int ggpm_embed_graph(const int64_t* fnode, int N1, const int64_t* fmess, int E1, int atom_size,
                      int bond_types, int max_pos, float* hnode, int ld_n, float* hmess, int ld_m,
                      ggpm_stream_t stream);
+int ggpm_gate_inputs_threehot(const int64_t* fnode, int N1, const int64_t* fmess, int E1, int atom_size, int bond_types,
+                              int max_pos, int H, int count, const ggpm_gemm_problem* gates, ggpm_stream_t stream);
 
 int ggpm_gru_backward_stashes(float* work, int E1, int H, int depth, float** DMP, float** DZP);
 int ggpm_lstm_backward_stashes(float* work, int E1, int H, int depth, float** DI, float** DO, float** DU);
@@ -164,6 +178,10 @@
 int ggpm_gru_weight_grads(int E1, int H, int depth, const float* Hs, const float* Ss, const float* Gs, float* work,
                           size_t work_bytes, float* dWz_h, int ld_dwz, float* dUr, int ld_dur, float* dbu,
                           float* dWh_h, int ld_dwh, const ggpm_level_opts* opts, ggpm_stream_t stream);
+int ggpm_gru_pack_forward(int E1, int H, const float* Wz_h, int ld_wz, const float* Ur, int ld_ur, const float* bu,
+                          const float* Wh_h, int ld_wh, float* wpack, const ggpm_level_opts* opts, ggpm_stream_t stream);
+int ggpm_gru_pack_backward(int E1, int H, const float* Wz_h, int ld_wz, const float* Ur, int ld_ur, const float* Wh_h,
+                           int ld_wh, float* work, const ggpm_level_opts* opts, ggpm_stream_t stream);
 
 int ggpm_gru_sparse_forward(int E1, int H, int depth, const float* h_in, const unsigned char* frozen, const float* Xz,
                             const float* Xr, const float* Xh, const float* Wz_h, int ld_wz, const float* Ur, int ld_ur,
@@ -186,6 +204,12 @@
                       const int32_t* pred_rowptr, const int32_t* pred_col, float* Hs, float* Cs,
                       float* Qs, float* Ss, float* Is, float* Os, float* Us, float* Fs, float* wpack,
                       int save_for_backward, const ggpm_level_opts* opts, ggpm_stream_t stream);
+int ggpm_lstm_pack_forward(int E1, int H, const float* Wi_h, int ld_wi, const float* Wo_h, int ld_wo, const float* Wu_h,
+                           int ld_wu, const float* Wf_h, int ld_wf, float* wpack, const ggpm_level_opts* opts,
+                           ggpm_stream_t stream);
+int ggpm_lstm_pack_backward(int E1, int H, const float* Wi_h, int ld_wi, const float* Wo_h, int ld_wo, const float* Wu_h,
+                            int ld_wu, const float* Wf_h, int ld_wf, float* work, const ggpm_level_opts* opts,
+                            ggpm_stream_t stream);
 size_t ggpm_lstm_backward_workspace_bytes(int E1, int H, int depth);
 int ggpm_lstm_backward(int E1, int H, int depth, const float* Xf, const float* Wi_h, int ld_wi,
                        const float* Wo_h, int ld_wo, const float* Wu_h, int ld_wu, const float* Wf_h,
```

Result: no change. 12430, median of 6 (+2.0%).
